# DanecLacey/basic_iterative_solvers

Hardware: AMD Instinct MI355X
Metric: CG iterations/sec + SpMV GFLOP/s (% HBM roofline), HPCG 256^3 at 1/2/4/8 GPUs (higher is better)
Workload: dtype f64

## Files before the change

basic_iterative_solvers_amd/__init__.py:

```python
import ctypes as C
import os

import numpy as np

PKG = os.path.dirname(os.path.abspath(__file__))
LIB_PATH = os.path.join(PKG, "lib", "libbis_hip.so")

PC = dict(none=0, j=1, gs=2, bgs=3, sgs=4, **{"2st": 5, "s2st": 6, "ilu0": 7, "ilu0it": 8, "fsai": 9, "mg": 10, "bj": 11})

_lib = None


class BisError(RuntimeError):
    pass


def load_library():
    global _lib
    if _lib is None:
        if not os.path.exists(LIB_PATH):
            raise BisError(
                f"{LIB_PATH} is missing: build it with "
                "`python -m basic_iterative_solvers_amd.build` (hipcc, gfx950)")
        _lib = C.CDLL(LIB_PATH)
# ... 165 lines not shown

    def scale_sym(self, A, init=0.0):
        s = self.alloc(A.n_rows)
        self.init_vector(s, init)
        self.check(self.lib.bis_mat_scale_sym(self.h, A.h, C.c_void_p(s.ptr)))
        return s

    def gather(self, out, vec, perm):
        n = len(perm)
        raw = np.zeros((n + 1) // 2 + 1)
        raw.view(np.int32)[:n] = np.asarray(perm, dtype=np.int32)
        store = self.upload(raw)
        self.check(self.lib.bis_vec_gather(self.h, C.c_void_p(out.ptr), C.c_void_p(vec.ptr), C.c_void_p(store.ptr), _i64(n)))
        self.sync()
        store.free()

    def tune_placement(self, A, max_trials=6):
        f, b = C.c_double(), C.c_double()
        self.check(self.lib.bis_mat_tune_placement(self.h, A.h, C.c_int(max_trials), C.byref(f), C.byref(b)))
        return f.value, b.value

    def split_strict(self, A):
        n = A.n_rows
        D, Dinv = self.alloc(n), self.alloc(n)
        hl, hu = C.c_void_p(), C.c_void_p()
        self.check(self.lib.bis_mat_split_strict(self.h, A.h, C.byref(hl), C.byref(hu),
                                                 C.c_void_p(D.ptr), C.c_void_p(Dinv.ptr)))
        return Mat(self, hl), Mat(self, hu), D, Dinv

    def mat_diag(self, A, row_offset=0):
        D, Dinv = self.alloc(A.n_rows), self.alloc(A.n_rows)
        self.check(self.lib.bis_mat_diag(self.h, A.h, _i64(row_offset), C.c_void_p(D.ptr), C.c_void_p(Dinv.ptr)))
        return D, Dinv

    def diag_block(self, A, row_offset=0):
        h = C.c_void_p()
        self.check(self.lib.bis_mat_diag_block(self.h, A.h, _i64(row_offset), C.byref(h)))
        return Mat(self, h)

    def ilu0(self, A, pivot_tol=1e-8, pivot_repl=1e-4):
        n = A.n_rows
        L_D, U_D = self.alloc(n), self.alloc(n)
        hl, hu = C.c_void_p(), C.c_void_p()
        self.check(self.lib.bis_mat_ilu0(self.h, A.h, C.c_double(pivot_tol), C.c_double(pivot_repl),
                                         C.byref(hl), C.byref(hu), C.c_void_p(L_D.ptr),
                                         C.c_void_p(U_D.ptr)))
        return Mat(self, hl), L_D, Mat(self, hu), U_D

    def iluk(self, A, level, pivot_tol=1e-8, pivot_repl=1e-4):
        n = A.n_rows
        L_D, U_D = self.alloc(n), self.alloc(n)
        hl, hu, nf = C.c_void_p(), C.c_void_p(), C.c_int64()
        self.check(self.lib.bis_mat_iluk(self.h, A.h, C.c_int(int(level)), C.c_double(pivot_tol), C.c_double(pivot_repl),
                                         C.byref(hl), C.byref(hu), C.c_void_p(L_D.ptr), C.c_void_p(U_D.ptr), C.byref(nf)))
        return Mat(self, hl), L_D, Mat(self, hu), U_D, nf.value

    def iluk_symbolic(self, A, level):
        h, nf = C.c_void_p(), C.c_int64()
        self.check(self.lib.bis_mat_iluk_symbolic(self.h, A.h, C.c_int(int(level)), C.byref(h), C.byref(nf)))
        return Mat(self, h), nf.value

    def fsai(self, A):
        hg, hgt, nf = C.c_void_p(), C.c_void_p(), C.c_int64()
        self.check(self.lib.bis_mat_fsai(self.h, A.h, C.byref(hg), C.byref(hgt), C.byref(nf)))
        return Mat(self, hg), Mat(self, hgt), nf.value

    def spgemm(self, A, B):
        h = C.c_void_p()
        self.check(self.lib.bis_spgemm(self.h, A.h, B.h, C.byref(h)))
        return Mat(self, h)

    def mg(self, A, cycle=None, cycle_levels=0, smooth=False, prolong_omega=0.0, smoother=None, degree=2, ratio=None, est_steps=10,
           safety=1.1, **params):
        m = MG(self, A, smooth=smooth, prolong_omega=prolong_omega, **params)
        try:
            if cycle is not None:
                m.set_cycle(cycle, cycle_levels)
            if smoother is not None:
                m.set_smoother(smoother, degree=degree, ratio=ratio, est_steps=est_steps, safety=safety)
        except Exception:
            m.free()
            raise
        return m

    def bjacobi(self, A, block_size=None, block_ptr=None, symmetrize=False):
        return BJ(self, A, block_size, block_ptr, symmetrize)

    def spmv(self, A, x, y):
        self.check(self.lib.bis_spmv(self.h, A.h, C.c_void_p(x.ptr), C.c_void_p(y.ptr)))

    def spmm(self, A, X, Y, k):
        self.check(self.lib.bis_spmm(self.h, A.h, C.c_void_p(X.ptr), C.c_void_p(Y.ptr), C.c_int(int(k))))

    def mvec_set_col(self, X, n, k, j, v):
        self.check(self.lib.bis_mvec_set_col(self.h, C.c_void_p(X.ptr), _i64(n), C.c_int(int(k)), C.c_int(int(j)), C.c_void_p(v.ptr)))

    def mvec_get_col(self, v, X, n, k, j):
        self.check(self.lib.bis_mvec_get_col(self.h, C.c_void_p(v.ptr), C.c_void_p(X.ptr), _i64(n), C.c_int(int(k)), C.c_int(int(j))))

    def sptrsv(self, Ls, x, D, b):
        self.check(self.lib.bis_sptrsv(self.h, Ls.h, C.c_void_p(x.ptr), C.c_void_p(D.ptr),
                                       C.c_void_p(b.ptr)))

    def bsptrsv(self, Us, x, D, b):
        self.check(self.lib.bis_bsptrsv(self.h, Us.h, C.c_void_p(x.ptr), C.c_void_p(D.ptr),
                                        C.c_void_p(b.ptr)))

    def sptrsm(self, Ls, X, D, B, k):
        self.check(self.lib.bis_sptrsm(self.h, Ls.h, C.c_void_p(X.ptr), C.c_void_p(D.ptr), C.c_void_p(B.ptr), C.c_int(int(k))))

    def bsptrsm(self, Us, X, D, B, k):
        self.check(self.lib.bis_bsptrsm(self.h, Us.h, C.c_void_p(X.ptr), C.c_void_p(D.ptr), C.c_void_p(B.ptr), C.c_int(int(k))))

    def mitrsv(self, T, D_inv, B, X, work, n_sweeps, k):
        self.check(self.lib.bis_mitrsv(self.h, T.h, C.c_void_p(D_inv.ptr), C.c_void_p(B.ptr), C.c_void_p(X.ptr),
                                       C.c_void_p(work.ptr) if work is not None else C.c_void_p(), C.c_int(int(n_sweeps)), C.c_int(int(k))))

    def mvec_div_diag(self, R, A, D, n, k):
        self.check(self.lib.bis_mvec_div_diag(self.h, C.c_void_p(R.ptr), C.c_void_p(A.ptr), C.c_void_p(D.ptr), _i64(n), C.c_int(int(k))))

    def mvec_mul_diag(self, R, A, D, n, k):
        self.check(self.lib.bis_mvec_mul_diag(self.h, C.c_void_p(R.ptr), C.c_void_p(A.ptr), C.c_void_p(D.ptr), _i64(n), C.c_int(int(k))))

    def itrsv(self, T, D_inv, b, x, work, n_sweeps):
        self.check(self.lib.bis_itrsv(self.h, T.h, C.c_void_p(D_inv.ptr), C.c_void_p(b.ptr), C.c_void_p(x.ptr),
                                      C.c_void_p(work.ptr) if work is not None else C.c_void_p(), C.c_int(int(n_sweeps))))

    def _ew3(self, fn, r, a, b, scale, n=None):
        n = r.n if n is None else n
        self.check(fn(self.h, C.c_void_p(r.ptr), C.c_void_p(a.ptr), C.c_void_p(b.ptr), _i64(n),
                      C.c_double(scale)))

    def subtract_vectors(self, r, a, b, scale=1.0, n=None):
        self._ew3(self.lib.bis_subtract_vectors, r, a, b, scale, n)

    def sum_vectors(self, r, a, b, scale=1.0, n=None):
        self._ew3(self.lib.bis_sum_vectors, r, a, b, scale, n)

    def elemwise_mult_vectors(self, r, a, b, scale=1.0, n=None):
        self._ew3(self.lib.bis_elemwise_mult_vectors, r, a, b, scale, n)

    def elemwise_div_vectors(self, r, a, b, scale=1.0, n=None):
        self._ew3(self.lib.bis_elemwise_div_vectors, r, a, b, scale, n)

    def compute_residual(self, A, x, b, res, tmp):
        self.check(self.lib.bis_compute_residual(self.h, A.h, C.c_void_p(x.ptr), C.c_void_p(b.ptr),
                                                 C.c_void_p(res.ptr), C.c_void_p(tmp.ptr)))

    def dot(self, a, b, n=None):
        out = C.c_double()
        self.check(self.lib.bis_dot(self.h, C.c_void_p(a.ptr), C.c_void_p(b.ptr),
                                    _i64(a.n if n is None else n), C.byref(out)))
        return out.value

    def euclidean_vec_norm(self, v, n=None):
        out = C.c_double()
        self.check(self.lib.bis_euclidean_vec_norm(self.h, C.c_void_p(v.ptr),
                                                   _i64(v.n if n is None else n), C.byref(out)))
        return out.value

    def scale(self, r, v, scalar, n=None):
        self.check(self.lib.bis_scale(self.h, C.c_void_p(r.ptr), C.c_void_p(v.ptr),
                                      C.c_double(scalar), _i64(r.n if n is None else n)))

    def init_vector(self, v, val, n=None):
        self.check(self.lib.bis_init_vector(self.h, C.c_void_p(v.ptr), C.c_double(val),
                                            _i64(v.n if n is None else n)))

    def copy_vector(self, out, inp, n=None):
        self.check(self.lib.bis_copy_vector(self.h, C.c_void_p(out.ptr), C.c_void_p(inp.ptr),
                                            _i64(out.n if n is None else n)))

    def normalize_x(self, x_new, x_old, D, b):
        self.check(self.lib.bis_normalize_x(self.h, C.c_void_p(x_new.ptr), C.c_void_p(x_old.ptr),
                                            C.c_void_p(D.ptr), C.c_void_p(b.ptr), _i64(x_new.n)))

    def multi_axpy(self, V, ldv, y_host, n_vec, out, n):
        y = np.ascontiguousarray(y_host, dtype=np.float64)
        self.check(self.lib.bis_multi_axpy(self.h, C.c_void_p(V.ptr), _i64(ldv), y.ctypes,
                                           C.c_int(n_vec), C.c_void_p(out.ptr), _i64(n)))

    def apply_preconditioner(self, pc, n, Ls, Us, A_D, A_D_inv, L_D, U_D, out, inp, tmp, work,
                             outer=1, inner=0):
        def p(v):
            return C.c_void_p(v.ptr) if v is not None else C.c_void_p()
        self.check(self.lib.bis_apply_preconditioner(
            self.h, C.c_int(PC[pc] if isinstance(pc, str) else pc), _i64(n),
            Ls.h if Ls is not None else C.c_void_p(), Us.h if Us is not None else C.c_void_p(),
            p(A_D), p(A_D_inv), p(L_D), p(U_D), p(out), p(inp), p(tmp), p(work),
            C.c_int(outer), C.c_int(inner)))

    def mapply_preconditioner(self, pc, n, k, Ls, Us, A_D, A_D_inv, L_D, U_D, out, inp, tmp, work, outer=1, inner=0):
        def p(v):
            return C.c_void_p(v.ptr) if v is not None else C.c_void_p()
        self.check(self.lib.bis_mapply_preconditioner(
            self.h, C.c_int(PC[pc] if isinstance(pc, str) else pc), _i64(n), C.c_int(int(k)),
            Ls.h if Ls is not None else C.c_void_p(), Us.h if Us is not None else C.c_void_p(),
            p(A_D), p(A_D_inv), p(L_D), p(U_D), p(out), p(inp), p(tmp), p(work),
            C.c_int(outer), C.c_int(inner)))

    def cg(self, A, b, x, A_D=None):
        return CG(self, A, b, x, A_D)

    def mcg(self, A, B, X, k, A_D=None):
        return MCG(self, A, B, X, k, A_D)

    def mbicgstab(self, A, B, X, k):
        return MBiCGSTAB(self, A, B, X, k)

    def mgmres(self, A, B, X, k, restart=10):
        return MGMRES(self, A, B, X, k, restart)

    def fgmres(self, A, b, x, restart=10):
        return FGMRES(self, A, b, x, restart)

    def minres(self, A, b, x):
        return MINRES(self, A, b, x)

    def idr(self, A, b, x, s=4):
        return IDR(self, A, b, x, s)

    def stat(self, kind, A, D, b, x, Ls=None, Us=None):
        return Stat(self, kind, A, D, b, x, Ls, Us)

    def profile(self, on):
        self.check(self.lib.bis_profile_enable(self.h, C.c_int(int(on))))

    def profile_read(self):
        n = C.c_int64()
        ms = C.c_double()
        self.check(self.lib.bis_profile_read(self.h, C.byref(n), C.byref(ms)))
        return n.value, ms.value

    def profile_read_sweeps(self):
        n = C.c_int64()
        ms = C.c_double()
        self.check(self.lib.bis_profile_read_sweeps(self.h, C.byref(n), C.byref(ms)))
        return n.value, ms.value


class Vec:

    def __init__(self, ctx, ptr, n, owner):
        self.ctx, self.ptr, self.n, self.owner = ctx, ptr, n, owner

    def offset(self, k, n=None):
        return Vec(self.ctx, self.ptr + 8 * int(k), self.n - int(k) if n is None else n, False)

    def to_host(self):
        out = np.empty(self.n, dtype=np.float64)
        self.ctx.check(self.ctx.lib.bis_vec_download(self.ctx.h, out.ctypes, C.c_void_p(self.ptr),
                                                     _i64(self.n)))
        return out

    def set(self, arr):
        arr = np.ascontiguousarray(arr, dtype=np.float64)
        assert arr.size == self.n
        self.ctx.check(self.ctx.lib.bis_vec_upload(self.ctx.h, C.c_void_p(self.ptr), arr.ctypes,
                                                   _i64(self.n)))

    def free(self):
        if self.owner and self.ptr:
            self.ctx.lib.bis_vec_free(self.ctx.h, C.c_void_p(self.ptr))
            self.ptr = 0


class Mat:
    def __init__(self, ctx, h):
        self.ctx, self.h = ctx, h
        n_rows, n_cols, nnz = C.c_int64(), C.c_int64(), C.c_int64()
        ctx.lib.bis_mat_info(h, C.byref(n_rows), C.byref(n_cols), C.byref(nnz))
        self.n_rows, self.n_cols, self.nnz = n_rows.value, n_cols.value, nnz.value

    @property
    def rp_width(self):
        return int(self.ctx.lib.bis_mat_rp_width(self.h))

    def spmv_stream_info(self):
        c, v, d, f = C.c_int(), C.c_int(), C.c_int(), C.c_int()
        self.ctx.check(self.ctx.lib.bis_mat_spmv_stream_info(self.ctx.h, self.h, C.byref(c), C.byref(v), C.byref(d), C.byref(f)))
        return c.value, v.value, d.value, f.value

    def spmv_streamed_bytes(self):
        b = C.c_int64()
        self.ctx.check(self.ctx.lib.bis_mat_spmv_streamed_bytes(self.ctx.h, self.h, C.byref(b)))
        return b.value

    def debug_ptrs(self):
        a, b, c = C.c_void_p(), C.c_void_p(), C.c_void_p()
        self.ctx.check(self.ctx.lib.bis_mat_debug_ptrs(self.h, C.byref(a), C.byref(b), C.byref(c)))
        return a.value, b.value, c.value

    def win8_tuning(self):
        t, a, b = C.c_int(), C.c_double(), C.c_double()
        self.ctx.lib.bis_mat_win8_tuning(self.h, C.byref(t), C.byref(a), C.byref(b))
        return t.value, a.value, b.value

    def win8_layout(self):
        ch, ex, sl = C.c_int64(), C.c_int64(), C.c_int64()
        bl, im = C.c_int(), C.c_int()
        self.ctx.lib.bis_mat_win8_layout(self.h, C.byref(ch), C.byref(ex), C.byref(sl), C.byref(bl), C.byref(im))
        return ch.value, ex.value, sl.value, bl.value, bool(im.value)

    def colslab_info(self):
        k, a, b = C.c_int(), C.c_double(), C.c_double()
        self.ctx.lib.bis_mat_colslab_info(self.h, C.byref(k), C.byref(a), C.byref(b))
        return k.value, a.value, b.value

    def sweep_kernel(self, backward=False):
        return self.ctx.lib.bis_mat_sweep_kernel(self.h, C.c_int(int(backward))).decode()

    def sweepm_kernel(self, backward=False):
        return self.ctx.lib.bis_mat_sweepm_kernel(self.h, C.c_int(int(backward))).decode()

    def spmv_kernel(self, fused=False):
        return self.ctx.lib.bis_mat_spmv_kernel(self.h, C.c_int(int(fused))).decode()

    def spmm_kernel(self):
        return self.ctx.lib.bis_mat_spmm_kernel(self.h).decode()

    def spmm_streamed_bytes(self, k):
        b = C.c_int64()
        if self.ctx.lib.bis_mat_spmm_streamed_bytes(self.h, C.c_int(int(k)), C.byref(b)) != 0:
            raise BisError("bis_mat_spmm_streamed_bytes: bad arguments")
        return b.value

    def ilu0_kernel(self):
        return self.ctx.lib.bis_mat_ilu0_kernel(self.h).decode()

    def iluk_kernel(self):
        return self.ctx.lib.bis_mat_iluk_kernel(self.h).decode()

    def fsai_kernel(self):
        return self.ctx.lib.bis_mat_fsai_kernel(self.h).decode()

    def itrsv_kernel(self):
        return self.ctx.lib.bis_itrsv_kernel(self.h).decode()

    def spgemm_kernel(self):
        return self.ctx.lib.bis_spgemm_kernel(self.h).decode()

    def transpose(self):
        h = C.c_void_p()
        self.ctx.check(self.ctx.lib.bis_mat_transpose(self.ctx.h, self.h, C.byref(h)))
        return Mat(self.ctx, h)

    def round_f32(self):
        m = C.c_double()
        self.ctx.check(self.ctx.lib.bis_mat_round_f32(self.ctx.h, self.h, C.byref(m)))
        return m.value

    def grid_hint(self):
        g = (C.c_int64 * 4)()
        self.ctx.check(self.ctx.lib.bis_mat_grid_hint(self.h, g))
        return tuple(g)

    def retune(self):
        self.ctx.check(self.ctx.lib.bis_mat_retune(self.ctx.h, self.h))

    def set_grid_hint(self, nx, ny, nz, dof=1):
        self.ctx.check(self.ctx.lib.bis_mat_set_grid_hint(self.h, _i64(nx), _i64(ny), _i64(nz), C.c_int(dof)))

    def download(self):
        rp = np.zeros(self.n_rows + 1, dtype=np.int64)
        col = np.zeros(self.nnz, dtype=np.int32)
        val = np.zeros(self.nnz, dtype=np.float64)
        self.ctx.check(self.ctx.lib.bis_mat_download(self.ctx.h, self.h, rp.ctypes, col.ctypes,
                                                     val.ctypes))
        return rp, col, val

    def free(self):
        if self.h:
            self.ctx.lib.bis_mat_destroy(self.ctx.h, self.h)
            self.h = C.c_void_p()


class MGParams(C.Structure):
    _fields_ = [("max_levels", C.c_int), ("coarse_limit", C.c_int64), ("coarsening", C.c_int), ("nu", C.c_int),
                ("coarse_sweeps", C.c_int), ("omega", C.c_double), ("coarse_scale", C.c_double)]


class MGSmoother(C.Structure):
    _fields_ = [("kind", C.c_int), ("degree", C.c_int), ("ratio", C.c_double), ("est_steps", C.c_int), ("safety", C.c_double)]


class MG:

    COARSENING = dict(auto=0, grid=1, mis=2)
    CYCLE = dict(v=0, w=1, k=2, kgcr=3)
    SMOOTHER = dict(jacobi=0, cheb=1)
    DEFAULT_RATIO = 4.0

    def __init__(self, ctx, A, max_levels=10, coarse_limit=256, coarsening=0, nu=1, coarse_sweeps=4, omega=0.0, coarse_scale=1.0,
                 smooth=False, prolong_omega=0.0):
        self.ctx, self._keep = ctx, A
        self.h = C.c_void_p()
        self.smoothed = bool(smooth)
        p = MGParams(int(max_levels), int(coarse_limit), int(self.COARSENING.get(coarsening, coarsening)), int(nu),
                     int(coarse_sweeps), float(omega), float(coarse_scale))
        if self.smoothed:
            ctx.check(ctx.lib.bis_mg_create_smoothed(ctx.h, A.h, C.byref(p), C.c_double(float(prolong_omega)), C.byref(self.h)))
        else:
            if prolong_omega:
                raise BisError("MG: prolong_omega needs smooth=True")
            ctx.check(ctx.lib.bis_mg_create(ctx.h, A.h, C.byref(p), C.byref(self.h)))
        n = C.c_int()
        rows, nnz, kinds = (C.c_int64 * 16)(), (C.c_int64 * 16)(), (C.c_int * 16)()
        ctx.lib.bis_mg_info(self.h, C.byref(n), rows, nnz, kinds)
        self.levels = n.value
        self.rows, self.nnz, self.kinds = list(rows[:n.value]), list(nnz[:n.value]), list(kinds[:n.value])
        self.operand = Mat(ctx, C.c_void_p(ctx.lib.bis_mg_operand(self.h)))

    def level_matrix(self, l):
        h = self.ctx.lib.bis_mg_level_matrix(self.h, C.c_int(int(l)))
        if not h:
            raise BisError(f"MG.level_matrix: no level {l}")
        return Mat(self.ctx, C.c_void_p(h))

    def prolongator(self, l):
        h = self.ctx.lib.bis_mg_level_prolongator(self.h, C.c_int(int(l)))
        return Mat(self.ctx, C.c_void_p(h)) if h else None

    def restrictor(self, l):
        h = self.ctx.lib.bis_mg_level_restrictor(self.h, C.c_int(int(l)))
        return Mat(self.ctx, C.c_void_p(h)) if h else None

    def prolong_omega(self, l):
        w = C.c_double()
        return w.value if self.ctx.lib.bis_mg_level_prolong_omega(self.h, C.c_int(int(l)), C.byref(w)) == 0 else None

    def aggregates(self, l):
        out = np.zeros(self.rows[l], dtype=np.int32)
        self.ctx.check(self.ctx.lib.bis_mg_level_aggregates(self.ctx.h, self.h, C.c_int(int(l)), out.ctypes))
        return out

    def weights(self, l):
        out = np.zeros(self.rows[l], dtype=np.float64)
        self.ctx.check(self.ctx.lib.bis_mg_level_weights(self.ctx.h, self.h, C.c_int(int(l)), out.ctypes))
        return out

    def set_cycle(self, cycle, levels=0):
        if isinstance(cycle, str):
            if cycle not in self.CYCLE:
                raise BisError(f"MG.set_cycle: cycle {cycle!r} is none of {sorted(self.CYCLE)}")
            cycle = self.CYCLE[cycle]
        self.ctx.check(self.ctx.lib.bis_mg_set_cycle(self.ctx.h, self.h, C.c_int(int(cycle)), C.c_int(int(levels))))

    @property
    def cycle(self):
        c, k = C.c_int(), C.c_int()
        self.ctx.check(self.ctx.lib.bis_mg_cycle(self.h, C.byref(c), C.byref(k)))
        return c.value, k.value

    def set_smoother(self, kind, degree=2, ratio=None, est_steps=10, safety=1.1):
        if isinstance(kind, str):
            if kind not in self.SMOOTHER:
                raise BisError(f"MG.set_smoother: kind {kind!r} is none of {sorted(self.SMOOTHER)}")
            kind = self.SMOOTHER[kind]
        s = MGSmoother(int(kind), int(degree), float(self.DEFAULT_RATIO if ratio is None else ratio), int(est_steps), float(safety))
        self.ctx.check(self.ctx.lib.bis_mg_set_smoother(self.ctx.h, self.h, C.byref(s)))

    def smoother(self):
        s = MGSmoother()
        self.ctx.check(self.ctx.lib.bis_mg_smoother_info(self.h, C.byref(s)))
        return dict(kind=s.kind, degree=s.degree, ratio=s.ratio, est_steps=s.est_steps, safety=s.safety)

    def spectrum(self, l):
        v = [C.c_double() for _ in range(4)]
        if self.ctx.lib.bis_mg_level_spectrum(self.h, C.c_int(int(l)), *[C.byref(x) for x in v]) != 0:
            return None
        return dict(zip(("bound", "estimate", "lambda_max", "lambda_min"), (x.value for x in v)))

    def cheb_coeffs(self, l):
        k = self.smoother()["degree"]
        c1, c2 = np.zeros(max(k, 1)), np.zeros(max(k, 1))
        if self.ctx.lib.bis_mg_level_cheb_coeffs(self.h, C.c_int(int(l)), c1.ctypes, c2.ctypes) != 0:
            return None
        return c1[:k], c2[:k]

    def apply(self, out, inp):
        self.ctx.check(self.ctx.lib.bis_mg_apply(self.ctx.h, self.h, C.c_void_p(out.ptr), C.c_void_p(inp.ptr)))

    def free(self):
        if self.h:
            self.ctx.lib.bis_mg_destroy(self.ctx.h, self.h)
            self.h = C.c_void_p()


class BJParams(C.Structure):
    _fields_ = [("block_size", C.c_int), ("block_ptr", C.POINTER(C.c_int32)), ("n_blocks", C.c_int64), ("symmetrize", C.c_int)]


class BJ:

    def __init__(self, ctx, A, block_size=None, block_ptr=None, symmetrize=False):
        self.ctx = ctx
        self.h = C.c_void_p()
        if block_ptr is not None:
            bp = np.ascontiguousarray(block_ptr, dtype=np.int32)
            p = BJParams(0 if block_size is None else int(block_size), bp.ctypes.data_as(C.POINTER(C.c_int32)), len(bp) - 1,
                         int(bool(symmetrize)))
        else:
            if block_size is None:
                raise BisError("Context.bjacobi: give block_size or block_ptr")
            p = BJParams(int(block_size), None, 0, int(bool(symmetrize)))
        ctx.check(ctx.lib.bis_bj_create(ctx.h, A.h, C.byref(p), C.byref(self.h)))
        self.n_blocks, self.max_block, self.value_count = self.info()
        self.operand = Mat(ctx, C.c_void_p(ctx.lib.bis_bj_operand(self.h)))

    def info(self):
        nb, mb, vc = C.c_int64(), C.c_int(), C.c_int64()
        self.ctx.lib.bis_bj_info(self.h, C.byref(nb), C.byref(mb), C.byref(vc))
        return nb.value, mb.value, vc.value

    def blocks(self):
        vals = np.zeros(self.value_count, dtype=np.float64)
        offs = np.zeros(self.n_blocks + 1, dtype=np.int64)
        self.ctx.check(self.ctx.lib.bis_bj_blocks(self.ctx.h, self.h, vals.ctypes, offs.ctypes))
        return vals, offs

    def apply(self, out, inp):
        self.ctx.check(self.ctx.lib.bis_bj_apply(self.ctx.h, self.h, C.c_void_p(out.ptr), C.c_void_p(inp.ptr)))

    def mapply(self, out, inp, k):
        self.ctx.check(self.ctx.lib.bis_bj_mapply(self.ctx.h, self.h, C.c_void_p(out.ptr), C.c_void_p(inp.ptr), C.c_int(int(k))))

    def free(self):
        if self.h:
            self.ctx.lib.bis_bj_destroy(self.ctx.h, self.h)
            self.h = C.c_void_p()


def _handle_pc(pc, Ls):
    if isinstance(pc, MG):
        return "mg", pc.operand
    if isinstance(pc, BJ):
        return "bj", pc.operand
    return pc, Ls


class _Solver:

    _sym = None

    def _fn(self, what):
        return getattr(self.ctx.lib, f"bis_{self._sym}_{what}")

    def set_preconditioner(self, pc, Ls=None, Us=None, A_D=None, A_D_inv=None, L_D=None, U_D=None, outer=1, inner=0):
        def p(v):
            return C.c_void_p(v.ptr) if v is not None else C.c_void_p()
        pc, Ls = _handle_pc(pc, Ls)
        self._keep_pc = (Ls, Us, A_D, A_D_inv, L_D, U_D)
        self.ctx.check(self._fn("set_preconditioner")(
            self.ctx.h, self.h, C.c_int(PC[pc] if isinstance(pc, str) else pc),
            Ls.h if Ls is not None else C.c_void_p(), Us.h if Us is not None else C.c_void_p(),
            p(A_D), p(A_D_inv), p(L_D), p(U_D), C.c_int(outer), C.c_int(inner)))

    def iterate(self, n):
        self.ctx.check(self._fn("iterate")(self.ctx.h, self.h, C.c_int(int(n))))

    def free(self):
        if self.h:
            self._fn("destroy")(self.ctx.h, self.h)
            self.h = C.c_void_p()


class CG(_Solver):
    _sym = "cg"

    def __init__(self, ctx, A, b, x, A_D=None):
        self.ctx = ctx
        self.h = C.c_void_p()
        ctx.check(ctx.lib.bis_cg_create(ctx.h, A.h, C.c_void_p(A_D.ptr) if A_D else C.c_void_p(),
                                        C.c_void_p(b.ptr), C.c_void_p(x.ptr), C.byref(self.h)))

    def init(self, tol):
        r0 = C.c_double()
        self.ctx.check(self.ctx.lib.bis_cg_init(self.ctx.h, self.h, C.c_double(tol), C.byref(r0)))
        return r0.value

    def status(self, hist_cap=4096):
        iters, conv = C.c_int(), C.c_int()
        hist = np.zeros(hist_cap)
        self.ctx.check(self.ctx.lib.bis_cg_status(self.ctx.h, self.h, C.byref(iters), C.byref(conv),
                                                  hist.ctypes, C.c_int(hist_cap)))
        return iters.value, bool(conv.value), hist[:min(iters.value + 1, hist_cap)].copy()


class MCG(_Solver):

    _sym = "mcg"

    def __init__(self, ctx, A, B, X, k, A_D=None):
        self.ctx, self.k = ctx, int(k)
        self.h = C.c_void_p()
        self._keep = (A, B, X, A_D)
        ctx.check(ctx.lib.bis_mcg_create(ctx.h, A.h, C.c_void_p(A_D.ptr) if A_D else C.c_void_p(),
                                         C.c_void_p(B.ptr), C.c_void_p(X.ptr), C.c_int(self.k), C.byref(self.h)))

    def init(self, tol):
        r0 = np.zeros(self.k)
        self.ctx.check(self.ctx.lib.bis_mcg_init(self.ctx.h, self.h, C.c_double(tol), r0.ctypes))
        return r0

    def status(self, j, hist_cap=4096):
        iters, conv = C.c_int(), C.c_int()
# ... 289 lines not shown
```

basic_iterative_solvers_amd/csrc/bis_blas1.hip:

```cpp
#include "bis_internal.hpp"

#include <algorithm>
#include <cstdlib>

namespace {

constexpr int kEwThreads = 256;
constexpr int kMaxEwBlocks = 16384;

inline int ew_grid(int64_t n_items) {
    int64_t g = (n_items + kEwThreads - 1) / kEwThreads;
    if (g < 1) g = 1;
    if (g > kMaxDotBlocks) g = kMaxDotBlocks;
    return (int)g;
}
inline int ew_grid_wide(int64_t n_items) {
    int64_t g = (n_items + kEwThreads - 1) / kEwThreads;
    if (g < 1) g = 1;
    if (g > kMaxEwBlocks) g = kMaxEwBlocks;
    return (int)g;
}

typedef double ew_v2d_t __attribute__((ext_vector_type(2)));
__device__ __forceinline__ double2 ld_stream(const double2 *p) {
    const ew_v2d_t v = __builtin_nontemporal_load(reinterpret_cast<const ew_v2d_t *>(p));
    return make_double2(v.x, v.y);
}
__device__ __forceinline__ double ld_stream(const double *p) { return __builtin_nontemporal_load(p); }

inline bool aligned16(const void *p) { return (reinterpret_cast<uintptr_t>(p) & 15) == 0; }

enum { OP_SUB, OP_SUM, OP_MUL, OP_DIV };

template <int OP>
__device__ __forceinline__ double ew_apply(double a, double b, double s) {
    if (OP == OP_SUB) return fma(-s, b, a);
    if (OP == OP_SUM) return fma(s, b, a);
    if (OP == OP_MUL) return (a * s) * b;
    return a / (s * b);
}

template <int OP, bool VEC>
__global__ __launch_bounds__(kEwThreads) void ew3_kernel(double *r, const double *a,
                                                         const double *b, int64_t n,
                                                         double s_val, const double *s_dev) {
    const double s = s_dev ? *s_dev : s_val;
    const int64_t stride = (int64_t)gridDim.x * kEwThreads;
    int64_t i = (int64_t)blockIdx.x * kEwThreads + threadIdx.x;
    if (VEC) {
        const int64_t n2 = n >> 1;
        const double2 *a2 = reinterpret_cast<const double2 *>(a);
        const double2 *b2 = reinterpret_cast<const double2 *>(b);
        double2 *r2 = reinterpret_cast<double2 *>(r);
        for (; i < n2; i += stride) {
            double2 av = ld_stream(a2 + i), bv = ld_stream(b2 + i), rv;
            rv.x = ew_apply<OP>(av.x, bv.x, s);
            rv.y = ew_apply<OP>(av.y, bv.y, s);
            r2[i] = rv;
        }
        if ((n & 1) && blockIdx.x == 0 && threadIdx.x == 0)
            r[n - 1] = ew_apply<OP>(a[n - 1], b[n - 1], s);
    } else {
        for (; i < n; i += stride) r[i] = ew_apply<OP>(ld_stream(a + i), ld_stream(b + i), s);
    }
}

enum { U_SCALE, U_COPY, U_FILL };

template <int OP, bool VEC>
__global__ __launch_bounds__(kEwThreads) void ew2_kernel(double *r, const double *a,
                                                         int64_t n, double s_val, const double *s_dev) {
    const double s = s_dev ? *s_dev : s_val;
    const int64_t stride = (int64_t)gridDim.x * kEwThreads;
    int64_t i = (int64_t)blockIdx.x * kEwThreads + threadIdx.x;
    if (VEC) {
        const int64_t n2 = n >> 1;
        const double2 *a2 = reinterpret_cast<const double2 *>(a);
        double2 *r2 = reinterpret_cast<double2 *>(r);
        for (; i < n2; i += stride) {
            double2 rv;
            if (OP == U_FILL) {
                rv.x = s; rv.y = s;
            } else {
                double2 av = ld_stream(a2 + i);
                rv.x = (OP == U_SCALE) ? av.x * s : av.x;
                rv.y = (OP == U_SCALE) ? av.y * s : av.y;
            }
            r2[i] = rv;
        }
        if ((n & 1) && blockIdx.x == 0 && threadIdx.x == 0)
            r[n - 1] = (OP == U_FILL) ? s : ((OP == U_SCALE) ? a[n - 1] * s : a[n - 1]);
    } else {
        for (; i < n; i += stride)
            r[i] = (OP == U_FILL) ? s : ((OP == U_SCALE) ? a[i] * s : a[i]);
    }
}

__global__ __launch_bounds__(kEwThreads) void normalize_x_kernel(double *x_new,
                                                                 const double *x_old,
                                                                 const double *D,
                                                                 const double *b,
                                                                 int64_t n) {
    const int64_t stride = (int64_t)gridDim.x * kEwThreads;
    for (int64_t i = (int64_t)blockIdx.x * kEwThreads + threadIdx.x; i < n; i += stride) {
        const double d = ld_stream(D + i);
        const double adjusted = fma(-d, ld_stream(x_old + i), ld_stream(x_new + i));
        x_new[i] = (ld_stream(b + i) - adjusted) / d;
    }
}

struct MultiAxpyCoef { double y[64]; };
__global__ __launch_bounds__(kEwThreads) void multi_axpy_kernel(const double *V, int64_t ldv,
                                                                MultiAxpyCoef c, int n_vec,
                                                                double *out, int64_t n) {
    const int64_t stride = (int64_t)gridDim.x * kEwThreads;
    for (int64_t i = (int64_t)blockIdx.x * kEwThreads + threadIdx.x; i < n; i += stride) {
        double acc = 0.0;
        for (int k = 0; k < n_vec; ++k) acc = fma(ld_stream(V + (int64_t)k * ldv + i), c.y[k], acc);
        out[i] = acc;
    }
}

template <bool VEC, bool SAME>
__global__ __launch_bounds__(kEwThreads) void dot_partial_kernel(const double *a,
                                                                 const double *b, int64_t n,
                                                                 double *partials) {
    __shared__ double lds[kEwThreads / 64];
    const int64_t stride = (int64_t)gridDim.x * kEwThreads;
    int64_t i = (int64_t)blockIdx.x * kEwThreads + threadIdx.x;
    double acc0 = 0.0, acc1 = 0.0;
    if (VEC) {
        const int64_t n2 = n >> 1;
        const double2 *a2 = reinterpret_cast<const double2 *>(a);
        const double2 *b2 = reinterpret_cast<const double2 *>(b);
        for (; i < n2; i += stride) {
            const double2 av = ld_stream(a2 + i), bv = SAME ? av : ld_stream(b2 + i);
            acc0 = fma(av.x, bv.x, acc0);
            acc1 = fma(av.y, bv.y, acc1);
        }
        if ((n & 1) && blockIdx.x == 0 && threadIdx.x == 0)
            acc0 = fma(a[n - 1], b[n - 1], acc0);
    } else {
        for (; i < n; i += stride) { const double av = ld_stream(a + i); acc0 = fma(av, SAME ? av : ld_stream(b + i), acc0); }
    }
    const double s = block_sum<kEwThreads>(acc0 + acc1, lds);
    if (threadIdx.x == 0) partials[blockIdx.x] = s;
}

template <bool VEC>
__global__ __launch_bounds__(kEwThreads) void axpy_dot_kernel(double *w, const double *u, const double *v, int64_t n,
                                                              const double *s_dev, double *partials) {
    __shared__ double lds[kEwThreads / 64];
    const double s = *s_dev;
    const int64_t stride = (int64_t)gridDim.x * kEwThreads;
    int64_t i = (int64_t)blockIdx.x * kEwThreads + threadIdx.x;
    double acc0 = 0.0, acc1 = 0.0;
    if (VEC) {
        const int64_t n2 = n >> 1;
        double2 *w2 = reinterpret_cast<double2 *>(w);
        const double2 *u2 = reinterpret_cast<const double2 *>(u);
        const double2 *v2 = reinterpret_cast<const double2 *>(v);
        for (; i < n2; i += stride) {
            double2 wv = ld_stream(w2 + i);
            const double2 uv = ld_stream(u2 + i);
            wv.x = ew_apply<OP_SUB>(wv.x, uv.x, s);
            wv.y = ew_apply<OP_SUB>(wv.y, uv.y, s);
            w2[i] = wv;
            const double2 vv = v ? ld_stream(v2 + i) : wv;
            acc0 = fma(wv.x, vv.x, acc0);
            acc1 = fma(wv.y, vv.y, acc1);
        }
        if ((n & 1) && blockIdx.x == 0 && threadIdx.x == 0) {
            const double t = ew_apply<OP_SUB>(w[n - 1], u[n - 1], s);
            w[n - 1] = t;
            acc0 = fma(t, v ? v[n - 1] : t, acc0);
        }
    } else {
        for (; i < n; i += stride) {
            const double t = ew_apply<OP_SUB>(w[i], u[i], s);
            w[i] = t;
            acc0 = fma(t, v ? v[i] : t, acc0);
        }
    }
    const double r = block_sum<kEwThreads>(acc0 + acc1, lds);
    if (threadIdx.x == 0) partials[blockIdx.x] = r;
}

__global__ __launch_bounds__(256) void reduce_finish_kernel(const double *partials,
                                                            int n_partials, size_t stride,
                                                            double *result) {
    __shared__ double lds[4];
    const double *p = partials + (size_t)blockIdx.x * stride;
    double acc = 0.0;
    for (int i = threadIdx.x; i < n_partials; i += 256) acc += p[i];
    const double s = block_sum<256>(acc, lds);
    if (threadIdx.x == 0) result[blockIdx.x] = s;
}

enum { SC_DIV, SC_RATIO_PRODUCT, SC_SQRT_INV };
__global__ void scalar_kernel(int op, double *out, double *out2, const double *a, const double *b, const double *c,
                              const double *d) {
    if (op == SC_DIV) *out = *a / *b;
    else if (op == SC_RATIO_PRODUCT) *out = (*a / *b) * (*c / *d);
    else { const double nrm = sqrt(*a); *out = nrm; *out2 = 1.0 / nrm; }
}

}

bis_status bis_reduce_finish(bis_ctx *ctx, int n_partials, int n_values, size_t stride,
                             double *result_dev) {
    hipLaunchKernelGGL(reduce_finish_kernel, dim3(n_values), dim3(256), 0, ctx->stream,
                       ctx->partials, n_partials, stride, result_dev);
    BIS_HIP_CHECK(ctx, hipGetLastError());
    return BIS_OK;
}

bis_status bis_ensure_partials(bis_ctx *ctx, size_t n) {
    if (n <= ctx->partials_cap) return BIS_OK;
    BIS_HIP_CHECK(ctx, hipStreamSynchronize(ctx->stream));
    if (ctx->partials) BIS_HIP_CHECK(ctx, hipFree(ctx->partials));
    ctx->partials = nullptr;
    ctx->partials_cap = 0;
    BIS_HIP_CHECK(ctx, hipMalloc(&ctx->partials, sizeof(double) * n));
    ctx->partials_cap = n;
    return BIS_OK;
}

bis_status bis_fault_check(bis_ctx *ctx) {
    volatile unsigned *f = ctx->fault_host;
    if (!f || *f == 0) return BIS_OK;
    *f = 0;
    ctx->err = "a triangular sweep lost a hand-off: a row waited for a result that was never published "
               "(a workgroup of the persistent grid could not become resident, or the dependency data is corrupt); "
               "the vectors written since the last blocking call are invalid";
    return BIS_ERR_SYNC;
}

#define BIS_OPTIONS_ENV(X) X(spmv_variant) X(spmv_window) X(spmv_chunk) X(spmv_chunk_fused) X(spmv_xcd_remap) X(trsv_grid) X(ilu0_wgs) X(trsv_wave_wgs) X(trsv_trial) X(trsv_one_xcd) X(trsv_host_analysis) X(ilu0_wave) X(spmv_packed) X(spmv_packed32) X(spmv_valdict) X(spmv_sellwin) X(device_share) X(spmv_sellwin_rows) X(spmv_sellwin_joint) X(spmv_sellwin_pairs) X(spmv_sellwin_masks) X(spmv_colslab) X(spmv_win8) X(spmv_win8_rows) X(spmv_win8_depth) X(spmv_win8_sets) X(spmv_win8_implicit) X(spmv_win8_tune) X(spmv_win4) X(grid_autodetect) X(tune_placement) X(force_rp64) X(trsv_tiled) X(trsv_chain) X(trsv_tile_rows) X(trsv_tile_wgs) X(trsv_tile_edge) X(trsv_tile_backoff)
#define BIS_OPTIONS_API(Y) Y(trsv_batch) Y(trsv_wave) Y(ilu0_persistent) Y(trsv_by_pos) Y(spmv_lds_pad) Y(trsv_chain_idle) Y(trsv_chain_pause) Y(trsv_chain_pairs) Y(trsv_chain_prefix) Y(trsv_tile_exp) Y(cg_nt_x) Y(spmv_sellwin_nt) Y(dist_host_plan) Y(trsv_inject_loss) Y(trsv_inject_oom) Y(trsm_form) Y(spgemm_row_cap) Y(spgemm_batch)

namespace {
std::string &opts_env_seen() { static std::string s; return s; }
std::string upper_env(const char *name) {
    std::string e = "BIS_";
    for (const char *c = name; *c; ++c) e += (char)((*c >= 'a' && *c <= 'z') ? *c - 32 : *c);
    return e;
}
}

bis_options &bis_opts() {
    static bis_options o = [] {
        bis_options v;
#define X(name) { const std::string en = upper_env(#name); if (const char *e = getenv(en.c_str())) { v.name = atoi(e); \
                  std::string &seen = opts_env_seen(); if (!seen.empty()) seen += ' '; seen += en + "=" + e; } }
        BIS_OPTIONS_ENV(X)
#undef X
        return v;
    }();
    return o;
}

extern "C" {

bis_status bis_set_option(const char *name, int value) {
    if (!name) return BIS_ERR_INVALID;
    bis_options &o = bis_opts();
#define X(opt) if (!strcmp(name, #opt)) { o.opt = value; return BIS_OK; }
    BIS_OPTIONS_ENV(X)
    BIS_OPTIONS_API(X)
#undef X
    return BIS_ERR_INVALID;
}

int bis_options_describe(char *buf, int cap) {
    const bis_options &o = bis_opts();
    std::string s = "{";
    bool first = true;
#define X(opt) if (o.opt != -1) { if (!first) s += ", "; first = false; s += std::string("\"") + #opt + "\": " + std::to_string(o.opt); }
    BIS_OPTIONS_ENV(X)
    BIS_OPTIONS_API(X)
#undef X
    if (!first) s += ", ";
    s += "\"env\": \"";
    for (char c : opts_env_seen()) if (c != '"' && c != '\\' && (unsigned char)c >= 32) s += c;
    s += "\"}";
    if (buf && cap > 0) { const int n = std::min((int)s.size(), cap - 1); memcpy(buf, s.data(), (size_t)n); buf[n] = 0; }
    return (int)s.size();
}

int bis_abi_version(void) { return 1; }

bis_status bis_ctx_create(int device, void *stream, bis_ctx **out) {
    if (!out) return BIS_ERR_INVALID;
    *out = nullptr;
    int count = 0;
    if (hipGetDeviceCount(&count) != hipSuccess || count <= 0) return BIS_ERR_NO_DEVICE;
    if (device < 0 || device >= count) return BIS_ERR_NO_DEVICE;
    if (hipSetDevice(device) != hipSuccess) return BIS_ERR_NO_DEVICE;
    hipDeviceProp_t prop;
    if (hipGetDeviceProperties(&prop, device) != hipSuccess) return BIS_ERR_NO_DEVICE;
    bis_ctx *ctx = new bis_ctx;
    ctx->device = device;
    ctx->n_cus = prop.multiProcessorCount;
    ctx->arch = prop.gcnArchName;
    ctx->hbm_bytes = (int64_t)prop.totalGlobalMem;
    if (ctx->arch.rfind("gfx950", 0) != 0) {
        fprintf(stderr, "bis_hip: device %d is %s, this library is built for gfx950 only\n",
                device, ctx->arch.c_str());
        delete ctx;
        return BIS_ERR_NO_DEVICE;
    }
    if (stream) {
        ctx->stream = (hipStream_t)stream;
    } else {
        if (hipStreamCreateWithFlags(&ctx->stream, hipStreamNonBlocking) != hipSuccess) {
            delete ctx;
            return BIS_ERR_HIP;
        }
        ctx->own_stream = true;
    }
    ctx->partials_cap = std::max((size_t)kMaxReduceBlocks * 4, (size_t)kMaxDotBlocks * 2);
    bool ok = hipMalloc(&ctx->partials, sizeof(double) * ctx->partials_cap) == hipSuccess &&
              hipMalloc(&ctx->scalars_dev, sizeof(double) * 64) == hipSuccess &&
              hipHostMalloc(&ctx->scalars_host, sizeof(double) * 64) == hipSuccess &&
              hipMalloc(&ctx->counters, sizeof(unsigned) * 64) == hipSuccess &&
              hipMemset(ctx->counters, 0, sizeof(unsigned) * 64) == hipSuccess &&
              hipMemset(ctx->scalars_dev, 0, sizeof(double) * 64) == hipSuccess &&
              hipHostMalloc(&ctx->fault_host, sizeof(unsigned) * 16, hipHostMallocMapped) == hipSuccess &&
              hipHostGetDevicePointer((void **)&ctx->fault_dev, ctx->fault_host, 0) == hipSuccess;
    if (ok) memset(ctx->fault_host, 0, sizeof(unsigned) * 16);
    if (!ok) {
        delete ctx;
        return BIS_ERR_HIP;
    }
    *out = ctx;
    return BIS_OK;
}

bis_status bis_ctx_destroy(bis_ctx *ctx) {
    BIS_CTX_OK(ctx);
    hipStreamSynchronize(ctx->stream);
    for (auto &p : ctx->prof_events) { hipEventDestroy(p.first); hipEventDestroy(p.second); }
    for (auto &p : ctx->prof_sweep_events) { hipEventDestroy(p.first); hipEventDestroy(p.second); }
    hipFree(ctx->partials);
    hipFree(ctx->scalars_dev);
    hipHostFree(ctx->scalars_host);
    hipFree(ctx->counters);
    hipHostFree(ctx->fault_host);
    if (ctx->own_stream) hipStreamDestroy(ctx->stream);
    delete ctx;
    return BIS_OK;
}

const char *bis_last_error(const bis_ctx *ctx) { return ctx ? ctx->err.c_str() : "no context (no usable gfx950 device)"; }

bis_status bis_sync(bis_ctx *ctx) {
    BIS_CTX_OK(ctx);
    BIS_SYNC_CHECK(ctx);
    return BIS_OK;
}

void *bis_ctx_stream(bis_ctx *ctx) { return ctx ? (void *)ctx->stream : nullptr; }

bis_status bis_device_info(bis_ctx *ctx, char *arch, size_t arch_len, int *n_cus,
                           int64_t *hbm_bytes) {
    BIS_CTX_OK(ctx);
    if (arch && arch_len) {
        strncpy(arch, ctx->arch.c_str(), arch_len - 1);
        arch[arch_len - 1] = 0;
    }
    if (n_cus) *n_cus = ctx->n_cus;
    if (hbm_bytes) *hbm_bytes = ctx->hbm_bytes;
    return BIS_OK;
}

bis_status bis_vec_alloc(bis_ctx *ctx, int64_t n, double **out) {
    BIS_CTX_OK(ctx);
    BIS_REQUIRE(ctx, out && n >= 0, "bis_vec_alloc: bad arguments");
    void *p = nullptr;
    BIS_HIP_CHECK(ctx, hipMalloc(&p, sizeof(double) * (size_t)(n > 0 ? n : 1)));
    *out = (double *)p;
    return BIS_OK;
}

bis_status bis_vec_free(bis_ctx *ctx, double *v) {
    BIS_CTX_OK(ctx);
    if (!v) return BIS_OK;
    BIS_HIP_CHECK(ctx, hipStreamSynchronize(ctx->stream));
    BIS_HIP_CHECK(ctx, hipFree(v));
    return BIS_OK;
}

bis_status bis_vec_upload(bis_ctx *ctx, double *dst, const double *src, int64_t n) {
    BIS_CTX_OK(ctx);
    BIS_REQUIRE(ctx, n >= 0 && (n == 0 || (dst && src)), "bis_vec_upload: bad arguments");
    if (n == 0) return BIS_OK;
    BIS_HIP_CHECK(ctx, hipMemcpyAsync(dst, src, sizeof(double) * (size_t)n, hipMemcpyHostToDevice,
                                      ctx->stream));
    BIS_HIP_CHECK(ctx, hipStreamSynchronize(ctx->stream));
    return BIS_OK;
}

bis_status bis_vec_download(bis_ctx *ctx, double *dst, const double *src, int64_t n) {
    BIS_CTX_OK(ctx);
    BIS_REQUIRE(ctx, n >= 0 && (n == 0 || (dst && src)), "bis_vec_download: bad arguments");
    if (n == 0) return BIS_OK;
    BIS_HIP_CHECK(ctx, hipMemcpyAsync(dst, src, sizeof(double) * (size_t)n, hipMemcpyDeviceToHost,
                                      ctx->stream));
    BIS_SYNC_CHECK(ctx);
    return BIS_OK;
}

}

template <int OP>
static bis_status launch_ew3(bis_ctx *ctx, double *r, const double *a, const double *b,
                             int64_t n, double s, const double *s_dev = nullptr) {
    BIS_CTX_OK(ctx);
    BIS_REQUIRE(ctx, n >= 0 && (n == 0 || (r && a && b)), "elementwise kernel: bad arguments");
    if (n == 0) return BIS_OK;
    const bool vec = aligned16(r) && aligned16(a) && aligned16(b) && n >= 2;
    if (vec)
        hipLaunchKernelGGL((ew3_kernel<OP, true>), dim3(ew_grid_wide(n >> 1)), dim3(kEwThreads), 0,
                           ctx->stream, r, a, b, n, s, s_dev);
    else
        hipLaunchKernelGGL((ew3_kernel<OP, false>), dim3(ew_grid_wide(n)), dim3(kEwThreads), 0,
                           ctx->stream, r, a, b, n, s, s_dev);
    BIS_HIP_CHECK(ctx, hipGetLastError());
    return BIS_OK;
}

template <int OP>
static bis_status launch_ew2(bis_ctx *ctx, double *r, const double *a, int64_t n, double s, const double *s_dev = nullptr);

extern "C" {

bis_status bis_subtract_vectors(bis_ctx *ctx, double *r, const double *a, const double *b,
                                int64_t n, double scale) {
    return launch_ew3<OP_SUB>(ctx, r, a, b, n, scale);
}
bis_status bis_sum_vectors(bis_ctx *ctx, double *r, const double *a, const double *b, int64_t n,
                           double scale) {
    return launch_ew3<OP_SUM>(ctx, r, a, b, n, scale);
}
bis_status bis_elemwise_mult_vectors(bis_ctx *ctx, double *r, const double *a, const double *b,
                                     int64_t n, double scale) {
    return launch_ew3<OP_MUL>(ctx, r, a, b, n, scale);
}
bis_status bis_elemwise_div_vectors(bis_ctx *ctx, double *r, const double *a, const double *b,
                                    int64_t n, double scale) {
    return launch_ew3<OP_DIV>(ctx, r, a, b, n, scale);
}
bis_status bis_subtract_vectors_dev(bis_ctx *ctx, double *r, const double *a, const double *b,
                                    int64_t n, const double *scale_dev) {
    BIS_REQUIRE(ctx, scale_dev, "bis_subtract_vectors_dev: null scalar");
    return launch_ew3<OP_SUB>(ctx, r, a, b, n, 0.0, scale_dev);
}
bis_status bis_sum_vectors_dev(bis_ctx *ctx, double *r, const double *a, const double *b, int64_t n,
                               const double *scale_dev) {
    BIS_REQUIRE(ctx, scale_dev, "bis_sum_vectors_dev: null scalar");
    return launch_ew3<OP_SUM>(ctx, r, a, b, n, 0.0, scale_dev);
}

}

template <int OP>
static bis_status launch_ew2(bis_ctx *ctx, double *r, const double *a, int64_t n, double s, const double *s_dev) {
    BIS_CTX_OK(ctx);
    BIS_REQUIRE(ctx, n >= 0 && (n == 0 || (r && (a || OP == U_FILL))),
                "elementwise kernel: bad arguments");
    if (n == 0) return BIS_OK;
    const bool vec = aligned16(r) && (OP == U_FILL || aligned16(a)) && n >= 2;
    if (vec)
        hipLaunchKernelGGL((ew2_kernel<OP, true>), dim3(ew_grid_wide(n >> 1)), dim3(kEwThreads), 0,
                           ctx->stream, r, a, n, s, s_dev);
    else
        hipLaunchKernelGGL((ew2_kernel<OP, false>), dim3(ew_grid_wide(n)), dim3(kEwThreads), 0,
                           ctx->stream, r, a, n, s, s_dev);
    BIS_HIP_CHECK(ctx, hipGetLastError());
    return BIS_OK;
}

extern "C" {

bis_status bis_scale(bis_ctx *ctx, double *r, const double *v, double scalar, int64_t n) {
    return launch_ew2<U_SCALE>(ctx, r, v, n, scalar);
}
bis_status bis_scale_dev(bis_ctx *ctx, double *r, const double *v, const double *scalar_dev, int64_t n) {
    BIS_REQUIRE(ctx, scalar_dev, "bis_scale_dev: null scalar");
    return launch_ew2<U_SCALE>(ctx, r, v, n, 0.0, scalar_dev);
}
bis_status bis_init_vector(bis_ctx *ctx, double *v, double val, int64_t n) {
    return launch_ew2<U_FILL>(ctx, v, nullptr, n, val);
}
bis_status bis_copy_vector(bis_ctx *ctx, double *out, const double *in, int64_t n) {
    if (out == in) return ctx ? BIS_OK : BIS_ERR_NO_DEVICE;
    return launch_ew2<U_COPY>(ctx, out, in, n, 0.0);
}

bis_status bis_normalize_x(bis_ctx *ctx, double *x_new, const double *x_old, const double *D,
                           const double *b, int64_t n) {
    BIS_CTX_OK(ctx);
    BIS_REQUIRE(ctx, n >= 0 && (n == 0 || (x_new && x_old && D && b)), "bis_normalize_x: bad arguments");
    if (n == 0) return BIS_OK;
    hipLaunchKernelGGL(normalize_x_kernel, dim3(ew_grid_wide(n)), dim3(kEwThreads), 0, ctx->stream,
                       x_new, x_old, D, b, n);
    BIS_HIP_CHECK(ctx, hipGetLastError());
    return BIS_OK;
}

bis_status bis_multi_axpy(bis_ctx *ctx, const double *V, int64_t ldv, const double *y_host,
                          int n_vec, double *out, int64_t n) {
    BIS_CTX_OK(ctx);
    BIS_REQUIRE(ctx, n >= 0 && n_vec >= 0 && n_vec <= 64 && (n == 0 || (V && out)) &&
                         (n_vec == 0 || y_host),
                "bis_multi_axpy: bad arguments (n_vec must be <= 64)");
    if (n == 0) return BIS_OK;
    MultiAxpyCoef c;
    for (int k = 0; k < 64; ++k) c.y[k] = k < n_vec ? y_host[k] : 0.0;
    hipLaunchKernelGGL(multi_axpy_kernel, dim3(ew_grid_wide(n)), dim3(kEwThreads), 0, ctx->stream, V,
                       ldv, c, n_vec, out, n);
    BIS_HIP_CHECK(ctx, hipGetLastError());
    return BIS_OK;
}

bis_status bis_dot_dev(bis_ctx *ctx, const double *a, const double *b, int64_t n,
                       double *result_dev) {
    BIS_CTX_OK(ctx);
    BIS_REQUIRE(ctx, n >= 0 && result_dev && (n == 0 || (a && b)), "bis_dot: bad arguments");
    const bool vec = aligned16(a) && aligned16(b) && n >= 2;
    const int grid = n == 0 ? 1 : (vec ? ew_grid(n >> 1) : ew_grid(n));
#define BIS_DOT_LAUNCH(V, S) hipLaunchKernelGGL((dot_partial_kernel<V, S>), dim3(grid), dim3(kEwThreads), 0, ctx->stream, a, b, n, ctx->partials)
    if (vec) { if (a == b) BIS_DOT_LAUNCH(true, true); else BIS_DOT_LAUNCH(true, false); }
    else { if (a == b) BIS_DOT_LAUNCH(false, true); else BIS_DOT_LAUNCH(false, false); }
#undef BIS_DOT_LAUNCH
    BIS_HIP_CHECK(ctx, hipGetLastError());
    return bis_reduce_finish(ctx, grid, 1, 0, result_dev);
}

bis_status bis_axpy_dot_dev(bis_ctx *ctx, double *w, const double *u, const double *scale_dev, const double *v, int64_t n,
                            double *result_dev) {
// ... 107 lines not shown
```

basic_iterative_solvers_amd/csrc/bis_internal.hpp:

```cpp
#pragma once

#include <hip/hip_runtime.h>

#include <cstdint>
#include <cstdio>
#include <cstring>
#include <map>
#include <string>
#include <vector>

#include "bis_hip.h"

struct bis_trsv_plan;
struct bis_trsv_tiled;
struct bis_trsv_chain;
struct bis_trsm_plan;
struct bis_trsv_side {
    bis_trsv_plan *level = nullptr;
    bis_trsv_tiled *tiled = nullptr;
    bis_trsv_chain *chain = nullptr;
    bis_trsm_plan *multi = nullptr;
    bool tiled_tried = false, chain_tried = false;
    const char *kernel = "";
    const char *kernel_m = "";
};

struct bis_named_kernel {
    int type = 0;
    const bis_mat *A = nullptr;
    double *B = nullptr, *C = nullptr;
    int64_t size_B = 0, size_C = 0;
    const double *D = nullptr;
    bool upper = false;
};

struct bis_ctx {
    int device = 0;
    hipStream_t stream = nullptr;
    bool own_stream = false;
    int n_cus = 0;
    std::string arch;
    int64_t hbm_bytes = 0;
    std::string err;

    double *partials = nullptr;
    size_t partials_cap = 0;
    double *scalars_dev = nullptr;
    double *scalars_host = nullptr;
    unsigned *counters = nullptr;
    unsigned *fault_host = nullptr, *fault_dev = nullptr;

    std::map<std::string, bis_named_kernel> kernels;

    const int *spmv_stop = nullptr;

    bool profile = false;
    std::vector<std::pair<hipEvent_t, hipEvent_t>> prof_events;
    size_t prof_used = 0;
    std::vector<std::pair<hipEvent_t, hipEvent_t>> prof_sweep_events;
    size_t prof_sweep_used = 0;
};

struct bis_options;
bis_options &bis_opts();
struct bis_options {
    int spmv_variant = -1;
    int spmv_window = -1;
    int spmv_chunk = -1;
    int spmv_chunk_fused = -1;
    int spmv_xcd_remap = -1;
    int trsv_grid = -1;
    int ilu0_wave = -1;
    int ilu0_wgs = -1;
    int ilu0_persistent = -1;
    int trsv_host_analysis = -1;
    int trsv_wave = -1;
    int trsv_wave_wgs = -1;
    int trsv_trial = -1;
    int trsv_batch = -1;
    int trsv_by_pos = -1;
    int trsv_one_xcd = -1;
    int tune_placement = -1;
    int spmv_packed32 = -1;
    int spmv_lds_pad = -1;
    int spmv_packed = -1;
    int spmv_valdict = -1;
    int dist_host_plan = -1;
    int grid_autodetect = -1;
    int trsv_chain = -1;
    int trsv_chain_idle = -1;
    int trsv_chain_pause = -1;
    int trsv_chain_prefix = -1;
    int trsv_chain_pairs = -1;
    int trsv_tiled = -1;
    int trsv_tile_rows = -1;
    int trsv_tile_wgs = -1;
    int trsv_tile_backoff = -1;
    int spmv_sellwin_nt = -1;
    int cg_nt_x = -1;
    int trsv_tile_exp = -1;
    int trsv_tile_edge = -1;
    int force_rp64 = -1;
    int spmv_sellwin = -1;
    int spmv_sellwin_rows = -1;
    int spmv_sellwin_pairs = -1;
    int spmv_sellwin_joint = -1;
    int spmv_colslab = -1;
    int spmv_win8 = -1;
    int spmv_win8_rows = -1;
    int spmv_win8_depth = -1;
    int spmv_win8_sets = -1;
    int spmv_win8_implicit = -1;
    int spmv_win8_tune = -1;
    int spmv_win4 = -1;
    int spmv_sellwin_masks = -1;
    int device_share = -1;
    int trsm_form = -1;
    int spgemm_row_cap = -1;
    int spgemm_batch = -1;
    int trsv_inject_oom = -1;
    int trsv_inject_loss = -1;
};
inline bool bis_want_rp64(int64_t nnz) { return nnz >= (int64_t)INT32_MAX - 8 || bis_opts().force_rp64 > 0; }

constexpr int kMaxReduceBlocks = 2048;
constexpr int kMaxDotBlocks = 8192;
constexpr int kWinMaxTiles = 128;
constexpr int kWinTile = 16;
constexpr int kWinTileLog = 4;
constexpr int kSwRows = 256;
constexpr int kSwMaxR = 4;

struct bis_mat {
    int64_t n_rows = 0, n_cols = 0, nnz = 0;
    bool rp64 = false;
    bool view = false;
    void *row_ptr = nullptr;
    int32_t *col = nullptr;
    double *val = nullptr;
    int32_t *blk_row = nullptr;
    int64_t *blk_nnz = nullptr;
    uint16_t *loc = nullptr;
    int32_t *tiles = nullptr;
    int32_t *tile_cnt = nullptr;
    int64_t loc_base = 0;
    int max_tiles = 0;
    bool win_ok = false;
    int n_blocks = 0;
    uint16_t *pk[2] = {nullptr, nullptr};
    int32_t *pk_seg[2] = {nullptr, nullptr};
    int64_t pk_base[2] = {0, 0};
    int pk_state[2] = {0, 0};
    int pk_kind[2] = {0, 0};
    uint8_t *vcode = nullptr;
    double *vdict = nullptr;
    int64_t vd_base = 0;
    int vd_state = 0, vd_n = 0;
    double *vdiag = nullptr;
    bool vd_diag = false;
    bool vd_rm_only = false;
    int64_t view_row0 = 0;
    int64_t *rm_nnz = nullptr;
    uint16_t *rm_pk = nullptr;
    int32_t *rm_seg = nullptr;
    int64_t rm_base = 0;
    int rm_state = 0, rm_blocks = 0, rm_kind = 1;
    struct bis_sellwin *sw = nullptr;
    int sw_state = 0;
    struct bis_sellwin *sw8 = nullptr;
    std::vector<bis_mat *> *colslabs = nullptr;
    int cs_state = 0;
    double cs_trial_ms[2] = {0.0, 0.0};
    int sw8_state = 0;
    struct bis_sellwin *sw4 = nullptr;
    int sw4_state = 0;
    bool f32_exact = false;
    int32_t *blkf_row = nullptr;
    int64_t *blkf_nnz = nullptr;
    int n_blocks_f = 0;
    int chunk_f = 0;
    int chunk_nnz = 0;
    int max_row_nnz = 0;
    int64_t max_block_nnz = 0;
    int64_t grid[4] = {0, 0, 0, 0};
    bis_trsv_side trsv[2];
    const char *spmv_kernel[2] = {"", ""};
    const char *ilu0_kernel = "";
    const char *itrsv_kernel = "";
    const char *spmm_kernel = "";
    const char *iluk_kernel = "";
    const char *spgemm_kernel = "";
    const char *fsai_kernel = "";
    struct bis_mg *mg = nullptr;
    struct bis_bj *bj = nullptr;
};

#define BIS_HIP_CHECK(ctx, call)                                               \
    do {                                                                       \
        hipError_t e_ = (call);                                                \
        if (e_ != hipSuccess) {                                                \
            (ctx)->err = std::string(#call) + ": " + hipGetErrorString(e_);    \
            return BIS_ERR_HIP;                                                \
        }                                                                      \
    } while (0)

bis_status bis_fault_check(bis_ctx *ctx);
#define BIS_SYNC_CHECK(ctx)                                                    \
    do {                                                                       \
        BIS_HIP_CHECK(ctx, hipStreamSynchronize((ctx)->stream));               \
        if (bis_status fs_ = bis_fault_check(ctx)) return fs_;                 \
    } while (0)

#define BIS_REQUIRE(ctx, cond, msg)                                            \
    do {                                                                       \
        if (!(cond)) {                                                         \
            if (ctx) (ctx)->err = (msg);                                       \
            return BIS_ERR_INVALID;                                            \
        }                                                                      \
    } while (0)

#define BIS_CTX_OK(ctx)                                                        \
    do {                                                                       \
        if (!(ctx)) return BIS_ERR_NO_DEVICE;                                  \
    } while (0)

template <class T>
inline bis_status bis_alloc_zeroed(bis_ctx *ctx, T **out, size_t count) {
    const size_t bytes = sizeof(T) * count;
    return hipMalloc(out, bytes) == hipSuccess && hipMemsetAsync(*out, 0, bytes, ctx->stream) == hipSuccess ? BIS_OK : BIS_ERR_HIP;
}

__device__ __forceinline__ double wave_sum(double v) {
#pragma unroll
    for (int off = 32; off > 0; off >>= 1) v += __shfl_down(v, off, 64);
    return v;
}

__device__ __forceinline__ double bis_mul_sep(double a, double b) {
    double p = a * b;
    asm volatile("" : "+v"(p));
    return p;
}

template <int T>
__device__ __forceinline__ double block_sum(double v, double *lds ) {
    v = wave_sum(v);
    const int lane = threadIdx.x & 63, w = threadIdx.x >> 6;
    if (lane == 0) lds[w] = v;
    __syncthreads();
    double r = 0.0;
    if (threadIdx.x == 0) {
#pragma unroll
        for (int i = 0; i < T / 64; ++i) r += lds[i];
    }
    return r;
}

__device__ __forceinline__ void publish(double *slot, double v) {
    __hip_atomic_store(slot, v, __ATOMIC_RELAXED, __HIP_MEMORY_SCOPE_AGENT);
}
__device__ __forceinline__ double fetch(const double *slot) {
    return __hip_atomic_load(slot, __ATOMIC_RELAXED, __HIP_MEMORY_SCOPE_AGENT);
}
__device__ __forceinline__ bool arrive_last(unsigned *counter, unsigned n_groups) {
    asm volatile("s_waitcnt vmcnt(0)" ::: "memory");
    const unsigned t = __hip_atomic_fetch_add(counter, 1u, __ATOMIC_RELAXED, __HIP_MEMORY_SCOPE_AGENT);
    if (t != n_groups - 1) return false;
    __hip_atomic_store(counter, 0u, __ATOMIC_RELAXED, __HIP_MEMORY_SCOPE_AGENT);
    return true;
}

constexpr unsigned kArriveGroup = 16;
constexpr unsigned kArriveSubs = 2048 / kArriveGroup;
__device__ __forceinline__ bool arrive_last2(unsigned *top, unsigned *sub, unsigned block, unsigned n_blocks) {
    asm volatile("s_waitcnt vmcnt(0)" ::: "memory");
    const unsigned g = block / kArriveGroup;
    const unsigned n_in = min(kArriveGroup, n_blocks - g * kArriveGroup), n_groups = (n_blocks + kArriveGroup - 1) / kArriveGroup;
    if (__hip_atomic_fetch_add(&sub[g], 1u, __ATOMIC_RELAXED, __HIP_MEMORY_SCOPE_AGENT) != n_in - 1) return false;
    __hip_atomic_store(&sub[g], 0u, __ATOMIC_RELAXED, __HIP_MEMORY_SCOPE_AGENT);
    if (__hip_atomic_fetch_add(top, 1u, __ATOMIC_RELAXED, __HIP_MEMORY_SCOPE_AGENT) != n_groups - 1) return false;
    __hip_atomic_store(top, 0u, __ATOMIC_RELAXED, __HIP_MEMORY_SCOPE_AGENT);
    return true;
}

__device__ __forceinline__ int xcd_remap(int b, int n_padded8) {
    const int per = n_padded8 >> 3;
    return (b & 7) * per + (b >> 3);
}
__device__ __forceinline__ int xcd_group_remap(int b, int G) {
    const int j = b & 7, q = b >> 3;
    return (q / G) * (8 * G) + j * G + (q % G);
}

inline void bis_prof_begin(bis_ctx *ctx) {
    if (!ctx->profile) return;
    if (ctx->prof_used == ctx->prof_events.size()) {
        hipEvent_t a, b;
        hipEventCreate(&a);
        hipEventCreate(&b);
        ctx->prof_events.emplace_back(a, b);
    }
    hipEventRecord(ctx->prof_events[ctx->prof_used].first, ctx->stream);
}
inline void bis_prof_end(bis_ctx *ctx) {
    if (!ctx->profile) return;
    hipEventRecord(ctx->prof_events[ctx->prof_used].second, ctx->stream);
    ++ctx->prof_used;
}

bis_status bis_reduce_finish(bis_ctx *ctx, int n_partials, int n_values,
                             size_t stride, double *result_dev);
bis_status bis_ensure_partials(bis_ctx *ctx, size_t n);
bis_status bis_spmv_launch(bis_ctx *ctx, const bis_mat *A, const double *x,
                           double *y, const double *w, int *n_partials,
                           size_t partials_off = 0);
bis_status bis_spmm_launch(bis_ctx *ctx, const bis_mat *A, const double *X, double *Y, int n_rhs);
size_t bis_spmv_partials_bound(const bis_mat *A);
bis_status bis_spmv_trsv_level(bis_ctx *ctx, const bis_mat *T, const double *x, double *y,
                               const double *b, const double *D);
bis_status bis_spmv_itrsv_step(bis_ctx *ctx, const bis_mat *T, const double *x_old, double *x_new, const double *b,
                               const double *D_inv, int *form);
bis_status bis_mat_row_view(bis_ctx *ctx, const bis_mat *A, int64_t ra,
                            int64_t rb, bis_mat **out);

bis_status bis_mat_alloc(bis_ctx *ctx, int64_t n_rows, int64_t n_cols,
                         int64_t nnz, bool rp64, bis_mat **out);
bis_status bis_mat_finalize(bis_ctx *ctx, bis_mat *A);
bis_status bis_spmv_build_window(bis_ctx *ctx, bis_mat *A);
void bis_spmv_drop_packed(bis_mat *A);
void bis_spmv_drop_valdict(bis_mat *A);
bis_status bis_spmv_try_valdict(bis_ctx *ctx, bis_mat *A, bool consecutive_ok);
bis_status bis_spmv_sellwin_try(bis_ctx *ctx, bis_mat *A);
int bis_spmv_sellwin_blocks(const bis_mat *A);
int64_t bis_spmv_sellwin_bytes(const bis_mat *A);
int64_t bis_spmv_sellwin_slices(const bis_mat *A);
int bis_spmv_sellwin_format(const bis_mat *A);
bis_status bis_spmv_sellwin_launch(bis_ctx *ctx, const bis_mat *A, const double *x, double *y, int mode, const double *w,
                                   double *partials, const int *stop, int remap_arg, int grid);
void bis_spmv_sellwin_drop(bis_mat *A);
bis_status bis_spmv_win8_try(bis_ctx *ctx, bis_mat *A, int vb = 8);
int bis_spmv_win8_blocks(const bis_mat *A, int vb = 8);
int bis_spmv_win8_rows(const bis_mat *A, int vb = 8);
int64_t bis_spmv_win8_bytes(const bis_mat *A, int vb = 8);
bis_status bis_spmv_win8_launch(bis_ctx *ctx, const bis_mat *A, const double *x, double *y, int mode, const double *w,
                                double *partials, const int *stop, int remap_arg, int grid, int vb = 8);
void bis_spmv_win8_drop(bis_mat *A);
int bis_spmv_win8_active(const bis_mat *A);
bis_status bis_spmv_colslab_build(bis_ctx *ctx, const bis_mat *A, int K, std::vector<bis_mat *> &slabs, bool *ok);
void bis_spmv_colslab_free(bis_ctx *ctx, std::vector<bis_mat *> &slabs);
void bis_spmv_colslab_drop(bis_mat *A);
int bis_spmv_remap_arg(int nb);
int bis_spmv_grid(int nb);
size_t bis_spmv_win8_stream_bytes(const bis_mat *A, int vb = 8);
bool bis_spmv_win8_implied(const bis_mat *A, int vb = 8);
double bis_spmv_win8_moved_bytes(const bis_mat *A, int vb = 8);
bool bis_spmv_win8_fast(const bis_mat *A, double ms, int vb = 8);
void *bis_spmv_win8_swap_stream(bis_mat *A, void *stream, int vb = 8);
bis_status bis_spmv_try_pack(bis_ctx *ctx, bis_mat *A, int t);
void bis_mat_free_meta(bis_mat *A);
void bis_mat_values_changed(bis_mat *A);
void bis_trsv_plan_destroy(bis_trsv_plan *p);
void bis_trsm_plan_destroy(bis_trsm_plan *p);
inline bis_trsv_side &bis_trsv_side_of(bis_mat *A, bool backward) { return A->trsv[backward ? 1 : 0]; }
void bis_trsv_drop(bis_mat *A, bool chains);
bool bis_trsv_holds_plans(const bis_mat *A);
void bis_trsv_plan_adopt(bis_mat *to, bis_mat *from, bool backward);
bis_status bis_mat_split_strict_impl(bis_ctx *ctx, const bis_mat *A, bis_mat **L_strict,
                                     bis_mat **U_strict, double *D, double *D_inv, bool check_diag);
bis_status bis_mat_ilu0_impl(bis_ctx *ctx, const bis_mat *A, double pivot_tol, double pivot_repl, bis_mat **L_strict,
                             bis_mat **U_strict, double *L_D, double *U_D, bool fill);
bis_status bis_mat_sorted_copy(bis_ctx *ctx, const bis_mat *A, bis_mat **W, int64_t **dpos, int64_t **ustart);
bis_status bis_mat_pattern_symmetric(bis_ctx *ctx, const bis_mat *A, bool *symmetric);
bis_status bis_trsv_tiled_build(bis_ctx *ctx, const bis_mat *T, bool backward, bis_trsv_tiled **out);
bis_status bis_trsv_tiled_solve(bis_ctx *ctx, bis_trsv_tiled *p, double *x, const double *D, const double *b);
void bis_trsv_tiled_destroy(bis_trsv_tiled *p);
bis_status bis_trsv_analyse_device(bis_ctx *ctx, const bis_mat *T, bool backward, int32_t *perm_dev,
                                   std::vector<int64_t> &level_ptr, int &n_levels, int64_t &max_width,
                                   bool &triangular, int **level_out = nullptr);
bis_status bis_trsv_chain_build(bis_ctx *ctx, const bis_mat *T, bool backward, const int *level_dev, int n_levels,
                                bis_trsv_chain **out);
bis_status bis_trsv_chain_solve(bis_ctx *ctx, const bis_mat *T, bis_trsv_chain *p, double *x, const double *D, const double *b);
void bis_trsv_chain_destroy(bis_trsv_chain *p);
int bis_trsv_chain_resident_pairs(const bis_ctx *ctx, bool rp64, bool backward);
bis_status bis_trsv_blocks_device(bis_ctx *ctx, const bis_mat *T, bool backward, int max_blocks,
                                  std::vector<int64_t> &bounds, int32_t *perm_dev, bool &triangular);
bis_status bis_trsv_level_sets(bis_ctx *ctx, const bis_mat *T_lower, const std::vector<int64_t> **level_ptr,
                               const int32_t **perm_dev);
```

basic_iterative_solvers_amd/csrc/bis_spmv_sell.hip:

```cpp
#include <algorithm>
#include <cstring>
#include <cstdio>
#include <cstdlib>
#include <vector>

#include <rocprim/rocprim.hpp>

#include "bis_internal.hpp"

struct bis_sellwin {
    int n_blocks = 0;
    int64_t n_slices = 0, total_chunks = 0;
    int32_t *hdr = nullptr;
    int64_t *slice_chunk0 = nullptr;
    int32_t *own_rank = nullptr;
    uint32_t *codes = nullptr;
    double *dict = nullptr;
    int max_gran = 0;
    int fmt = 0;
    int uniform_chunks = 0;
    int n_pairs = 0, pair_stride = 0, diag_pair = -1;
    int16_t *blk_base = nullptr;
    unsigned long long *pair_key = nullptr;
    uint16_t *row_of = nullptr;
    void *own_codes = nullptr;
    size_t w8_desc = 0, w8_side = 0, w8_end = 0;
    int64_t *slice_rec = nullptr;
    int64_t expl_chunks = 0;
    int64_t win_gran_sum = 0;
    int tune_trials = 0;
    double tune_first_ms = 0.0, tune_kept_ms = 0.0;
    int R = 1;
    int vb = 8;
    bool diag = false;
    int pad_idx = 0, diag_idx = 0;
};

namespace {

constexpr int kSwRuns = 32;
constexpr int kSwRunGran = 64;
constexpr int kSwHash = 4096;
constexpr int kSwMaxGran = 940;
constexpr int kSwDefaultR = 2;
constexpr int kSwMaxPairs = 253;
inline int sw_gran_cap(int R) { return R == 4 ? kSwMaxGran : std::min(kSwMaxGran, (65536 - (4096 + 4096 * R) - 16) / 64); }

__device__ __forceinline__ unsigned long long sw_pair_key(int32_t offset, unsigned vcode) {
    return ((unsigned long long)((unsigned)offset ^ 0x80000000u) << 8) | vcode;
}

__device__ __forceinline__ int sw_wave_max(int v) {
    for (int o = 32; o > 0; o >>= 1) v = max(v, __shfl_xor(v, o));
    return v;
}

template <typename RP>
__global__ __launch_bounds__(256) void sw_plan_kernel(const RP *__restrict__ row_ptr, const int32_t *__restrict__ col,
                                                      int64_t n_rows, int R, int max_gran, int64_t row0, int32_t *__restrict__ hdr,
                                                      int32_t *__restrict__ slice_chunks, int32_t *__restrict__ own_rank, int *status) {
    __shared__ int table[kSwHash];
    __shared__ int list[1024];
    __shared__ int cnt, n_runs, failed;
    __shared__ int run_g0[kSwRuns], run_rank[kSwRuns], srt_g0[kSwRuns], srt_rank[kSwRuns + 1];
    const int b = blockIdx.x, tid = threadIdx.x;
    const int64_t r0 = (int64_t)b * kSwRows * R;
    const int rows = (int)min((int64_t)kSwRows * R, n_rows - r0);
    for (int i = tid; i < kSwHash; i += 256) table[i] = -1;
    if (tid == 0) { cnt = 0; n_runs = 0; failed = 0; }
    __syncthreads();
    for (int r = 0; r < R; ++r) {
        const int sl = (tid >> 6) * R + r, lr = sl * 64 + (tid & 63);
        int len = 0;
        if (lr < rows) len = (int)((int64_t)row_ptr[r0 + lr + 1] - (int64_t)row_ptr[r0 + lr]);
        const int m = sw_wave_max(len);
        if ((tid & 63) == 0) { slice_chunks[(size_t)b * 4 * R + sl] = (m + 3) >> 2; atomicMax(&status[5], (m + 3) >> 2); }
    }
    const int64_t s = (int64_t)row_ptr[r0], e = (int64_t)row_ptr[r0 + rows];
    for (int64_t k = s + tid; k < e; k += 256) {
        if (__hip_atomic_load(&failed, __ATOMIC_RELAXED, __HIP_MEMORY_SCOPE_WORKGROUP)) break;
        const int g = col[k] >> 3;
        unsigned h = ((unsigned)g * 2654435761u) >> 20;
        for (;;) {
            const int cur = __hip_atomic_load(&table[h], __ATOMIC_RELAXED, __HIP_MEMORY_SCOPE_WORKGROUP);
            if (cur == g) break;
            if (cur == -1) {
                const int old = atomicCAS(&table[h], -1, g);
                if (old == -1) {
                    if (atomicAdd(&cnt, 1) >= max_gran) atomicExch(&failed, 1);
                    break;
                }
                if (old == g) break;
            }
            h = (h + 1) & (kSwHash - 1);
        }
    }
    __syncthreads();
    const int n = cnt;
    if (failed || n > max_gran) {
        if (tid == 0) atomicExch(&status[0], 1);
        return;
    }
    __syncthreads();
    if (tid == 0) cnt = 0;
    __syncthreads();
    for (int i = tid; i < kSwHash; i += 256) {
        const int g = table[i];
        if (g != -1) list[atomicAdd(&cnt, 1)] = g;
    }
    int P = 2;
    while (P < n) P <<= 1;
    __syncthreads();
    for (int i = n + tid; i < P; i += 256) list[i] = INT32_MAX;
    __syncthreads();
    for (int k = 2; k <= P; k <<= 1)
        for (int j = k >> 1; j > 0; j >>= 1) {
            for (int i = tid; i < P; i += 256) {
                const int o = i ^ j;
                if (o > i) {
                    const int a = list[i], c = list[o];
                    if ((a > c) == ((i & k) == 0)) { list[i] = c; list[o] = a; }
                }
            }
            __syncthreads();
        }
    if (tid == 0) {
        const int64_t c_first = r0 + row0, c_last = c_first + rows - 1;
        int own = -1;
        if ((c_first & 7) == 0) {
            const int g_first = (int)(c_first >> 3), g_last = (int)(c_last >> 3);
            int lo = 0, hi = n - 1;
            while (lo < hi) { const int mid = (lo + hi) >> 1; if (list[mid] < g_first) lo = mid + 1; else hi = mid; }
            if (n > 0 && list[lo] == g_first && lo + (g_last - g_first) < n && list[lo + (g_last - g_first)] == g_last) own = lo;
        }
        own_rank[b] = own;
    }
    for (int i = tid; i < n; i += 256)
        if (i == 0 || list[i] != list[i - 1] + 1) {
            const int idx = atomicAdd(&n_runs, 1);
            if (idx < kSwRuns) { run_g0[idx] = list[i]; run_rank[idx] = i; }
        }
    __syncthreads();
    const int nr = n_runs;
    if (nr > kSwRuns) {
        if (tid == 0) atomicExch(&status[0], 1);
        return;
    }
    if (tid < nr) {
        const int my = run_rank[tid];
        int pos = 0;
        for (int m = 0; m < nr; ++m) pos += run_rank[m] < my;
        srt_g0[pos] = run_g0[tid];
        srt_rank[pos] = my;
    }
    if (tid == 0) srt_rank[nr] = n;
    __syncthreads();
    if (tid == 0) {
        int m = 0;
        for (int k = 0; k < nr; ++k) {
            const int len = srt_rank[k + 1] - srt_rank[k];
            for (int o = 0; o < len; o += kSwRunGran, ++m)
                if (m < kSwRuns) {
                    run_g0[m] = srt_g0[k] + o;
                    run_rank[m] = (srt_rank[k] + o) | (min(kSwRunGran, len - o) << 16);
                }
        }
        n_runs = m;
    }
    __syncthreads();
    const int nr2 = n_runs;
    if (nr2 > kSwRuns) {
        if (tid == 0) atomicExch(&status[0], 1);
        return;
    }
    if (tid < 64) {
        const int k = tid & 31;
        int word = 0;
        if (k < nr2) word = tid < 32 ? run_g0[k] : run_rank[k];
        hdr[(size_t)b * 64 + tid] = word;
    }
    if (tid == 0) atomicMax(&status[1], n);
}

__global__ __launch_bounds__(256) void sw_uniform_kernel(int64_t *__restrict__ chunk0, int64_t n, int64_t per) {
    const int64_t i = (int64_t)blockIdx.x * 256 + threadIdx.x;
    if (i < n) chunk0[i] = i * per;
}

__global__ __launch_bounds__(256) void sw_widen_kernel(const int32_t *__restrict__ in, int64_t *__restrict__ out, int64_t n) {
    const int64_t i = (int64_t)blockIdx.x * 256 + threadIdx.x;
    if (i < n) out[i] = in[i];
}

template <typename RP>
__global__ __launch_bounds__(256) void sw_fill_kernel(const RP *__restrict__ row_ptr, const int32_t *__restrict__ col,
                                                      const uint8_t *__restrict__ vcode, int64_t vd_base, int64_t n_rows, int R, int fmt,
                                                      const int32_t *__restrict__ hdr, const int64_t *__restrict__ slice_chunk0,
                                                      uint32_t *__restrict__ codes, int pad_idx, int diag_idx) {
    __shared__ int g0s[kSwRuns], rk[kSwRuns];
    __shared__ int nr_s;
    const int b = blockIdx.x, tid = threadIdx.x, lane = tid & 63, wv = tid >> 6;
    if (tid < kSwRuns) {
        g0s[tid] = hdr[(size_t)b * 64 + tid];
        const int w2 = hdr[(size_t)b * 64 + 32 + tid];
        rk[tid] = w2 & 0xffff;
        const unsigned long long m = __ballot((w2 >> 16) != 0);
        if (tid == 0) nr_s = __popcll(m);
    }
    __syncthreads();
    const int nr = nr_s;
    const int words = fmt == 2 ? 2 : 3;
    for (int rr = 0; rr < R; ++rr) {
        const int64_t slice = ((int64_t)b * 4 + wv) * R + rr;
        const int64_t r = slice * 64 + lane;
        int64_t rs = 0;
        int len = 0;
        if (r < n_rows) {
            rs = (int64_t)row_ptr[r];
            len = (int)((int64_t)row_ptr[r + 1] - rs);
        }
        const int64_t c0 = slice_chunk0[slice];
        const int nch = (int)(slice_chunk0[slice + 1] - c0);
        for (int c = 0; c < nch; ++c) {
            unsigned cc[4], vv[4];
#pragma unroll
            for (int q = 0; q < 4; ++q) {
                const int j = 4 * c + q;
                cc[q] = 0;
                vv[q] = (unsigned)pad_idx;
                if (j < len) {
                    const int ci = col[rs + j];
                    const int g = ci >> 3;
                    int lo = 0, hi = nr - 1;
                    while (lo < hi) {
                        const int mid = (lo + hi + 1) >> 1;
                        if (g0s[mid] <= g) lo = mid; else hi = mid - 1;
                    }
                    cc[q] = (unsigned)(2 + (rk[lo] + (g - g0s[lo])) * 8 + (ci & 7));
                    const unsigned vb = vcode[rs + j - vd_base];
                    vv[q] = vb == 255u && diag_idx >= 0 ? (unsigned)diag_idx : vb;
                }
            }
            uint32_t *dst = codes + ((size_t)(c0 + c) * 64 + lane) * words;
            if (fmt == 2) {
                dst[0] = (cc[0] << 3 | vv[0]) | (cc[1] << 3 | vv[1]) << 16;
                dst[1] = (cc[2] << 3 | vv[2]) | (cc[3] << 3 | vv[3]) << 16;
            } else {
                const unsigned sh = fmt == 1 ? 3 : 0;
                dst[0] = (cc[0] * 8u) | (cc[1] * 8u) << 16;
                dst[1] = (cc[2] * 8u) | (cc[3] * 8u) << 16;
                dst[2] = (vv[0] << sh) | (vv[1] << sh) << 8 | (vv[2] << sh) << 16 | (vv[3] << sh) << 24;
            }
        }
    }
}

template <typename RP>
__global__ __launch_bounds__(64) void sw_pairs_kernel(const RP *__restrict__ row_ptr, const int32_t *__restrict__ col,
                                                      const uint8_t *__restrict__ vcode, int64_t vd_base, int64_t n_rows, int64_t row0,
                                                      unsigned long long *__restrict__ lists, int *overflow) {
    __shared__ unsigned long long list[256];
    const int lane = threadIdx.x;
    int n = 0;
    for (int64_t rb = (int64_t)blockIdx.x * 64; rb < n_rows && n <= kSwMaxPairs; rb += (int64_t)gridDim.x * 64) {
        if (__hip_atomic_load(overflow, __ATOMIC_RELAXED, __HIP_MEMORY_SCOPE_AGENT)) { n = kSwMaxPairs + 1; break; }
        const int64_t r = rb + lane;
        int64_t k = 0, k1 = 0;
        if (r < n_rows) { k = (int64_t)row_ptr[r]; k1 = (int64_t)row_ptr[r + 1]; }
        while (__ballot(k < k1) && n <= kSwMaxPairs) {
            bool found = true;
            unsigned long long v = 0;
            if (k < k1) {
                v = sw_pair_key(col[k] - (int32_t)(r + row0), vcode[k - vd_base]);
                found = false;
                ++k;
            }
            for (int j = 0; j < n && __ballot(!found); ++j) found |= list[j] == v;
            while (const unsigned long long open = __ballot(!found)) {
                const int leader = (int)__builtin_ctzll(open);
                const unsigned long long lv = __shfl(v, leader);
                if (n == kSwMaxPairs) { n = kSwMaxPairs + 1; break; }
                if (lane == 0) list[n] = lv;
                ++n;
                found |= v == lv;
            }
            __syncthreads();
        }
    }
    if (n > kSwMaxPairs && lane == 0) atomicExch(overflow, 1);
    if (lane == 0) lists[(size_t)blockIdx.x * 257] = (unsigned long long)n;
    for (int j = lane; j < n && j < 256; j += 64) lists[(size_t)blockIdx.x * 257 + 1 + j] = list[j];
}

template <typename RP>
__global__ __launch_bounds__(256) void sw_fill_pairs_kernel(const RP *__restrict__ row_ptr, const int32_t *__restrict__ col,
                                                            const uint8_t *__restrict__ vcode, int64_t vd_base, int64_t n_rows, int64_t row0,
                                                            int R, const int32_t *__restrict__ hdr, const int64_t *__restrict__ slice_chunk0,
                                                            uint32_t *__restrict__ codes, const unsigned long long *__restrict__ pair_key,
                                                            int n_pairs, int pair_stride, int16_t *__restrict__ blk_base, int *status) {
    __shared__ int g0s[kSwRuns], rk[kSwRuns];
    __shared__ int nr_s;
    __shared__ unsigned long long keys[256];
    __shared__ int base[256];
    const int b = blockIdx.x, tid = threadIdx.x, lane = tid & 63, wv = tid >> 6;
    keys[tid] = pair_key[tid];
    base[tid] = INT32_MIN;
    if (tid < kSwRuns) {
        g0s[tid] = hdr[(size_t)b * 64 + tid];
        const int w2 = hdr[(size_t)b * 64 + 32 + tid];
        rk[tid] = w2 & 0xffff;
        const unsigned long long m = __ballot((w2 >> 16) != 0);
        if (tid == 0) nr_s = __popcll(m);
    }
    __syncthreads();
    const int nr = nr_s;
    bool bad = false;
    for (int rr = 0; rr < R; ++rr) {
        const int64_t slice = ((int64_t)b * 4 + wv) * R + rr;
        const int64_t r = slice * 64 + lane;
        const int r_in_block = (wv * R + rr) * 64 + lane;
        int64_t rs = 0;
        int len = 0;
        if (r < n_rows) {
            rs = (int64_t)row_ptr[r];
            len = (int)((int64_t)row_ptr[r + 1] - rs);
        }
        const int64_t c0 = slice_chunk0[slice];
        const int nch = (int)(slice_chunk0[slice + 1] - c0);
        for (int c = 0; c < nch; ++c) {
            unsigned word = 0;
// ... 498 lines not shown
    int over = 0;
    SW_CHECK(hipMemcpyAsync(&over, status + 3, sizeof over, hipMemcpyDeviceToHost, ctx->stream));
    SW_CHECK(hipMemcpyAsync(h.data(), lists, sizeof(unsigned long long) * h.size(), hipMemcpyDeviceToHost, ctx->stream));
    SW_CHECK(hipStreamSynchronize(ctx->stream));
    hipFree(lists); tmp = nullptr;
    if (over) return BIS_OK;
    std::vector<unsigned long long> &all = P.all;
    for (int w = 0; w < n_waves; ++w) {
        const size_t n = (size_t)h[(size_t)w * 257];
        if (n > (size_t)kSwMaxPairs) { all.clear(); return BIS_OK; }
        all.insert(all.end(), h.begin() + (size_t)w * 257 + 1, h.begin() + (size_t)w * 257 + 1 + n);
    }
    std::sort(all.begin(), all.end());
    all.erase(std::unique(all.begin(), all.end()), all.end());
    P.fits = !all.empty() && all.size() <= (size_t)kSwMaxPairs;
    return BIS_OK;
}

static bis_status sw_try_pairs(bis_ctx *ctx, bis_mat *A, const double *table, int pad_idx, SwPairs &P) {
    bis_sellwin *sw = A->sw;
    int *status = (int *)ctx->counters + 52;
    if (!P.known) {
        if (bis_status st = sw_collect_pairs(ctx, A, P)) return st;
        if (!A->sw) return BIS_OK;
    }
    if (!P.fits) return BIS_OK;
    const std::vector<unsigned long long> &all = P.all;
    const int n_pairs = (int)all.size();
    unsigned long long keys[256];
    double vals[256];
    int diag_pair = -1;
    for (int e = 0; e < 256; ++e) { keys[e] = ~0ull; vals[e] = 0.0; }
    for (int e = 0; e < n_pairs; ++e) {
        keys[e] = all[e];
        const unsigned vc = (unsigned)(all[e] & 0xffu);
        if (A->vd_diag && vc == 255u) {
            if (diag_pair >= 0) return BIS_OK;
            diag_pair = e;
        } else vals[e] = table[vc];
    }
    vals[n_pairs] = table[pad_idx];
    const int stride = (n_pairs + 63) / 64 * 64;
    const int nb = sw->n_blocks;
    for (int attempt = (n_pairs <= 32 && diag_pair < 0 && bis_opts().spmv_sellwin_masks != 0) ? 0 : 1; attempt < 2; ++attempt) {
        const bool masks = attempt == 0;
        const int64_t total = sw->total_chunks;
        const size_t code_words = masks ? (size_t)nb * 256 * (size_t)sw->R : 64 * (size_t)(total + 1);
        int16_t *blk_base = nullptr;
        unsigned long long *pair_key = nullptr;
        uint32_t *codes = nullptr;
        double *dict3 = nullptr;
        hipError_t e = hipMalloc(&blk_base, sizeof(int16_t) * (size_t)stride * (size_t)nb);
        if (e == hipSuccess) e = hipMalloc(&pair_key, sizeof keys);
        if (e == hipSuccess) e = hipMalloc(&codes, sizeof(uint32_t) * code_words);
        if (e == hipSuccess) e = hipMalloc(&dict3, sizeof vals);
        if (e == hipSuccess) e = hipMemcpyAsync(pair_key, keys, sizeof keys, hipMemcpyHostToDevice, ctx->stream);
        if (e == hipSuccess) e = hipMemcpyAsync(dict3, vals, sizeof vals, hipMemcpyHostToDevice, ctx->stream);
        if (e == hipSuccess) e = hipMemsetAsync(status + 2, 0, sizeof(int), ctx->stream);
        if (e == hipSuccess && !masks) e = hipMemsetAsync(codes + (size_t)total * 64, 0, sizeof(uint32_t) * 64, ctx->stream);
        if (e == hipSuccess) {
#define SW_FILLP(RP) hipLaunchKernelGGL((sw_fill_pairs_kernel<RP>), dim3(nb), dim3(256), 0, ctx->stream, (const RP *)A->row_ptr, A->col, A->vcode, A->vd_base, A->n_rows, A->view_row0, sw->R, sw->hdr, sw->slice_chunk0, codes, pair_key, n_pairs, stride, blk_base, status)
#define SW_FILLM(RP) hipLaunchKernelGGL((sw_fill_masks_kernel<RP>), dim3(nb), dim3(256), 0, ctx->stream, (const RP *)A->row_ptr, A->col, A->vcode, A->vd_base, A->n_rows, A->view_row0, sw->R, sw->hdr, codes, pair_key, n_pairs, stride, blk_base, status)
            if (masks) { if (A->rp64) SW_FILLM(int64_t); else SW_FILLM(int32_t); }
            else { if (A->rp64) SW_FILLP(int64_t); else SW_FILLP(int32_t); }
#undef SW_FILLP
#undef SW_FILLM
            e = hipGetLastError();
        }
        int bad = 0;
        if (e == hipSuccess) e = hipMemcpyAsync(&bad, status + 2, sizeof bad, hipMemcpyDeviceToHost, ctx->stream);
        if (e == hipSuccess) e = hipStreamSynchronize(ctx->stream);
        if (e != hipSuccess || bad) {
            hipFree(blk_base); hipFree(pair_key); hipFree(codes); hipFree(dict3);
            if (e == hipSuccess && masks) continue;
            if (e == hipSuccess || e == hipErrorOutOfMemory) { (void)hipGetLastError(); return BIS_OK; }
            ctx->err = std::string("bis_spmv sellwin pairs: ") + hipGetErrorString(e);
            bis_spmv_sellwin_drop(A);
            A->sw_state = -1;
            return BIS_ERR_HIP;
        }
        hipFree(sw->dict);
        sw->dict = dict3;
        sw->codes = codes;
        sw->blk_base = blk_base;
        sw->pair_key = pair_key;
        sw->fmt = masks ? 4 : 3;
        sw->n_pairs = n_pairs;
        sw->pair_stride = stride;
        sw->diag_pair = diag_pair;
        A->sw_state = 1;
        return BIS_OK;
    }
    return BIS_OK;
}

static bis_status sw_try_rows(bis_ctx *ctx, bis_mat *A, int R, SwPairs &P);

bis_status bis_spmv_sellwin_try(bis_ctx *ctx, bis_mat *A) {
    if (A->sw_state != 0) return BIS_OK;
    A->sw_state = -1;
    if (!sw_enabled() || A->vd_state != 1 || A->n_rows == 0 || A->nnz == 0 || A->n_cols >= ((int64_t)1 << 31) - 16) return BIS_OK;
    int R = kSwDefaultR;
    while (R > 1 && A->n_rows < (int64_t)kSwRows * R * 1024) R >>= 1;
    bool big = R == 2 && A->n_rows >= (int64_t)kSwRows * 4 * 1024;
    if (bis_opts().spmv_sellwin_rows > 0) {
        R = bis_opts().spmv_sellwin_rows >= 2 ? 2 : 1;
        big = bis_opts().spmv_sellwin_rows >= 4;
    }
    SwPairs P;
    if (big && !A->vd_diag && bis_opts().spmv_sellwin_masks != 0 && bis_opts().spmv_sellwin_pairs != 0) {
        if (bis_status st = sw_collect_pairs(ctx, A, P)) return st;
        if (P.fits && P.all.size() <= 32) {
            if (bis_status st = sw_try_rows(ctx, A, 4, P)) return st;
            if (A->sw_state == 1) return BIS_OK;
            A->sw_state = -1;
        }
    }
    return sw_try_rows(ctx, A, R, P);
}

static bis_status sw_try_rows(bis_ctx *ctx, bis_mat *A, int R, SwPairs &P) {
    const int64_t nb64 = (A->n_rows + (int64_t)kSwRows * R - 1) / ((int64_t)kSwRows * R);
    if (nb64 > (int64_t)1 << 26) return BIS_OK;
    const int nb = (int)nb64;
    double table[256];
    BIS_HIP_CHECK(ctx, hipMemcpyAsync(table, A->vdict, sizeof table, hipMemcpyDeviceToHost, ctx->stream));
    BIS_HIP_CHECK(ctx, hipStreamSynchronize(ctx->stream));
    const int cap_small = A->vd_diag ? 31 : 32, cap_gen = A->vd_diag ? 255 : 256;
    int pad_idx = -1;
    for (int i = 0; i < A->vd_n; ++i)
        if (table[i] == 1.0 && !std::signbit(table[i])) pad_idx = i;
    int n_tab = A->vd_n;
    if (pad_idx < 0) {
        if (n_tab >= cap_gen) return BIS_OK;
        pad_idx = n_tab++;
        table[pad_idx] = 1.0;
    }
    bis_sellwin *sw = new bis_sellwin;
    A->sw = sw;
    sw->n_blocks = nb;
    sw->R = R;
    sw->n_slices = (int64_t)nb * 4 * R;
    sw->diag = A->vd_diag;
    const bool joint = n_tab <= (A->vd_diag ? 7 : 8) && bis_opts().spmv_sellwin_joint != 0;
    sw->fmt = joint ? 2 : (n_tab <= cap_small ? 1 : 0);
    sw->pad_idx = pad_idx;
    sw->diag_idx = !A->vd_diag ? -1 : (sw->fmt == 2 ? 7 : (sw->fmt == 1 ? 31 : 255));
    int32_t *slice_chunks = nullptr;
    void *tmp = nullptr;
    int *status = (int *)ctx->counters + 52;
    SW_CHECK(hipMalloc(&sw->hdr, sizeof(int32_t) * 64 * (size_t)nb));
    SW_CHECK(hipMalloc(&sw->own_rank, sizeof(int32_t) * (size_t)nb));
    SW_CHECK(hipMemsetAsync(sw->own_rank, 0xFF, sizeof(int32_t) * (size_t)nb, ctx->stream));
    SW_CHECK(hipMalloc(&slice_chunks, sizeof(int32_t) * (size_t)(sw->n_slices + 1)));
    SW_CHECK(hipMalloc(&sw->slice_chunk0, sizeof(int64_t) * (size_t)(sw->n_slices + 1)));
    SW_CHECK(hipMalloc(&sw->dict, sizeof table));
    SW_CHECK(hipMemcpyAsync(sw->dict, table, sizeof table, hipMemcpyHostToDevice, ctx->stream));
    SW_CHECK(hipMemsetAsync(status, 0, 2 * sizeof(int), ctx->stream));
    SW_CHECK(hipMemsetAsync(status + 5, 0, sizeof(int), ctx->stream));
    SW_CHECK(hipMemsetAsync(slice_chunks + sw->n_slices, 0, sizeof(int32_t), ctx->stream));
    if (A->rp64) hipLaunchKernelGGL(sw_plan_kernel<int64_t>, dim3(nb), dim3(256), 0, ctx->stream, (const int64_t *)A->row_ptr, A->col, A->n_rows, R, sw_gran_cap(R), A->view_row0, sw->hdr, slice_chunks, sw->own_rank, status);
    else hipLaunchKernelGGL(sw_plan_kernel<int32_t>, dim3(nb), dim3(256), 0, ctx->stream, (const int32_t *)A->row_ptr, A->col, A->n_rows, R, sw_gran_cap(R), A->view_row0, sw->hdr, slice_chunks, sw->own_rank, status);
    SW_CHECK(hipGetLastError());
    int h[2] = {0, 0}, h_maxch = 0;
    SW_CHECK(hipMemcpyAsync(h, status, sizeof h, hipMemcpyDeviceToHost, ctx->stream));
    SW_CHECK(hipMemcpyAsync(&h_maxch, status + 5, sizeof h_maxch, hipMemcpyDeviceToHost, ctx->stream));
    const int64_t ns1 = sw->n_slices + 1;
    hipLaunchKernelGGL(sw_widen_kernel, dim3((unsigned)((ns1 + 255) / 256)), dim3(256), 0, ctx->stream, slice_chunks, sw->slice_chunk0, ns1);
    SW_CHECK(hipGetLastError());
    size_t tmp_bytes = 0;
    SW_CHECK(rocprim::exclusive_scan(nullptr, tmp_bytes, sw->slice_chunk0, sw->slice_chunk0, (int64_t)0, (size_t)ns1, rocprim::plus<int64_t>(), ctx->stream));
    SW_CHECK(hipMalloc(&tmp, tmp_bytes));
    SW_CHECK(rocprim::exclusive_scan(tmp, tmp_bytes, sw->slice_chunk0, sw->slice_chunk0, (int64_t)0, (size_t)ns1, rocprim::plus<int64_t>(), ctx->stream));
    int64_t total = 0;
    SW_CHECK(hipMemcpyAsync(&total, sw->slice_chunk0 + sw->n_slices, sizeof total, hipMemcpyDeviceToHost, ctx->stream));
    SW_CHECK(hipStreamSynchronize(ctx->stream));
    hipFree(tmp); tmp = nullptr;
    hipFree(slice_chunks); slice_chunks = nullptr;
    if (h_maxch > 0 && h_maxch <= 8 && !h[0] && (double)h_maxch * (double)sw->n_slices <= 1.03 * (double)total) {
        hipLaunchKernelGGL(sw_uniform_kernel, dim3((unsigned)((ns1 + 255) / 256)), dim3(256), 0, ctx->stream, sw->slice_chunk0, ns1, (int64_t)h_maxch);
        SW_CHECK(hipGetLastError());
        total = (int64_t)h_maxch * sw->n_slices;
        sw->uniform_chunks = h_maxch;
    }
    sw->total_chunks = total;
    sw->max_gran = h[1];
    if (h[0] || (double)total * 256.0 > 1.3 * (double)A->nnz + 256.0 * 4 * 64) {
        bis_spmv_sellwin_drop(A);
        A->sw_state = -1;
        return BIS_OK;
    }
    if (bis_opts().spmv_sellwin_pairs != 0) {
        if (bis_status st = sw_try_pairs(ctx, A, table, pad_idx, P)) return st;
        if (A->sw && sw->R == 4 && !(A->sw_state == 1 && sw->fmt == 4)) {
            bis_spmv_sellwin_drop(A);
            A->sw_state = -1;
            return BIS_OK;
        }
        if (A->sw_state == 1 || !A->sw) return BIS_OK;
    }
    if (sw->R == 4) { bis_spmv_sellwin_drop(A); A->sw_state = -1; return BIS_OK; }
    const size_t cw = sw->fmt == 2 ? 128 : 192;
    SW_CHECK(hipMalloc(&sw->codes, sizeof(uint32_t) * cw * (size_t)(total + 1)));
    SW_CHECK(hipMemsetAsync(sw->codes + (size_t)total * cw, 0, sizeof(uint32_t) * cw, ctx->stream));
#define SW_FILL(RP) hipLaunchKernelGGL((sw_fill_kernel<RP>), dim3(nb), dim3(256), 0, ctx->stream, (const RP *)A->row_ptr, A->col, A->vcode, A->vd_base, A->n_rows, R, sw->fmt, sw->hdr, sw->slice_chunk0, sw->codes, sw->pad_idx, sw->diag_idx)
    if (A->rp64) SW_FILL(int64_t); else SW_FILL(int32_t);
#undef SW_FILL
    SW_CHECK(hipGetLastError());
    A->sw_state = 1;
    return BIS_OK;
}

int bis_spmv_sellwin_blocks(const bis_mat *A) { return A->sw_state == 1 ? A->sw->n_blocks : 0; }
int64_t bis_spmv_sellwin_slices(const bis_mat *A) { return A->sw_state == 1 ? A->sw->n_slices : 0; }
int bis_spmv_sellwin_format(const bis_mat *A) { return A->sw_state == 1 ? A->sw->fmt : -1; }

int64_t bis_spmv_sellwin_bytes(const bis_mat *A) {
    if (A->sw_state != 1) return 0;
    if (A->sw->fmt == 4)
        return 4 * (int64_t)A->sw->n_blocks * 256 * A->sw->R + (int64_t)A->sw->n_blocks * (256 + 2 * A->sw->pair_stride + 4) + 2048;
    const int64_t chunk_bytes = A->sw->fmt == 3 ? 256 : (A->sw->fmt == 2 ? 512 : 768);
    return A->sw->total_chunks * chunk_bytes + (int64_t)A->sw->n_blocks * (256 + 2 * A->sw->pair_stride) + 8 * (A->sw->n_slices + 1) + 2048;
}

bis_status bis_spmv_sellwin_launch(bis_ctx *ctx, const bis_mat *A, const double *x, double *y, int mode, const double *w,
                                   double *partials, const int *stop, int remap_arg, int grid) {
    const bis_sellwin *sw = A->sw;
    const int x_al16 = ((uintptr_t)x & 15) == 0;
    const size_t win = (size_t)(2 + 8 * sw->max_gran) * 8;
    const size_t win_off3 = (size_t)sw_layout3(sw->n_pairs, sw->diag, sw->R).win_off;
    static long long *dbg_buf = nullptr;
    static int dbg_cap = 0;
    long long *dbg = nullptr;
    const char *dbg_file = getenv("BIS_SELLWIN_DEBUG");
    if (dbg_file) {
        if (dbg_cap < sw->n_blocks) { hipFree(dbg_buf); dbg_buf = nullptr; if (hipMalloc(&dbg_buf, sizeof(long long) * 4 * (size_t)sw->n_blocks) == hipSuccess) dbg_cap = sw->n_blocks; }
        dbg = dbg_buf;
    }
    const int32_t *own = (mode == 1 && w == x + A->view_row0 && x_al16) ? sw->own_rank : nullptr;
    if (sw->fmt == 4) {
#define SM_L3(MODE, RR, NN)                                                                                                \
    hipLaunchKernelGGL((spmv_sellmask_kernel<MODE, RR, NN>), dim3(grid), dim3(256), win, ctx->stream, x, y, A->n_rows, A->n_cols, \
                       sw->n_blocks, remap_arg, w, partials, stop, sw->hdr, sw->codes, sw->dict, x_al16 | (bis_opts().spmv_sellwin_nt != 0 ? 2 : 0), \
                       (const int32_t *)sw->blk_base, sw->n_pairs, own, dbg)
#define SM_L2(MODE) do {                                                                                                   \
        if (sw->R == 4 && sw->n_pairs == 27) SM_L3(MODE, 4, 27);                                                           \
        else if (sw->R == 4) SM_L3(MODE, 4, 0);                                                                            \
        else if (sw->R == 2 && sw->n_pairs == 27) SM_L3(MODE, 2, 27);                                                      \
        else if (sw->R == 2) SM_L3(MODE, 2, 0); else SM_L3(MODE, 1, 0); } while (0)
        if (mode == 1) SM_L2(1); else SM_L2(0);
#undef SM_L2
#undef SM_L3
    } else {
#define SW_L4(MODE, DIAG, FMT, RR)                                                                                     \
    hipLaunchKernelGGL((spmv_sellwin_kernel<MODE, DIAG, FMT, RR>), dim3(grid), dim3(256), (FMT == 3 ? win_off3 : (size_t)(SwLayout<DIAG, FMT, RR>::kWinOff)) + win, \
                       ctx->stream, x, y, A->n_rows, A->n_cols, sw->n_blocks, remap_arg, w, partials, stop, sw->hdr,   \
                       sw->slice_chunk0, sw->codes, sw->dict, A->vdiag, x_al16 | (bis_opts().spmv_sellwin_nt != 0 ? 2 : 0), sw->blk_base, sw->pair_stride, sw->n_pairs, sw->diag_pair, own, dbg)
#define SW_L4N(MODE, DIAG, RR, NN)                                                                                      \
    hipLaunchKernelGGL((spmv_sellwin_kernel<MODE, DIAG, 3, RR, NN>), dim3(grid), dim3(256), win_off3 + win,             \
                       ctx->stream, x, y, A->n_rows, A->n_cols, sw->n_blocks, remap_arg, w, partials, stop, sw->hdr,   \
                       sw->slice_chunk0, sw->codes, sw->dict, A->vdiag, x_al16 | (bis_opts().spmv_sellwin_nt != 0 ? 2 : 0), sw->blk_base, sw->pair_stride, sw->n_pairs, sw->diag_pair, own, dbg)
#define SW_L3(MODE, DIAG, FMT) do {                                                                                    \
        if (FMT == 3 && sw->uniform_chunks == 7 && sw->R == 2) SW_L4N(MODE, DIAG, 2, 7);                               \
        else if (FMT == 3 && sw->uniform_chunks == 2 && sw->R == 2) SW_L4N(MODE, DIAG, 2, 2);                          \
        else if (sw->R == 2) SW_L4(MODE, DIAG, FMT, 2); else SW_L4(MODE, DIAG, FMT, 1); } while (0)
#define SW_L2(MODE, DIAG) do { if (sw->fmt == 3) SW_L3(MODE, DIAG, 3); else if (sw->fmt == 2) SW_L3(MODE, DIAG, 2); else if (sw->fmt == 1) SW_L3(MODE, DIAG, 1); else SW_L3(MODE, DIAG, 0); } while (0)
#define SW_L1(MODE) do { if (sw->diag) SW_L2(MODE, true); else SW_L2(MODE, false); } while (0)
    if (mode == 1) SW_L1(1); else SW_L1(0);
#undef SW_L1
#undef SW_L2
#undef SW_L3
#undef SW_L4
#undef SW_L4N
    }
    BIS_HIP_CHECK(ctx, hipGetLastError());
    if (dbg) {
        std::vector<long long> hd((size_t)4 * sw->n_blocks);
        BIS_HIP_CHECK(ctx, hipMemcpyAsync(hd.data(), dbg, sizeof(long long) * hd.size(), hipMemcpyDeviceToHost, ctx->stream));
        BIS_HIP_CHECK(ctx, hipStreamSynchronize(ctx->stream));
        if (FILE *f = fopen(dbg_file, "w")) {
            for (int b = 0; b < sw->n_blocks; ++b) fprintf(f, "%lld %lld %lld %lld\n", hd[4 * b], hd[4 * b + 1], hd[4 * b + 2], hd[4 * b + 3]);
            fclose(f);
        }
    }
    return BIS_OK;
}

namespace {

constexpr int kW8ChunkBytes = 2560;
constexpr int kW8ValBytes = 2048;
template <typename VT> constexpr int w8_chunk_bytes() { return 512 + 256 * (int)sizeof(VT); }
template <typename VT> constexpr int w8_val_bytes() { return 256 * (int)sizeof(VT); }
static_assert(w8_chunk_bytes<double>() == kW8ChunkBytes && w8_val_bytes<double>() == kW8ValBytes, "the 8-byte stream's chunk sizes");
inline size_t w8_chunk_bytes(int vb) { return 512 + 256 * (size_t)vb; }
inline size_t w8_val_bytes(int vb) { return 256 * (size_t)vb; }

constexpr int kW8Runs = 64;
constexpr int kW8GapMerge = 4;

template <typename RP>
__global__ __launch_bounds__(256) void w8_plan_kernel(const RP *__restrict__ row_ptr, const int32_t *__restrict__ col, int64_t n_rows, int R,
                                                      int max_gran, int64_t row0, int32_t *__restrict__ hdr, int32_t *__restrict__ slice_chunks,
                                                      int32_t *__restrict__ own_rank, uint16_t *__restrict__ row_of, int *status) {
    __shared__ int table[kSwHash];
    __shared__ int list[1024];
    __shared__ int keys[1024];
    __shared__ int cnt, failed, n_out, win_gran, own_s, ident;
    __shared__ int out_g0[kW8Runs], out_rk[kW8Runs];
    const int b = blockIdx.x, tid = threadIdx.x;
    const int64_t r0 = (int64_t)b * kSwRows * R;
    const int rows = (int)min((int64_t)kSwRows * R, n_rows - r0);
    const int cap = kSwRows * R;
    for (int i = tid; i < kSwHash; i += 256) table[i] = -1;
    if (tid == 0) { cnt = 0; failed = 0; n_out = 0; win_gran = 0; own_s = -1; ident = 1; }
    __syncthreads();
    for (int i = tid; i < 1024; i += 256) {
        int len = -1;
        if (i < rows) len = (int)((int64_t)row_ptr[r0 + i + 1] - (int64_t)row_ptr[r0 + i]);
        keys[i] = i < cap ? ((min(len, (1 << 20) - 1) + 1) << 10 | (1023 - i)) : -1;
    }
    __syncthreads();
    for (int k = 2; k <= 1024; k <<= 1)
        for (int j = k >> 1; j > 0; j >>= 1) {
            for (int i = tid; i < 1024; i += 256) {
                const int o = i ^ j;
                if (o > i) {
                    const int a = keys[i], c = keys[o];
                    if ((a < c) == ((i & k) == 0)) { keys[i] = c; keys[o] = a; }
                }
            }
            __syncthreads();
        }
    for (int i = tid; i < cap; i += 256) {
        const int row = 1023 - (keys[i] & 1023);
        row_of[(size_t)b * cap + i] = (uint16_t)row;
        if (row != i) atomicExch(&ident, 0);
        if ((i & 63) == 0) {
            const int len = (keys[i] >> 10) - 1;
            const int ch = len > 0 ? (len + 3) >> 2 : 0;
            slice_chunks[(size_t)b * 4 * R + (i >> 6)] = ch;
            atomicMax(&status[5], ch);
        }
    }
    const int64_t s = (int64_t)row_ptr[r0], e = (int64_t)row_ptr[r0 + rows];
    for (int64_t k = s + tid; k < e; k += 256) {
        if (__hip_atomic_load(&failed, __ATOMIC_RELAXED, __HIP_MEMORY_SCOPE_WORKGROUP)) break;
        const int g = col[k] >> 3;
        unsigned h = ((unsigned)g * 2654435761u) >> 20;
        for (;;) {
            const int cur = __hip_atomic_load(&table[h], __ATOMIC_RELAXED, __HIP_MEMORY_SCOPE_WORKGROUP);
            if (cur == g) break;
            if (cur == -1) {
                const int old = atomicCAS(&table[h], -1, g);
                if (old == -1) {
                    if (atomicAdd(&cnt, 1) >= max_gran) atomicExch(&failed, 1);
                    break;
                }
                if (old == g) break;
            }
            h = (h + 1) & (kSwHash - 1);
        }
    }
    __syncthreads();
    const int n = cnt;
    if (failed || n > max_gran) {
        if (tid == 0) atomicExch(&status[0], 1);
        return;
    }
    __syncthreads();
    if (tid == 0) cnt = 0;
    __syncthreads();
    for (int i = tid; i < kSwHash; i += 256) {
        const int g = table[i];
        if (g != -1) list[atomicAdd(&cnt, 1)] = g;
    }
    int P = 2;
    while (P < n) P <<= 1;
    __syncthreads();
    for (int i = n + tid; i < P; i += 256) list[i] = INT32_MAX;
    __syncthreads();
    for (int k = 2; k <= P; k <<= 1)
        for (int j = k >> 1; j > 0; j >>= 1) {
            for (int i = tid; i < P; i += 256) {
                const int o = i ^ j;
                if (o > i) {
                    const int a = list[i], c = list[o];
                    if ((a > c) == ((i & k) == 0)) { list[i] = c; list[o] = a; }
                }
            }
            __syncthreads();
        }
    if (tid == 0) {
        int m = 0, rank = 0;
        int i = 0;
        bool ok = true;
        const int64_t c_first = r0 + row0, c_last = c_first + rows - 1;
        const int g_first = (int)(c_first >> 3), g_last = (int)(c_last >> 3);
        int own = -1;
        while (i < n && ok) {
            const int g0 = list[i];
            int g1 = g0;
            ++i;
            while (i < n && list[i] - g1 <= kW8GapMerge + 1) { g1 = list[i]; ++i; }
            const int len = g1 - g0 + 1;
            if ((c_first & 7) == 0 && g0 <= g_first && g_last <= g1) own = rank + (g_first - g0);
            for (int o = 0; o < len && ok; o += kSwRunGran) {
                if (m >= kW8Runs) { ok = false; break; }
                out_g0[m] = g0 + o;
                out_rk[m] = (rank + o) | (min(kSwRunGran, len - o) << 16);
                ++m;
            }
            rank += len;
            if (rank > max_gran) ok = false;
        }
        if (!ok) atomicExch(&failed, 1);
        n_out = m;
        win_gran = rank;
        own_s = own;
    }
    __syncthreads();
    if (failed) {
        if (tid == 0) atomicExch(&status[0], 1);
        return;
    }
    if (tid < 2 * kW8Runs) {
        const int k = tid % kW8Runs;
        int word = 0;
        if (k < n_out) word = tid < kW8Runs ? out_g0[k] : out_rk[k];
        hdr[(size_t)b * 2 * kW8Runs + tid] = word;
    }
    if (tid == 0) {
        own_rank[b] = ident ? own_s : -1;
        atomicMax(&status[1], win_gran);
        atomicAdd(reinterpret_cast<unsigned *>(&status[2]), (unsigned)win_gran);
    }
}

template <typename RP, int PHASE, typename VT = double>
__global__ __launch_bounds__(256) void w8_fill_kernel(const RP *__restrict__ row_ptr, const int32_t *__restrict__ col, const double *__restrict__ val,
                                                      int64_t n_rows, int R, const int32_t *__restrict__ hdr,
                                                      const int64_t *__restrict__ slice_chunk0, const uint16_t *__restrict__ row_of,
                                                      unsigned char *__restrict__ stream, int64_t *__restrict__ slice_rec,
                                                      uint2 *__restrict__ desc, unsigned char *__restrict__ side) {
    __shared__ int g0s[kW8Runs], rk[kW8Runs];
    __shared__ int nr_s;
    const int b = blockIdx.x, tid = threadIdx.x, lane = tid & 63, wv = tid >> 6;
    if (tid < kW8Runs) {
        g0s[tid] = hdr[(size_t)b * 2 * kW8Runs + tid];
        const int w2 = hdr[(size_t)b * 2 * kW8Runs + kW8Runs + tid];
        rk[tid] = w2 & 0xffff;
        const unsigned long long m = __ballot((w2 >> 16) != 0);
        if (tid == 0) nr_s = __popcll(m);
    }
    __syncthreads();
    const int nr = nr_s;
    for (int rr = 0; rr < R; ++rr) {
        const int64_t slice = ((int64_t)b * 4 + wv) * R + rr;
        const int64_t pos = slice * 64 + lane;
        const int in_block = row_of[pos];
        const int64_t r = (int64_t)b * kSwRows * R + in_block;
        int64_t rs = 0;
        int len = 0;
        if (r < n_rows) {
            rs = (int64_t)row_ptr[r];
            len = (int)((int64_t)row_ptr[r + 1] - rs);
        }
        const int64_t c0 = slice_chunk0[slice];
        const int nch = (int)(slice_chunk0[slice + 1] - c0);
        bool implicit = false;
        if (PHASE == 1) implicit = __ballot(r < n_rows && len == __builtin_amdgcn_readfirstlane(len)) == ~0ull;
        if (PHASE == 2) implicit = slice_rec[slice + 1] == slice_rec[slice];
        for (int c = 0; c < nch && (PHASE != 1 || implicit); ++c) {
            unsigned cc[4];
            double vv[4];
#pragma unroll
            for (int q = 0; q < 4; ++q) {
                const int j = 4 * c + q;
                cc[q] = 0;
                vv[q] = 1.0;
                if (j < len) {
                    const int ci = col[rs + j];
                    const int g = ci >> 3;
                    int lo = 0, hi = nr - 1;
                    while (lo < hi) {
                        const int mid = (lo + hi + 1) >> 1;
                        if (g0s[mid] <= g) lo = mid; else hi = mid - 1;
                    }
                    cc[q] = (unsigned)(2 + (rk[lo] + (g - g0s[lo])) * 8 + (ci & 7)) * 8u;
                    if (PHASE != 1) vv[q] = val[rs + j];
                }
            }
            unsigned base[4];
#pragma unroll
            for (int q = 0; q < 4; ++q) base[q] = 4 * c + q < len ? (cc[q] - 8u * (unsigned)in_block) & 0xffffu : 1u;
            if (PHASE == 1) {
#pragma unroll
                for (int q = 0; q < 4; ++q)
                    if (__ballot(base[q] != (unsigned)__builtin_amdgcn_readfirstlane((int)base[q])) != 0ull) implicit = false;
            } else if (PHASE == 0) {
                unsigned char *p = stream + (size_t)(c0 + c) * w8_chunk_bytes<VT>();
                *reinterpret_cast<uint2 *>(p + lane * 8) = make_uint2(cc[0] | cc[1] << 16, cc[2] | cc[3] << 16);
                if constexpr (sizeof(VT) == 4) {
                    *reinterpret_cast<float4 *>(p + 512 + lane * 16) = make_float4((float)vv[0], (float)vv[1], (float)vv[2], (float)vv[3]);
                } else {
                    *reinterpret_cast<double2 *>(p + 512 + lane * 16) = make_double2(vv[0], vv[1]);
                    *reinterpret_cast<double2 *>(p + 1536 + lane * 16) = make_double2(vv[2], vv[3]);
                }
            } else {
                unsigned char *p = stream + (size_t)(c0 + c) * w8_val_bytes<VT>();
                if constexpr (sizeof(VT) == 4) {
                    *reinterpret_cast<float4 *>(p + lane * 16) = make_float4((float)vv[0], (float)vv[1], (float)vv[2], (float)vv[3]);
                } else {
                    *reinterpret_cast<double2 *>(p + lane * 16) = make_double2(vv[0], vv[1]);
                    *reinterpret_cast<double2 *>(p + 1024 + lane * 16) = make_double2(vv[2], vv[3]);
                }
                if (!implicit) *reinterpret_cast<uint2 *>(side + (size_t)(slice_rec[slice] + c) * 512 + lane * 8) = make_uint2(cc[0] | cc[1] << 16, cc[2] | cc[3] << 16);
                else if (lane == 0) desc[c0 + c] = make_uint2(base[0] | base[1] << 16, base[2] | base[3] << 16);
            }
        }
        if (PHASE == 1 && lane == 0) slice_rec[slice] = implicit ? 0 : nch;
    }
}

typedef double w8_v2d __attribute__((ext_vector_type(2)));
typedef unsigned w8_v2u __attribute__((ext_vector_type(2)));
typedef float w8_v4f __attribute__((ext_vector_type(4)));
template <typename VT> struct W8Chunk { w8_v2u code; w8_v2d v0, v1; };
template <> struct W8Chunk<float> { w8_v2u code; w8_v4f v; };

template <typename VT>
__device__ __forceinline__ W8Chunk<VT> w8_load(const unsigned char *__restrict__ stream, int64_t c, int lane) {
    const unsigned char *p = stream + (size_t)c * w8_chunk_bytes<VT>();
    W8Chunk<VT> ch;
    ch.code = __builtin_nontemporal_load(reinterpret_cast<const w8_v2u *>(p + lane * 8));
    if constexpr (sizeof(VT) == 4) {
        ch.v = __builtin_nontemporal_load(reinterpret_cast<const w8_v4f *>(p + 512 + lane * 16));
    } else {
        ch.v0 = __builtin_nontemporal_load(reinterpret_cast<const w8_v2d *>(p + 512 + lane * 16));
        ch.v1 = __builtin_nontemporal_load(reinterpret_cast<const w8_v2d *>(p + 1536 + lane * 16));
    }
    return ch;
}

template <typename VT>
__device__ __forceinline__ void w8_load_values(const unsigned char *__restrict__ stream, int64_t c, int lane, W8Chunk<VT> &ch) {
    const unsigned char *p = stream + (size_t)c * w8_val_bytes<VT>();
    if constexpr (sizeof(VT) == 4) {
        ch.v = __builtin_nontemporal_load(reinterpret_cast<const w8_v4f *>(p + lane * 16));
    } else {
        ch.v0 = __builtin_nontemporal_load(reinterpret_cast<const w8_v2d *>(p + lane * 16));
        ch.v1 = __builtin_nontemporal_load(reinterpret_cast<const w8_v2d *>(p + 1024 + lane * 16));
    }
}

typedef unsigned short w8_v2h __attribute__((ext_vector_type(2)));
__device__ __forceinline__ unsigned w8_imply(unsigned code, unsigned off2) {
    const unsigned pad = (code & 0x10001u) * 0xffffu;
    return __builtin_bit_cast(unsigned, __builtin_bit_cast(w8_v2h, code) + __builtin_bit_cast(w8_v2h, off2)) & ~pad;
}

__device__ __forceinline__ void w8_consume(const unsigned char *win, const W8Chunk<double> &ch, double &acc) {
#pragma clang fp contract(off)
    const double x0 = *reinterpret_cast<const double *>(win + (ch.code.x & 0xffffu));
    const double x1 = *reinterpret_cast<const double *>(win + (ch.code.x >> 16));
    const double x2 = *reinterpret_cast<const double *>(win + (ch.code.y & 0xffffu));
    const double x3 = *reinterpret_cast<const double *>(win + (ch.code.y >> 16));
    const double p0 = ch.v0.x * x0, p1 = ch.v0.y * x1, p2 = ch.v1.x * x2, p3 = ch.v1.y * x3;
    acc = acc + p0;
    acc = acc + p1;
    acc = acc + p2;
    acc = acc + p3;
}
__device__ __forceinline__ void w8_consume(const unsigned char *win, const W8Chunk<float> &ch, double &acc) {
#pragma clang fp contract(off)
    const double x0 = *reinterpret_cast<const double *>(win + (ch.code.x & 0xffffu));
    const double x1 = *reinterpret_cast<const double *>(win + (ch.code.x >> 16));
    const double x2 = *reinterpret_cast<const double *>(win + (ch.code.y & 0xffffu));
    const double x3 = *reinterpret_cast<const double *>(win + (ch.code.y >> 16));
    const double p0 = (double)ch.v.x * x0, p1 = (double)ch.v.y * x1, p2 = (double)ch.v.z * x2, p3 = (double)ch.v.w * x3;
    acc = acc + p0;
    acc = acc + p1;
    acc = acc + p2;
    acc = acc + p3;
}

template <int MODE, int R, int D, bool IMPL, typename VT = double, bool TWO = false>
__global__ __launch_bounds__(256) void spmv_win8_kernel(
    const double *x, double *__restrict__ y, int64_t n_rows, int64_t n_cols, int n_blocks, int remap_arg, const double *w,
    double *__restrict__ partials, const int *stop, const int32_t *__restrict__ hdr, const int64_t *__restrict__ slice_chunk0,
    const unsigned char *__restrict__ stream, int x_al16, const int32_t *__restrict__ own_rank, const uint16_t *__restrict__ row_of,
    const w8_v2u *__restrict__ desc, const unsigned char *__restrict__ side, const int64_t *__restrict__ slice_rec) {
    if (stop && stop[1]) return;
    extern __shared__ __attribute__((aligned(16))) unsigned char lds[];
    const int b = remap_arg > 0 ? xcd_remap(blockIdx.x, remap_arg)
                                : (remap_arg < -1 ? xcd_group_remap(blockIdx.x, -remap_arg) : (int)blockIdx.x);
    if (b >= n_blocks) return;
    const int tid = threadIdx.x, lane = tid & 63;
    const int wv = __builtin_amdgcn_readfirstlane(tid >> 6);
    const int hw_g = hdr[(size_t)b * 2 * kW8Runs + lane], hw_r = hdr[(size_t)b * 2 * kW8Runs + kW8Runs + lane];
    const int64_t slice0 = ((int64_t)b * 4 + wv) * R;
    const int64_t block_row0 = (int64_t)b * kSwRows * R;
    int64_t rows_of[R];
#pragma unroll
    for (int r = 0; r < R; ++r) rows_of[r] = block_row0 + row_of[(slice0 + r) * 64 + lane];
    const int64_t my_bnd = slice_chunk0[slice0 + min(lane, R)];
    auto bnd = [&](int r) {
        const unsigned lo = (unsigned)__builtin_amdgcn_readlane((int)(unsigned)(unsigned long long)my_bnd, r);
        const unsigned hi = (unsigned)__builtin_amdgcn_readlane((int)(unsigned)((unsigned long long)my_bnd >> 32), r);
        return (int64_t)(((unsigned long long)hi << 32) | lo);
    };
    const int64_t C0 = bnd(0), C1 = bnd(R);
    const int64_t c_last = max(C1 - 1, C0);
    int64_t e[R];
#pragma unroll
    for (int rr = 0; rr < R; ++rr) e[rr] = bnd(rr + 1);
    int64_t rec[R + 1];
    unsigned off2[R];
    if (IMPL) {
        const int64_t my_rec = slice_rec[slice0 + min(lane, R)];
#pragma unroll
        for (int r = 0; r <= R; ++r) {
            const unsigned lo = (unsigned)__builtin_amdgcn_readlane((int)(unsigned)(unsigned long long)my_rec, r);
            const unsigned hi = (unsigned)__builtin_amdgcn_readlane((int)(unsigned)((unsigned long long)my_rec >> 32), r);
            rec[r] = (int64_t)(((unsigned long long)hi << 32) | lo);
        }
#pragma unroll
        for (int r = 0; r < R; ++r) off2[r] = rec[r + 1] == rec[r] ? (unsigned)(rows_of[r] - block_row0) * 0x80008u : 0u;
    }
    auto load = [&](int64_t cc) {
        if (!IMPL) return w8_load<VT>(stream, cc, lane);
        W8Chunk<VT> ch;
        w8_load_values<VT>(stream, cc, lane, ch);
        int64_t rs = 0, re = 0, cs = 0;
#pragma unroll
        for (int rr = 0; rr < R; ++rr)
            if (cc >= (rr ? e[rr - 1] : C0) && cc < e[rr]) { rs = rec[rr]; re = rec[rr + 1]; cs = rr ? e[rr - 1] : C0; }
        if (re > rs) ch.code = __builtin_nontemporal_load(reinterpret_cast<const w8_v2u *>(side + (size_t)(rs + cc - cs) * 512 + lane * 8));
        else ch.code = desc[cc];
        return ch;
    };
    W8Chunk<VT> ring[D];
#pragma unroll
    for (int d = 0; d < D; ++d) ring[d] = load(min(C0 + d, c_last));
    double wr[R];
    int own = -1;
    if (MODE == 1 && own_rank) own = own_rank[b];
#pragma unroll
    for (int r = 0; r < R; ++r) {
        const int64_t row = rows_of[r];
        wr[r] = (MODE == 1 && own < 0 && row < n_rows) ? w[row] : 0.0;
    }
    if (tid == 0) *reinterpret_cast<double *>(lds) = -0.0;
    {
        const int n_runs = __popcll(__ballot((hw_r >> 16) != 0));
        unsigned char *win = lds + 16;
        for (int k = 0; k < n_runs; ++k) {
            const int g0 = __builtin_amdgcn_readlane(hw_g, k);
            const int w2 = __builtin_amdgcn_readlane(hw_r, k);
            const int rank = w2 & 0xffff, n_pieces = (w2 >> 16) * 4;
            const int j = (wv + k) & 3;
            const int p = j * 64 + lane;
            const int64_t c = (int64_t)g0 * 8 + 2 * p;
            unsigned char *dst = win + (size_t)rank * 64 + (size_t)j * 1024;
            if (p < n_pieces) {
                if (x_al16 && c + 1 < n_cols) {
                    __builtin_amdgcn_global_load_lds((const __attribute__((address_space(1))) void *)(x + c),
                                                     (__attribute__((address_space(3))) void *)dst, 16, 0, 0);
                } else {
                    double2 v;
                    v.x = c < n_cols ? x[c] : 0.0;
                    v.y = c + 1 < n_cols ? x[c + 1] : 0.0;
                    *reinterpret_cast<double2 *>(dst + lane * 16) = v;
                }
            }
        }
    }
    __syncthreads();
    if (MODE == 1 && own >= 0) {
#pragma unroll
        for (int r = 0; r < R; ++r) wr[r] = *reinterpret_cast<const double *>(lds + 16 + ((size_t)own * 8 + (wv * R + r) * 64 + lane) * 8);
    }
    double dot_acc = 0.0;
    int64_t c = C0;
    int next = 0;
    double acc = 0.0;
    unsigned cur_off = IMPL ? off2[0] : 0u;
#define W8_END_SLICES()                                                                    \
    _Pragma("unroll") for (int rr = 0; rr < R; ++rr)                                       \
        if (rr == next && c == e[rr]) {                                                    \
            const int64_t row = rows_of[rr];                                               \
            if (row < n_rows) y[row] = acc;                                                \
            if (MODE == 1) dot_acc += row < n_rows ? acc * wr[rr] : 0.0;                   \
            acc = 0.0;                                                                     \
            ++next;                                                                        \
            if (IMPL) cur_off = off2[rr + 1 < R ? rr + 1 : R - 1];                         \
        }
    W8_END_SLICES()
#define W8_STEP(FROM, INTO)                                                                \
    {                                                                                      \
        W8Chunk<VT> cur = FROM;                                                            \
        INTO = load(min(c + D, c_last));                                                   \
        if (IMPL) {                                                                        \
            cur.code.x = w8_imply(cur.code.x, cur_off);                                    \
            cur.code.y = w8_imply(cur.code.y, cur_off);                                    \
        }                                                                                  \
        w8_consume(lds, cur, acc);                                                         \
        ++c;                                                                               \
        W8_END_SLICES()                                                                    \
    }
#define W8_TAIL(FROM)                                                                      \
    _Pragma("unroll") for (int d = 0; d < D - 1; ++d)                                      \
        if (c < C1) {                                                                      \
            W8Chunk<VT> cur = FROM[d];                                                     \
            if (IMPL) {                                                                    \
                cur.code.x = w8_imply(cur.code.x, cur_off);                                \
                cur.code.y = w8_imply(cur.code.y, cur_off);                                \
            }                                                                              \
            w8_consume(lds, cur, acc);                                                     \
            ++c;                                                                           \
            W8_END_SLICES()                                                                \
        }
    if constexpr (TWO) {
        W8Chunk<VT> ring2[D];
        while (c + 2 * D <= C1) {
#pragma unroll
            for (int d = 0; d < D; ++d) W8_STEP(ring[d], ring2[d])
#pragma unroll
            for (int d = 0; d < D; ++d) W8_STEP(ring2[d], ring[d])
        }
        if (c + D <= C1) {
#pragma unroll
            for (int d = 0; d < D; ++d) W8_STEP(ring[d], ring2[d])
            W8_TAIL(ring2)
        } else {
            W8_TAIL(ring)
        }
    } else {
        while (c < C1) {
#pragma unroll
            for (int d = 0; d < D; ++d) {
                if (c < C1) W8_STEP(ring[d], ring[d])
            }
        }
    }
#undef W8_TAIL
#undef W8_STEP
#undef W8_END_SLICES
    if (MODE == 1) {
        const double t = wave_sum(dot_acc);
        if (lane == 0) partials[(size_t)b * 4 + wv] = t;
    }
}

}

static inline bis_sellwin *&w8_ptr(bis_mat *A, int vb) { return vb == 4 ? A->sw4 : A->sw8; }
static inline int &w8_state(bis_mat *A, int vb) { return vb == 4 ? A->sw4_state : A->sw8_state; }
static inline const bis_sellwin *w8_get(const bis_mat *A, int vb) {
    return (vb == 4 ? A->sw4_state : A->sw8_state) == 1 ? (vb == 4 ? A->sw4 : A->sw8) : nullptr;
}

static void w8_drop_one(bis_mat *A, int vb) {
    if (bis_sellwin *&sw = w8_ptr(A, vb)) {
        if (sw->own_codes) sw->codes = reinterpret_cast<uint32_t *>(sw->own_codes);
        hipFree(sw->hdr); hipFree(sw->slice_chunk0); hipFree(sw->own_rank); hipFree(sw->codes); hipFree(sw->row_of);
        hipFree(sw->slice_rec);
        delete sw;
        sw = nullptr;
    }
    w8_state(A, vb) = 0;
}

void bis_spmv_win8_drop(bis_mat *A) {
    w8_drop_one(A, 8);
    w8_drop_one(A, 4);
}

int bis_spmv_win8_active(const bis_mat *A) {
    return A->f32_exact && A->sw4_state == 1 && bis_opts().spmv_win4 != 0 && bis_opts().spmv_win8 != 0 ? 4 : 8;
}

int bis_spmv_win8_blocks(const bis_mat *A, int vb) { const bis_sellwin *sw = w8_get(A, vb); return sw ? sw->n_blocks : 0; }
int bis_spmv_win8_rows(const bis_mat *A, int vb) { const bis_sellwin *sw = w8_get(A, vb); return sw ? sw->R : 0; }
bool bis_spmv_win8_implied(const bis_mat *A, int vb) { const bis_sellwin *sw = w8_get(A, vb); return sw && sw->slice_rec != nullptr; }
int64_t bis_spmv_win8_bytes(const bis_mat *A, int vb) {
    const bis_sellwin *sw = w8_get(A, vb);
    if (!sw) return 0;
    const int64_t meta = (int64_t)sw->n_blocks * (8 * kW8Runs + 2 * kSwRows * sw->R) + 8 * (sw->n_slices + 1);
    if (!sw->slice_rec) return sw->total_chunks * (int64_t)w8_chunk_bytes(vb) + meta;
    return sw->total_chunks * (int64_t)w8_val_bytes(vb) + 8 * (sw->total_chunks - sw->expl_chunks) + 512 * sw->expl_chunks + meta + 8 * (sw->n_slices + 1);
}

size_t bis_spmv_win8_stream_bytes(const bis_mat *A, int vb) {
    const bis_sellwin *sw = w8_get(A, vb);
    if (!sw) return 0;
    return sw->slice_rec ? sw->w8_end : w8_chunk_bytes(vb) * (size_t)(sw->total_chunks + 1);
}

double bis_spmv_win8_moved_bytes(const bis_mat *A, int vb) {
    const bis_sellwin *sw = w8_get(A, vb);
    if (!sw) return 0.0;
    return (double)bis_spmv_win8_bytes(A, vb) + 64.0 * (double)sw->win_gran_sum + 8.0 * (double)A->n_rows;
}
bool bis_spmv_win8_fast(const bis_mat *A, double ms, int vb) {
    return w8_get(A, vb) && ms > 0.0 && bis_spmv_win8_moved_bytes(A, vb) / (ms * 1e-3) >= 6.85e12;
}
void *bis_spmv_win8_swap_stream(bis_mat *A, void *stream, int vb) {
    bis_sellwin *sw = w8_ptr(A, vb);
    void *old = sw->codes;
    sw->codes = reinterpret_cast<uint32_t *>(stream);
    return old;
}

#define W8_CHECK(call)                                                         \
    do {                                                                       \
        hipError_t e_ = (call);                                                \
        if (e_ != hipSuccess) {                                                \
            (void)hipGetLastError();                                           \
            hipFree(slice_chunks); hipFree(tmp);                               \
            w8_drop_one(A, vb);                                                \
            w8_state(A, vb) = -1;                                              \
            if (e_ == hipErrorOutOfMemory) return BIS_OK;  \
            ctx->err = std::string(#call) + ": " + hipGetErrorString(e_);      \
            return BIS_ERR_HIP;                                                \
        }                                                                      \
    } while (0)

static bis_status w8_tune_placement(bis_ctx *ctx, bis_mat *A, int vb) {
    bis_sellwin *sw = w8_ptr(A, vb);
    const size_t bytes = bis_spmv_win8_stream_bytes(A, vb);
    const int k = bis_opts().spmv_win8_tune >= 0 ? bis_opts().spmv_win8_tune : ((size_t)kW8ChunkBytes * (size_t)(sw->total_chunks + 1) >= ((size_t)1 << 30) ? 12 : 0);
    if (k <= 0) return BIS_OK;
    double *x = nullptr, *y = nullptr, *part = nullptr;
    hipEvent_t e0 = nullptr, e1 = nullptr;
    std::vector<void *> losers;
    auto cleanup = [&]() {
        hipStreamSynchronize(ctx->stream);
        for (void *l : losers) hipFree(l);
        hipFree(x); hipFree(y); hipFree(part);
        if (e0) hipEventDestroy(e0);
        if (e1) hipEventDestroy(e1);
        (void)hipGetLastError();
    };
    const size_t nx = (size_t)std::max(A->n_cols, A->view_row0 + A->n_rows) + 2;
    if (hipMalloc(&x, sizeof(double) * nx) != hipSuccess || hipMalloc(&y, sizeof(double) * (size_t)A->n_rows) != hipSuccess ||
        hipMalloc(&part, sizeof(double) * 4 * (size_t)sw->n_blocks) != hipSuccess ||
        hipMemsetAsync(x, 0, sizeof(double) * nx, ctx->stream) != hipSuccess ||
        hipEventCreate(&e0) != hipSuccess || hipEventCreate(&e1) != hipSuccess) { cleanup(); return BIS_OK; }
    const int nb = sw->n_blocks, remap_arg = bis_spmv_remap_arg(nb), grid = bis_spmv_grid(nb);
    const bool implied = bis_spmv_win8_implied(A, vb);
    const int mode = implied ? 1 : 0;
    const double *w = implied ? x + A->view_row0 : nullptr;
    double *partials = implied ? part : nullptr;
    auto measure = [&](double &ms) -> bool {
        for (int i = 0; i < 2; ++i) if (bis_spmv_win8_launch(ctx, A, x, y, mode, w, partials, nullptr, remap_arg, grid, vb) != BIS_OK) return false;
        hipEventRecord(e0, ctx->stream);
        for (int i = 0; i < 5; ++i) if (bis_spmv_win8_launch(ctx, A, x, y, mode, w, partials, nullptr, remap_arg, grid, vb) != BIS_OK) return false;
        hipEventRecord(e1, ctx->stream);
        if (hipEventSynchronize(e1) != hipSuccess) return false;
        float f = 0.f;
        hipEventElapsedTime(&f, e0, e1);
        ms = f / 5.0;
        return true;
    };
    double best = 0.0;
    if (!measure(best)) { cleanup(); ctx->err = "win8 placement tuning: launch failed"; return BIS_ERR_HIP; }
    sw->tune_first_ms = best;
    double slowest = best;
    auto fast_enough = [&](double ms) { return bis_spmv_win8_fast(A, ms, vb) || (!implied && ms <= 0.92 * slowest); };
    int trials = 0;
    for (; trials < k && !fast_enough(best); ++trials) {
        size_t free_b = 0, total_b = 0;
        if (hipMemGetInfo(&free_b, &total_b) != hipSuccess || free_b < bytes + ((size_t)8 << 30)) break;
        void *cand = nullptr;
        if (hipMalloc(&cand, bytes) != hipSuccess) { (void)hipGetLastError(); break; }
        void *cur = bis_spmv_win8_swap_stream(A, cand, vb);
        hipMemcpyAsync(cand, cur, bytes, hipMemcpyDeviceToDevice, ctx->stream);
        double ms = 0.0;
        if (!measure(ms)) { bis_spmv_win8_swap_stream(A, cur, vb); losers.push_back(cand); cleanup(); ctx->err = "win8 placement tuning: launch failed"; return BIS_ERR_HIP; }
        slowest = std::max(slowest, ms);
        if (ms < best) { best = ms; losers.push_back(cur); }
        else { bis_spmv_win8_swap_stream(A, cur, vb); losers.push_back(cand); }
    }
    sw->tune_trials = trials;
    sw->tune_kept_ms = best;
    if (getenv("BIS_WIN8_STATS")) fprintf(stderr, "win8 placement: %d re-allocation(s) of %zu bytes tried, kernel %.4f ms on the first allocation, %.4f ms on the one kept (%.0f bytes moved: %.2f TB/s)\n", trials, bytes, sw->tune_first_ms, best, bis_spmv_win8_moved_bytes(A, vb), bis_spmv_win8_moved_bytes(A, vb) / (best * 1e9));
    cleanup();
    return BIS_OK;
}

extern "C" BIS_API bis_status bis_mat_win8_debug_stream(bis_mat *A, void **ptr, size_t *bytes, void *set) {
    const int vb = A ? bis_spmv_win8_active(A) : 8;
    if (!A || !w8_get(A, vb)) return BIS_ERR_INVALID;
    bis_sellwin *sw = w8_ptr(A, vb);
    if (ptr) *ptr = sw->own_codes ? sw->own_codes : (void *)sw->codes;
    if (bytes) *bytes = bis_spmv_win8_stream_bytes(A, vb);
    if (set) { if (!sw->own_codes) sw->own_codes = (void *)sw->codes; sw->codes = reinterpret_cast<uint32_t *>(set); }
    else if (sw->own_codes) { sw->codes = reinterpret_cast<uint32_t *>(sw->own_codes); sw->own_codes = nullptr; }
    return BIS_OK;
}

extern "C" BIS_API void bis_mat_win8_layout(const bis_mat *A, int64_t *chunks, int64_t *explicit_chunks, int64_t *slices, int *blocks, int *implied) {
    const bis_sellwin *sw = A ? w8_get(A, bis_spmv_win8_active(A)) : nullptr;
    if (chunks) *chunks = sw ? sw->total_chunks : 0;
    if (explicit_chunks) *explicit_chunks = sw ? sw->expl_chunks : 0;
    if (slices) *slices = sw ? sw->n_slices : 0;
    if (blocks) *blocks = sw ? sw->n_blocks : 0;
    if (implied) *implied = sw && sw->slice_rec != nullptr;
}

extern "C" BIS_API void bis_mat_win8_tuning(const bis_mat *A, int *trials, double *first_ms, double *kept_ms) {
    const bis_sellwin *sw = A ? w8_get(A, bis_spmv_win8_active(A)) : nullptr;
    if (trials) *trials = sw ? sw->tune_trials : 0;
    if (first_ms) *first_ms = sw ? sw->tune_first_ms : 0.0;
    if (kept_ms) *kept_ms = sw ? sw->tune_kept_ms : 0.0;
}

static bis_status w8_try_rows(bis_ctx *ctx, bis_mat *A, int R, bool *window_too_large, int vb);

bis_status bis_spmv_win8_try(bis_ctx *ctx, bis_mat *A, int vb) {
    if (w8_state(A, vb) != 0) return BIS_OK;
    w8_state(A, vb) = -1;
    if (A->n_rows == 0 || A->nnz == 0 || A->n_cols >= ((int64_t)1 << 31) - 16) return BIS_OK;
    int R = bis_opts().spmv_win8_rows > 0 ? std::min(bis_opts().spmv_win8_rows, 4) : 4;
    if (R == 3) R = 2;
    while (R > 1 && A->n_rows < (int64_t)kSwRows * R * 1024) R >>= 1;
    for (;; R >>= 1) {
        bool too_large = false;
        if (bis_status st = w8_try_rows(ctx, A, R, &too_large, vb)) return st;
        if (w8_state(A, vb) == 1 || !too_large || R == 1 || bis_opts().spmv_win8_rows > 0) return BIS_OK;
        w8_state(A, vb) = -1;
    }
}

static bis_status w8_try_rows(bis_ctx *ctx, bis_mat *A, int R, bool *window_too_large, int vb) {
    *window_too_large = false;
    const int64_t nb64 = (A->n_rows + (int64_t)kSwRows * R - 1) / ((int64_t)kSwRows * R);
    if (nb64 > (int64_t)1 << 26) return BIS_OK;
    const int nb = (int)nb64;
    bis_sellwin *sw = new bis_sellwin;
    w8_ptr(A, vb) = sw;
    sw->n_blocks = nb;
    sw->R = R;
    sw->vb = vb;
    sw->n_slices = (int64_t)nb * 4 * R;
    sw->fmt = 5;
    int32_t *slice_chunks = nullptr;
    void *tmp = nullptr;
    int *status = (int *)ctx->counters + 52;
    W8_CHECK(hipMalloc(&sw->hdr, sizeof(int32_t) * 2 * kW8Runs * (size_t)nb));
    W8_CHECK(hipMalloc(&sw->own_rank, sizeof(int32_t) * (size_t)nb));
    W8_CHECK(hipMemsetAsync(sw->own_rank, 0xFF, sizeof(int32_t) * (size_t)nb, ctx->stream));
    W8_CHECK(hipMalloc(&sw->row_of, sizeof(uint16_t) * (size_t)nb * kSwRows * (size_t)R));
    W8_CHECK(hipMalloc(&slice_chunks, sizeof(int32_t) * (size_t)(sw->n_slices + 1)));
    W8_CHECK(hipMalloc(&sw->slice_chunk0, sizeof(int64_t) * (size_t)(sw->n_slices + 1)));
    W8_CHECK(hipMemsetAsync(status, 0, 3 * sizeof(int), ctx->stream));
    W8_CHECK(hipMemsetAsync(status + 5, 0, sizeof(int), ctx->stream));
    W8_CHECK(hipMemsetAsync(slice_chunks, 0, sizeof(int32_t) * (size_t)(sw->n_slices + 1), ctx->stream));
    W8_CHECK(hipMemsetAsync(sw->hdr, 0, sizeof(int32_t) * 2 * kW8Runs * (size_t)nb, ctx->stream));
    if (A->rp64) hipLaunchKernelGGL(w8_plan_kernel<int64_t>, dim3(nb), dim3(256), 0, ctx->stream, (const int64_t *)A->row_ptr, A->col, A->n_rows, R, kSwMaxGran, A->view_row0, sw->hdr, slice_chunks, sw->own_rank, sw->row_of, status);
    else hipLaunchKernelGGL(w8_plan_kernel<int32_t>, dim3(nb), dim3(256), 0, ctx->stream, (const int32_t *)A->row_ptr, A->col, A->n_rows, R, kSwMaxGran, A->view_row0, sw->hdr, slice_chunks, sw->own_rank, sw->row_of, status);
    W8_CHECK(hipGetLastError());
    int h[3] = {0, 0, 0};
    W8_CHECK(hipMemcpyAsync(h, status, sizeof h, hipMemcpyDeviceToHost, ctx->stream));
    const int64_t ns1 = sw->n_slices + 1;
    hipLaunchKernelGGL(sw_widen_kernel, dim3((unsigned)((ns1 + 255) / 256)), dim3(256), 0, ctx->stream, slice_chunks, sw->slice_chunk0, ns1);
    W8_CHECK(hipGetLastError());
    size_t tmp_bytes = 0;
    W8_CHECK(rocprim::exclusive_scan(nullptr, tmp_bytes, sw->slice_chunk0, sw->slice_chunk0, (int64_t)0, (size_t)ns1, rocprim::plus<int64_t>(), ctx->stream));
    W8_CHECK(hipMalloc(&tmp, tmp_bytes));
    W8_CHECK(rocprim::exclusive_scan(tmp, tmp_bytes, sw->slice_chunk0, sw->slice_chunk0, (int64_t)0, (size_t)ns1, rocprim::plus<int64_t>(), ctx->stream));
    int64_t total = 0;
    W8_CHECK(hipMemcpyAsync(&total, sw->slice_chunk0 + sw->n_slices, sizeof total, hipMemcpyDeviceToHost, ctx->stream));
    W8_CHECK(hipStreamSynchronize(ctx->stream));
    hipFree(tmp); tmp = nullptr;
    hipFree(slice_chunks); slice_chunks = nullptr;
    sw->total_chunks = total;
    sw->max_gran = h[1];
    sw->win_gran_sum = (int64_t)(unsigned)h[2];
    if (h[0] || (double)total * 256.0 > 1.12 * (double)A->nnz + 256.0 * 4 * 64) {
        if (getenv("BIS_WIN8_STATS")) fprintf(stderr, "win8 plan (R = %d): %s, %.1f %% padding: not used\n", R, h[0] ? "window not representable" : "representable", 100.0 * ((double)total * 256.0 / (double)A->nnz - 1.0));
        *window_too_large = h[0] != 0;
        w8_drop_one(A, vb);
        w8_state(A, vb) = -1;
        return BIS_OK;
    }
#define W8_FILL(PHASE, VT, STREAM, DESC, SIDE)                                                                                                    \
    do {                                                                                                                                          \
        if (A->rp64) hipLaunchKernelGGL((w8_fill_kernel<int64_t, PHASE, VT>), dim3(nb), dim3(256), 0, ctx->stream, (const int64_t *)A->row_ptr, A->col, \
                                        A->val, A->n_rows, R, sw->hdr, sw->slice_chunk0, sw->row_of, STREAM, sw->slice_rec, DESC, SIDE);           \
        else hipLaunchKernelGGL((w8_fill_kernel<int32_t, PHASE, VT>), dim3(nb), dim3(256), 0, ctx->stream, (const int32_t *)A->row_ptr, A->col, \
                                A->val, A->n_rows, R, sw->hdr, sw->slice_chunk0, sw->row_of, STREAM, sw->slice_rec, DESC, SIDE);                   \
        W8_CHECK(hipGetLastError());                                                                                                              \
    } while (0)
    sw->expl_chunks = total;
    if (bis_opts().spmv_win8_implicit != 0 && total > 0) {
        W8_CHECK(hipMalloc(&sw->slice_rec, sizeof(int64_t) * (size_t)ns1));
        W8_CHECK(hipMemsetAsync(sw->slice_rec, 0, sizeof(int64_t) * (size_t)ns1, ctx->stream));
        W8_FILL(1, double, nullptr, nullptr, nullptr);
        tmp_bytes = 0;
        W8_CHECK(rocprim::exclusive_scan(nullptr, tmp_bytes, sw->slice_rec, sw->slice_rec, (int64_t)0, (size_t)ns1, rocprim::plus<int64_t>(), ctx->stream));
        W8_CHECK(hipMalloc(&tmp, tmp_bytes));
        W8_CHECK(rocprim::exclusive_scan(tmp, tmp_bytes, sw->slice_rec, sw->slice_rec, (int64_t)0, (size_t)ns1, rocprim::plus<int64_t>(), ctx->stream));
        int64_t expl = 0;
        W8_CHECK(hipMemcpyAsync(&expl, sw->slice_rec + sw->n_slices, sizeof expl, hipMemcpyDeviceToHost, ctx->stream));
        W8_CHECK(hipStreamSynchronize(ctx->stream));
        hipFree(tmp); tmp = nullptr;
        if (2 * (total - expl) >= total) sw->expl_chunks = expl;
        else { hipFree(sw->slice_rec); sw->slice_rec = nullptr; }
    }
    unsigned char *stream = nullptr;
    const size_t chunk_bytes = sw->slice_rec ? w8_val_bytes(vb) : w8_chunk_bytes(vb);
    size_t stream_bytes = chunk_bytes * (size_t)(total + 1);
    if (sw->slice_rec) {
        sw->w8_desc = stream_bytes;
        sw->w8_side = sw->w8_desc + ((8 * (size_t)(total + 1) + 255) & ~(size_t)255);
        sw->w8_end = stream_bytes = sw->w8_side + 512 * (size_t)sw->expl_chunks;
    }
    W8_CHECK(hipMalloc(&stream, stream_bytes));
    sw->codes = reinterpret_cast<uint32_t *>(stream);
    W8_CHECK(hipMemsetAsync(stream + (size_t)total * chunk_bytes, 0, chunk_bytes, ctx->stream));
    if (sw->slice_rec) {
        W8_CHECK(hipMemsetAsync(stream + sw->w8_desc, 0, sw->w8_side - sw->w8_desc, ctx->stream));
        if (vb == 4) W8_FILL(2, float, stream, reinterpret_cast<uint2 *>(stream + sw->w8_desc), stream + sw->w8_side);
        else W8_FILL(2, double, stream, reinterpret_cast<uint2 *>(stream + sw->w8_desc), stream + sw->w8_side);
    } else {
        if (vb == 4) W8_FILL(0, float, stream, nullptr, nullptr);
        else W8_FILL(0, double, stream, nullptr, nullptr);
    }
#undef W8_FILL
    w8_state(A, vb) = 1;
    if (bis_status tst = w8_tune_placement(ctx, A, vb)) return tst;
    if (getenv("BIS_WIN8_STATS")) fprintf(stderr, "win%d plan (R = %d): %d blocks, window <= %d granules (%zu bytes), %.1f %% padding: used; implied slots: %s, %.1f %% of %lld chunks implicit; stream at %p (%zu bytes), hdr %p\n", vb, R, nb, sw->max_gran, (size_t)(2 + 8 * sw->max_gran) * 8, 100.0 * ((double)total * 256.0 / (double)A->nnz - 1.0), sw->slice_rec ? "built" : "not built", 100.0 * (double)(total - sw->expl_chunks) / (double)std::max<int64_t>(total, 1), (long long)total, (void *)sw->codes, bis_spmv_win8_stream_bytes(A, vb), (void *)sw->hdr);
    return BIS_OK;
}
#undef W8_CHECK

bis_status bis_spmv_win8_launch(bis_ctx *ctx, const bis_mat *A, const double *x, double *y, int mode, const double *w,
                                double *partials, const int *stop, int remap_arg, int grid, int vb) {
    const bis_sellwin *sw = vb == 4 ? A->sw4 : A->sw8;
    const int x_al16 = ((uintptr_t)x & 15) == 0;
    const size_t lds = (size_t)(2 + 8 * sw->max_gran) * 8;
    const unsigned char *stream = reinterpret_cast<const unsigned char *>(sw->codes);
    const int32_t *own = (mode == 1 && w == x + A->view_row0 && x_al16) ? sw->own_rank : nullptr;
    const bool ragged = (double)sw->total_chunks * 256.0 > 1.08 * (double)A->nnz;
    const bool two = bis_opts().spmv_win8_sets > 0 ? bis_opts().spmv_win8_sets >= 2 : true;
    const int depth = bis_opts().spmv_win8_depth > 0 ? bis_opts().spmv_win8_depth
                      : two ? (sw->R == 1 ? 2 : 3) : (sw->R == 4 ? (ragged ? 2 : 1) : 3);
#define W8_L3(MODE, RR, DD) do { if (sw->slice_rec) W8_L5(MODE, RR, DD, true); else W8_L5(MODE, RR, DD, false); } while (0)
#define W8_L5(MODE, RR, DD, IMPL) do { if (vb == 4) W8_L6(MODE, RR, DD, IMPL, float); else W8_L6(MODE, RR, DD, IMPL, double); } while (0)
#define W8_L6(MODE, RR, DD, IMPL, VT) do { if (two && DD <= 4) W8_L4(MODE, RR, DD, IMPL, VT, (DD <= 4)); else W8_L4(MODE, RR, DD, IMPL, VT, false); } while (0)
#define W8_L4(MODE, RR, DD, IMPL, VT, TWO) hipLaunchKernelGGL((spmv_win8_kernel<MODE, RR, DD, IMPL, VT, TWO>), dim3(grid), dim3(256), lds, ctx->stream, x, y, A->n_rows, A->n_cols, \
                                               sw->n_blocks, remap_arg, w, partials, stop, sw->hdr, sw->slice_chunk0, stream, x_al16, own, sw->row_of, \
                                               reinterpret_cast<const w8_v2u *>(stream + sw->w8_desc), stream + sw->w8_side, sw->slice_rec)
#define W8_L2(MODE, RR) do { if (depth <= 1) W8_L3(MODE, RR, 1); else if (depth == 2) W8_L3(MODE, RR, 2); else if (depth == 3) W8_L3(MODE, RR, 3); else if (depth <= 5) W8_L3(MODE, RR, 4); else W8_L3(MODE, RR, 6); } while (0)
#define W8_L1(MODE) do { if (sw->R == 4) W8_L2(MODE, 4); else if (sw->R == 2) W8_L2(MODE, 2); else W8_L2(MODE, 1); } while (0)
    if (mode == 1) W8_L1(1); else W8_L1(0);
#undef W8_L1
#undef W8_L2
#undef W8_L3
#undef W8_L4
#undef W8_L5
#undef W8_L6
    BIS_HIP_CHECK(ctx, hipGetLastError());
    return BIS_OK;
}
```

include/bis_hip.h:

```cpp
#ifndef BIS_HIP_H
#define BIS_HIP_H

#include <stddef.h>
#include <stdint.h>

#ifdef __cplusplus
extern "C" {
#endif

#define BIS_API __attribute__((visibility("default")))

typedef int bis_status;
enum {
    BIS_OK = 0,
    BIS_ERR_NO_DEVICE = 1,
    BIS_ERR_INVALID = 2,
    BIS_ERR_HIP = 3,
    BIS_ERR_ZERO_DIAG = 4,
    BIS_ERR_NO_DIAG = 5,
    BIS_ERR_UNSUPPORTED = 6,
    BIS_ERR_COMM = 7,
    BIS_ERR_SYNC = 8
};

enum {
    BIS_PC_NONE = 0,
    BIS_PC_JACOBI = 1,
    BIS_PC_GAUSS_SEIDEL = 2,
    BIS_PC_BACKWARDS_GAUSS_SEIDEL = 3,
    BIS_PC_SYMMETRIC_GAUSS_SEIDEL = 4,
    BIS_PC_TWO_STAGE_GS = 5,
    BIS_PC_SYMMETRIC_TWO_STAGE_GS = 6,
    BIS_PC_ILU0 = 7,
    BIS_PC_ILU0_ITER = 8,
    BIS_PC_FSAI = 9,
    BIS_PC_MG = 10,
    BIS_PC_BLOCK_JACOBI = 11
};

typedef struct bis_ctx bis_ctx;
typedef struct bis_mat bis_mat;

BIS_API bis_status bis_ctx_create(int device, void *stream, bis_ctx **out);
BIS_API bis_status bis_ctx_destroy(bis_ctx *ctx);
BIS_API const char *bis_last_error(const bis_ctx *ctx);
BIS_API bis_status bis_sync(bis_ctx *ctx);
BIS_API void *bis_ctx_stream(bis_ctx *ctx);
BIS_API bis_status bis_device_info(bis_ctx *ctx, char *arch, size_t arch_len,
                                   int *n_cus, int64_t *hbm_bytes);
BIS_API bis_status bis_set_option(const char *name, int value);
BIS_API int bis_options_describe(char *buf, int cap);
BIS_API int bis_abi_version(void);

BIS_API bis_status bis_vec_alloc(bis_ctx *ctx, int64_t n, double **out);
BIS_API bis_status bis_vec_free(bis_ctx *ctx, double *v);
BIS_API bis_status bis_vec_upload(bis_ctx *ctx, double *dst_dev,
                                  const double *src_host, int64_t n);
BIS_API bis_status bis_vec_download(bis_ctx *ctx, double *dst_host,
                                    const double *src_dev, int64_t n);

BIS_API bis_status bis_mat_create(bis_ctx *ctx, int64_t n_rows, int64_t n_cols,
                                  int64_t nnz, const int32_t *row_ptr,
                                  const int32_t *col, const double *val,
                                  bis_mat **out);
BIS_API bis_status bis_mat_create64(bis_ctx *ctx, int64_t n_rows,
                                    int64_t n_cols, int64_t nnz,
                                    const int64_t *row_ptr, const int32_t *col,
                                    const double *val, bis_mat **out);
BIS_API bis_status bis_mat_destroy(bis_ctx *ctx, bis_mat *A);
BIS_API bis_status bis_mat_info(const bis_mat *A, int64_t *n_rows,
                                int64_t *n_cols, int64_t *nnz);
BIS_API int bis_mat_rp_width(const bis_mat *A);
BIS_API bis_status bis_mat_spmv_stream_info(bis_ctx *ctx, const bis_mat *A,
                                            int *col_bytes, int *val_bytes,
                                            int *n_dict, int *form);
BIS_API bis_status bis_mat_spmv_streamed_bytes(bis_ctx *ctx, const bis_mat *A,
                                               int64_t *bytes);
BIS_API bis_status bis_mat_set_grid_hint(bis_mat *A, int64_t nx, int64_t ny,
                                         int64_t nz, int dof);
BIS_API bis_status bis_mat_grid_hint(const bis_mat *A, int64_t hint[4]);
BIS_API bis_status bis_mat_retune(bis_ctx *ctx, bis_mat *A);
BIS_API void bis_mat_win8_tuning(const bis_mat *A, int *trials, double *first_ms, double *kept_ms);
BIS_API void bis_mat_win8_layout(const bis_mat *A, int64_t *chunks, int64_t *explicit_chunks, int64_t *slices, int *blocks, int *implied);
BIS_API void bis_mat_colslab_info(const bis_mat *A, int *slabs, double *one_pass_ms, double *slab_passes_ms);
BIS_API bis_status bis_mat_win8_debug_stream(bis_mat *A, void **ptr, size_t *bytes, void *set);
BIS_API bis_status bis_mat_tune_placement(bis_ctx *ctx, bis_mat *A, int max_trials,
                                          double *first_ms, double *best_ms);
BIS_API bis_status bis_mat_debug_ptrs(const bis_mat *A, void **row_ptr,
                                      void **col, void **val);
BIS_API bis_status bis_mat_download(bis_ctx *ctx, const bis_mat *A,
                                    int64_t *row_ptr, int32_t *col,
                                    double *val);

BIS_API bis_status bis_mat_gen_hpcg(bis_ctx *ctx, int64_t nx, int64_t ny,
                                    int64_t nz, int64_t row0, int64_t row1,
                                    bis_mat **out);
BIS_API bis_status bis_mat_gen_anderson(bis_ctx *ctx, int64_t L, double t,
                                        double W, double shift, uint64_t seed,
                                        int64_t row0, int64_t row1,
                                        bis_mat **out);

BIS_API bis_status bis_mat_gen_fem(bis_ctx *ctx, int64_t nx, int64_t ny,
                                   int64_t nz, int keep_percent, uint64_t seed,
                                   int64_t row0, int64_t row1, bis_mat **out);

BIS_API bis_status bis_mat_gen_unstr(bis_ctx *ctx, int64_t nx, int64_t ny,
                                     int64_t nz, int keep_percent, uint64_t seed,
                                     int32_t *perm_dev_out, bis_mat **out);

BIS_API bis_status bis_mat_split_strict(bis_ctx *ctx, const bis_mat *A,
                                        bis_mat **L_strict, bis_mat **U_strict,
                                        double *D, double *D_inv);

BIS_API bis_status bis_mat_scale_sym(bis_ctx *ctx, bis_mat *A, double *scale);

BIS_API bis_status bis_mat_round_f32(bis_ctx *ctx, bis_mat *A, double *max_rel_change);

BIS_API bis_status bis_mat_multicolour(bis_ctx *ctx, const bis_mat *A,
                                       bis_mat **B, int32_t *perm_dev,
                                       int *n_colours);
BIS_API bis_status bis_vec_gather(bis_ctx *ctx, double *out, const double *in,
                                  const int32_t *perm_dev, int64_t n);
BIS_API bis_status bis_mat_bfs_order(bis_ctx *ctx, const bis_mat *A, int rcm,
                                     int32_t *perm_dev);
BIS_API bis_status bis_mat_permute(bis_ctx *ctx, const bis_mat *A,
                                   const int32_t *perm_dev, bis_mat **B);
BIS_API bis_status bis_vec_scatter(bis_ctx *ctx, double *out, const double *in,
                                   const int32_t *perm_dev, int64_t n);

BIS_API bis_status bis_mat_ilu0(bis_ctx *ctx, const bis_mat *A, double pivot_tol,
                                double pivot_repl, bis_mat **L_strict,
                                bis_mat **U_strict, double *L_D, double *U_D);
BIS_API const char *bis_mat_ilu0_kernel(const bis_mat *L_strict);

BIS_API bis_status bis_mat_iluk_symbolic(bis_ctx *ctx, const bis_mat *A, int level, bis_mat **P, int64_t *n_fill);
BIS_API bis_status bis_mat_iluk(bis_ctx *ctx, const bis_mat *A, int level, double pivot_tol, double pivot_repl,
                                bis_mat **L_strict, bis_mat **U_strict, double *L_D, double *U_D, int64_t *n_fill);
BIS_API const char *bis_mat_iluk_kernel(const bis_mat *L_strict);
BIS_API bis_status bis_iluk_limits(int *max_level, int *max_visit);

BIS_API bis_status bis_mat_fsai(bis_ctx *ctx, const bis_mat *A, bis_mat **G, bis_mat **Gt, int64_t *n_fallback_rows);
BIS_API const char *bis_mat_fsai_kernel(const bis_mat *G);

BIS_API bis_status bis_spgemm(bis_ctx *ctx, const bis_mat *A, const bis_mat *B, bis_mat **C);
BIS_API bis_status bis_mat_transpose(bis_ctx *ctx, const bis_mat *A, bis_mat **At);
BIS_API const char *bis_spgemm_kernel(const bis_mat *C);
BIS_API bis_status bis_spgemm_limits(int *wave_cap, int *row_cap, int *row_cap_max, int64_t *batch);

typedef struct bis_mg bis_mg;
typedef struct {
    int max_levels;
    int64_t coarse_limit;
    int coarsening;
    int nu;
    int coarse_sweeps;
    double omega;
    double coarse_scale;
} bis_mg_params;
BIS_API bis_status bis_mg_create(bis_ctx *ctx, const bis_mat *A, const bis_mg_params *params, bis_mg **out);
BIS_API bis_status bis_mg_destroy(bis_ctx *ctx, bis_mg *mg);
BIS_API bis_status bis_mg_apply(bis_ctx *ctx, const bis_mg *mg, double *out, const double *in);
enum { BIS_MG_CYCLE_V = 0, BIS_MG_CYCLE_W = 1, BIS_MG_CYCLE_K = 2, BIS_MG_CYCLE_K_GCR = 3 };
BIS_API bis_status bis_mg_set_cycle(bis_ctx *ctx, bis_mg *mg, int cycle, int cycle_levels);
BIS_API bis_status bis_mg_cycle(const bis_mg *mg, int *cycle, int *cycle_levels);
BIS_API const bis_mat *bis_mg_operand(const bis_mg *mg);
BIS_API bis_status bis_mg_info(const bis_mg *mg, int *levels, int64_t *rows, int64_t *nnz, int *kind);
BIS_API const bis_mat *bis_mg_level_matrix(const bis_mg *mg, int level);
BIS_API bis_status bis_mg_level_aggregates(bis_ctx *ctx, const bis_mg *mg, int level, int32_t *host);
BIS_API bis_status bis_mg_level_weights(bis_ctx *ctx, const bis_mg *mg, int level, double *host);
BIS_API bis_status bis_mg_create_smoothed(bis_ctx *ctx, const bis_mat *A, const bis_mg_params *params, double prolong_omega, bis_mg **out);
BIS_API const bis_mat *bis_mg_level_prolongator(const bis_mg *mg, int level);
BIS_API const bis_mat *bis_mg_level_restrictor(const bis_mg *mg, int level);
BIS_API bis_status bis_mg_level_prolong_omega(const bis_mg *mg, int level, double *omega_l);
enum { BIS_MG_SMOOTH_JACOBI = 0, BIS_MG_SMOOTH_CHEBYSHEV = 1 };
typedef struct {
    int kind;
    int degree;
    double ratio;
    int est_steps;
    double safety;
} bis_mg_smoother;
BIS_API bis_status bis_mg_set_smoother(bis_ctx *ctx, bis_mg *mg, const bis_mg_smoother *smoother);
BIS_API bis_status bis_mg_smoother_info(const bis_mg *mg, bis_mg_smoother *out);
BIS_API bis_status bis_mg_level_spectrum(const bis_mg *mg, int level, double *bound, double *estimate, double *lambda_max,
                                         double *lambda_min);
BIS_API bis_status bis_mg_level_cheb_coeffs(const bis_mg *mg, int level, double *c1, double *c2);

typedef struct bis_bj bis_bj;
typedef struct {
    int block_size;
    const int32_t *block_ptr;
    int64_t n_blocks;
    int symmetrize;
} bis_bj_params;
BIS_API bis_status bis_bj_create(bis_ctx *ctx, const bis_mat *A, const bis_bj_params *params, bis_bj **out);
BIS_API bis_status bis_bj_destroy(bis_ctx *ctx, bis_bj *bj);
BIS_API bis_status bis_bj_apply(bis_ctx *ctx, const bis_bj *bj, double *out, const double *in);
BIS_API bis_status bis_bj_mapply(bis_ctx *ctx, const bis_bj *bj, double *OUT, const double *IN, int n_rhs);
BIS_API const bis_mat *bis_bj_operand(const bis_bj *bj);
BIS_API bis_status bis_bj_info(const bis_bj *bj, int64_t *n_blocks, int *max_block, int64_t *value_count);
BIS_API bis_status bis_bj_blocks(bis_ctx *ctx, const bis_bj *bj, double *host_values, int64_t *host_offsets);

BIS_API bis_status bis_spmv(bis_ctx *ctx, const bis_mat *A, const double *x,
                            double *y);
BIS_API bis_status bis_spmm(bis_ctx *ctx, const bis_mat *A, const double *X, double *Y, int n_rhs);
BIS_API const char *bis_mat_spmm_kernel(const bis_mat *A);
BIS_API bis_status bis_mat_spmm_streamed_bytes(const bis_mat *A, int n_rhs, int64_t *bytes);
BIS_API bis_status bis_mvec_set_col(bis_ctx *ctx, double *X, int64_t n, int n_rhs, int j, const double *v);
BIS_API bis_status bis_mvec_get_col(bis_ctx *ctx, double *v, const double *X, int64_t n, int n_rhs, int j);

BIS_API bis_status bis_sptrsv(bis_ctx *ctx, const bis_mat *L_strict, double *x,
                              const double *D, const double *b);
BIS_API bis_status bis_bsptrsv(bis_ctx *ctx, const bis_mat *U_strict,
                               double *x, const double *D, const double *b);
BIS_API bis_status bis_subtract_vectors(bis_ctx *ctx, double *r,
                                        const double *a, const double *b,
                                        int64_t n, double scale);
BIS_API bis_status bis_sum_vectors(bis_ctx *ctx, double *r, const double *a,
                                   const double *b, int64_t n, double scale);
BIS_API bis_status bis_elemwise_mult_vectors(bis_ctx *ctx, double *r,
                                             const double *a, const double *b,
                                             int64_t n, double scale);
BIS_API bis_status bis_elemwise_div_vectors(bis_ctx *ctx, double *r,
                                            const double *a, const double *b,
                                            int64_t n, double scale);
BIS_API bis_status bis_compute_residual(bis_ctx *ctx, const bis_mat *A,
                                        const double *x, const double *b,
                                        double *res, double *tmp);
BIS_API bis_status bis_euclidean_vec_norm(bis_ctx *ctx, const double *v,
                                          int64_t n, double *result_host);
BIS_API bis_status bis_dot(bis_ctx *ctx, const double *a, const double *b,
                           int64_t n, double *result_host);
BIS_API bis_status bis_dot_dev(bis_ctx *ctx, const double *a, const double *b,
                               int64_t n, double *result_dev);
BIS_API bis_status bis_sumsq_dev(bis_ctx *ctx, const double *v, int64_t n,
                                 double *result_dev);
BIS_API bis_status bis_axpy_dot_dev(bis_ctx *ctx, double *w, const double *u,
                                    const double *scale_dev, const double *v,
                                    int64_t n, double *result_dev);
BIS_API bis_status bis_subtract_vectors_dev(bis_ctx *ctx, double *r, const double *a,
                                            const double *b, int64_t n,
                                            const double *scale_dev);
BIS_API bis_status bis_sum_vectors_dev(bis_ctx *ctx, double *r, const double *a,
                                       const double *b, int64_t n,
                                       const double *scale_dev);
BIS_API bis_status bis_scale_dev(bis_ctx *ctx, double *r, const double *v,
                                 const double *scalar_dev, int64_t n);
BIS_API bis_status bis_scalar_div(bis_ctx *ctx, double *out_dev, const double *a_dev,
                                  const double *b_dev);
BIS_API bis_status bis_scalar_ratio_product(bis_ctx *ctx, double *out_dev,
                                            const double *a_dev, const double *b_dev,
                                            const double *c_dev, const double *d_dev);
BIS_API bis_status bis_scalar_sqrt_inv(bis_ctx *ctx, double *norm_dev, double *inv_dev,
                                       const double *sumsq_dev);
BIS_API bis_status bis_scale(bis_ctx *ctx, double *r, const double *v,
                             double scalar, int64_t n);
BIS_API bis_status bis_init_vector(bis_ctx *ctx, double *v, double val,
                                   int64_t n);
BIS_API bis_status bis_copy_vector(bis_ctx *ctx, double *out, const double *in,
                                   int64_t n);
BIS_API bis_status bis_normalize_x(bis_ctx *ctx, double *x_new,
                                   const double *x_old, const double *D,
                                   const double *b, int64_t n);
BIS_API bis_status bis_multi_axpy(bis_ctx *ctx, const double *V, int64_t ldv,
                                  const double *y_host, int n_vec, double *out,
                                  int64_t n);
BIS_API bis_status bis_two_stage_gauss_seidel(bis_ctx *ctx,
                                              const bis_mat *strict,
                                              double *tmp, double *work,
                                              const double *D_inv,
                                              const double *input,
                                              double *output, int64_t n,
                                              int inner_iters);
BIS_API bis_status bis_itrsv(bis_ctx *ctx, const bis_mat *T_strict, const double *D_inv,
                             const double *b, double *x, double *work, int n_sweeps);
BIS_API const char *bis_itrsv_kernel(const bis_mat *T_strict);
BIS_API bis_status bis_apply_preconditioner(
    bis_ctx *ctx, int precond_type, int64_t n, const bis_mat *L_strict,
    const bis_mat *U_strict, const double *A_D, const double *A_D_inv,
    const double *L_D, const double *U_D, double *output, double *input,
    double *tmp, double *work, int outer_iters, int inner_iters);

BIS_API bis_status bis_sptrsm(bis_ctx *ctx, const bis_mat *L_strict, double *X, const double *D, const double *B, int n_rhs);
BIS_API bis_status bis_bsptrsm(bis_ctx *ctx, const bis_mat *U_strict, double *X, const double *D, const double *B, int n_rhs);
BIS_API const char *bis_mat_sweepm_kernel(const bis_mat *T, int backward);
BIS_API bis_status bis_mvec_div_diag(bis_ctx *ctx, double *R, const double *A, const double *D, int64_t n, int n_rhs);
BIS_API bis_status bis_mvec_mul_diag(bis_ctx *ctx, double *R, const double *A, const double *D, int64_t n, int n_rhs);
BIS_API bis_status bis_mitrsv(bis_ctx *ctx, const bis_mat *T_strict, const double *D_inv, const double *B, double *X,
                              double *WORK, int n_sweeps, int n_rhs);
BIS_API bis_status bis_mapply_preconditioner(
    bis_ctx *ctx, int precond_type, int64_t n, int n_rhs, const bis_mat *L_strict,
    const bis_mat *U_strict, const double *A_D, const double *A_D_inv,
    const double *L_D, const double *U_D, double *OUT, double *IN,
    double *TMP, double *WORK, int outer_iters, int inner_iters);

enum { BIS_KERNEL_SPMV = 0, BIS_KERNEL_SPTRSV = 1 };
BIS_API bis_status bis_register_kernel(bis_ctx *ctx, const char *name, int type);
BIS_API bis_status bis_kernel_register_A(bis_ctx *ctx, const char *name,
                                         const bis_mat *A);
BIS_API bis_status bis_kernel_register_B(bis_ctx *ctx, const char *name,
                                         int64_t size, double *vec);
BIS_API bis_status bis_kernel_register_C(bis_ctx *ctx, const char *name,
                                         int64_t size, double *vec);
BIS_API bis_status bis_kernel_register_D(bis_ctx *ctx, const char *name,
                                         const double *diag);
BIS_API bis_status bis_kernel_set_mat_upper_triang(bis_ctx *ctx,
                                                   const char *name, int flag);
BIS_API bis_status bis_kernel_run(bis_ctx *ctx, const char *name,
                                  int64_t A_offset, int64_t B_offset,
                                  int64_t C_offset);
BIS_API bis_status bis_kernel_swap_operands(bis_ctx *ctx, const char *name);

enum { BIS_STAT_JACOBI = 0, BIS_STAT_GS = 1, BIS_STAT_SGS = 2 };
typedef struct bis_stat bis_stat;
BIS_API bis_status bis_stat_create(bis_ctx *ctx, int kind, const bis_mat *A,
                                   const bis_mat *L_strict, const bis_mat *U_strict,
                                   const double *D, const double *b, double *x,
                                   bis_stat **out);
BIS_API bis_status bis_stat_init(bis_ctx *ctx, bis_stat *s, double tol,
                                 double *r0_norm_host);
BIS_API bis_status bis_stat_iterate(bis_ctx *ctx, bis_stat *s, int n_iters);
BIS_API bis_status bis_stat_status(bis_ctx *ctx, bis_stat *s, int *iters,
                                   int *converged, double *hist_host, int hist_cap);
BIS_API bis_status bis_stat_solution(bis_ctx *ctx, bis_stat *s, double *x_out);
BIS_API bis_status bis_stat_destroy(bis_ctx *ctx, bis_stat *s);

typedef struct bis_cg bis_cg;
BIS_API bis_status bis_cg_create(bis_ctx *ctx, const bis_mat *A,
                                 const double *A_D, const double *b, double *x,
                                 bis_cg **out);
BIS_API bis_status bis_cg_destroy(bis_ctx *ctx, bis_cg *cg);
BIS_API bis_status bis_cg_set_preconditioner(bis_ctx *ctx, bis_cg *cg, int precond_type,
                                             const bis_mat *L_strict, const bis_mat *U_strict,
                                             const double *A_D, const double *A_D_inv,
                                             const double *L_D, const double *U_D,
                                             int outer_iters, int inner_iters);
BIS_API bis_status bis_cg_init(bis_ctx *ctx, bis_cg *cg, double tol,
                               double *r0_norm_host);
BIS_API bis_status bis_cg_iterate(bis_ctx *ctx, bis_cg *cg, int n_iters);
BIS_API bis_status bis_cg_status(bis_ctx *ctx, bis_cg *cg, int *iters,
                                 int *converged, double *hist_host,
                                 int hist_cap);

typedef struct bis_mcg bis_mcg;
BIS_API bis_status bis_mcg_create(bis_ctx *ctx, const bis_mat *A, const double *A_D, const double *B, double *X,
                                  int n_rhs, bis_mcg **out);
BIS_API bis_status bis_mcg_set_preconditioner(bis_ctx *ctx, bis_mcg *m, int precond_type,
                                              const bis_mat *L_strict, const bis_mat *U_strict,
                                              const double *A_D, const double *A_D_inv,
                                              const double *L_D, const double *U_D,
                                              int outer_iters, int inner_iters);
BIS_API bis_status bis_mcg_init(bis_ctx *ctx, bis_mcg *m, double tol, double *r0_norms_host);
BIS_API bis_status bis_mcg_iterate(bis_ctx *ctx, bis_mcg *m, int n_iters);
BIS_API bis_status bis_mcg_status(bis_ctx *ctx, bis_mcg *m, int j, int *iters, int *converged, double *hist_host,
                                  int hist_cap);
BIS_API bis_status bis_mcg_destroy(bis_ctx *ctx, bis_mcg *m);

typedef struct bis_mbicgstab bis_mbicgstab;
BIS_API bis_status bis_mbicgstab_create(bis_ctx *ctx, const bis_mat *A, const double *B, double *X, int n_rhs,
                                        bis_mbicgstab **out);
BIS_API bis_status bis_mbicgstab_set_preconditioner(bis_ctx *ctx, bis_mbicgstab *m, int precond_type,
                                                    const bis_mat *L_strict, const bis_mat *U_strict,
                                                    const double *A_D, const double *A_D_inv,
                                                    const double *L_D, const double *U_D,
                                                    int outer_iters, int inner_iters);
BIS_API bis_status bis_mbicgstab_init(bis_ctx *ctx, bis_mbicgstab *m, double tol, double *r0_norms_host);
BIS_API bis_status bis_mbicgstab_iterate(bis_ctx *ctx, bis_mbicgstab *m, int n_iters);
BIS_API bis_status bis_mbicgstab_status(bis_ctx *ctx, bis_mbicgstab *m, int j, int *iters, int *converged,
                                        double *hist_host, int hist_cap);
BIS_API bis_status bis_mbicgstab_destroy(bis_ctx *ctx, bis_mbicgstab *m);

typedef struct bis_mgmres bis_mgmres;
BIS_API bis_status bis_mgmres_create(bis_ctx *ctx, const bis_mat *A, const double *B, double *X, int n_rhs,
                                     int restart_len, bis_mgmres **out);
BIS_API bis_status bis_mgmres_set_preconditioner(bis_ctx *ctx, bis_mgmres *m, int precond_type,
                                                 const bis_mat *L_strict, const bis_mat *U_strict,
                                                 const double *A_D, const double *A_D_inv,
                                                 const double *L_D, const double *U_D,
                                                 int outer_iters, int inner_iters);
BIS_API bis_status bis_mgmres_init(bis_ctx *ctx, bis_mgmres *m, double tol, double *r0_norms_host);
BIS_API bis_status bis_mgmres_iterate(bis_ctx *ctx, bis_mgmres *m, int n_iters);
BIS_API bis_status bis_mgmres_solution(bis_ctx *ctx, bis_mgmres *m, double *X_out);
BIS_API bis_status bis_mgmres_status(bis_ctx *ctx, bis_mgmres *m, int j, int *iters, int *converged, int *n_hist,
                                     double *hist_host, int hist_cap);
BIS_API bis_status bis_mgmres_destroy(bis_ctx *ctx, bis_mgmres *m);

// ... 114 lines not shown
```

Baseline: 1171.

## Drop padded tail value planes from win8 f64 SpMV stream

Per slice, the last chunk's unused 512-byte value planes (up to two) are left out of the f64 win8 stream. An exclusive scan of the per-slice drop counts gives a skew that shifts later chunk addresses. The kernel gets a TAIL template variant that loads the shortened tail with 8-byte alignment and pads the missing values in registers. This cuts the HBM bytes streamed per SpMV in exchange for extra address arithmetic and per-chunk branching. It is enabled by default when the value stream exceeds 256 MB, or when the option is set.

```diff
diff --git a/basic_iterative_solvers_amd/__init__.py b/basic_iterative_solvers_amd/__init__.py
--- a/basic_iterative_solvers_amd/__init__.py
+++ b/basic_iterative_solvers_amd/__init__.py
@@ -491,6 +491,11 @@
         self.ctx.lib.bis_mat_win8_layout(self.h, C.byref(ch), C.byref(ex), C.byref(sl), C.byref(bl), C.byref(im))
         return ch.value, ex.value, sl.value, bl.value, bool(im.value)
 
+    def win8_tail(self):
+        d, on = C.c_int64(), C.c_int()
+        self.ctx.lib.bis_mat_win8_tail(self.h, C.byref(d), C.byref(on))
+        return d.value, bool(on.value)
+
     def colslab_info(self):
         k, a, b = C.c_int(), C.c_double(), C.c_double()
         self.ctx.lib.bis_mat_colslab_info(self.h, C.byref(k), C.byref(a), C.byref(b))
diff --git a/basic_iterative_solvers_amd/csrc/bis_blas1.hip b/basic_iterative_solvers_amd/csrc/bis_blas1.hip
--- a/basic_iterative_solvers_amd/csrc/bis_blas1.hip
+++ b/basic_iterative_solvers_amd/csrc/bis_blas1.hip
@@ -236,7 +236,7 @@
     return BIS_ERR_SYNC;
 }
 
-#define BIS_OPTIONS_ENV(X) X(spmv_variant) X(spmv_window) X(spmv_chunk) X(spmv_chunk_fused) X(spmv_xcd_remap) X(trsv_grid) X(ilu0_wgs) X(trsv_wave_wgs) X(trsv_trial) X(trsv_one_xcd) X(trsv_host_analysis) X(ilu0_wave) X(spmv_packed) X(spmv_packed32) X(spmv_valdict) X(spmv_sellwin) X(device_share) X(spmv_sellwin_rows) X(spmv_sellwin_joint) X(spmv_sellwin_pairs) X(spmv_sellwin_masks) X(spmv_colslab) X(spmv_win8) X(spmv_win8_rows) X(spmv_win8_depth) X(spmv_win8_sets) X(spmv_win8_implicit) X(spmv_win8_tune) X(spmv_win4) X(grid_autodetect) X(tune_placement) X(force_rp64) X(trsv_tiled) X(trsv_chain) X(trsv_tile_rows) X(trsv_tile_wgs) X(trsv_tile_edge) X(trsv_tile_backoff)
+#define BIS_OPTIONS_ENV(X) X(spmv_variant) X(spmv_window) X(spmv_chunk) X(spmv_chunk_fused) X(spmv_xcd_remap) X(trsv_grid) X(ilu0_wgs) X(trsv_wave_wgs) X(trsv_trial) X(trsv_one_xcd) X(trsv_host_analysis) X(ilu0_wave) X(spmv_packed) X(spmv_packed32) X(spmv_valdict) X(spmv_sellwin) X(device_share) X(spmv_sellwin_rows) X(spmv_sellwin_joint) X(spmv_sellwin_pairs) X(spmv_sellwin_masks) X(spmv_colslab) X(spmv_win8) X(spmv_win8_rows) X(spmv_win8_depth) X(spmv_win8_sets) X(spmv_win8_implicit) X(spmv_win8_tail) X(spmv_win8_tune) X(spmv_win4) X(grid_autodetect) X(tune_placement) X(force_rp64) X(trsv_tiled) X(trsv_chain) X(trsv_tile_rows) X(trsv_tile_wgs) X(trsv_tile_edge) X(trsv_tile_backoff)
 #define BIS_OPTIONS_API(Y) Y(trsv_batch) Y(trsv_wave) Y(ilu0_persistent) Y(trsv_by_pos) Y(spmv_lds_pad) Y(trsv_chain_idle) Y(trsv_chain_pause) Y(trsv_chain_pairs) Y(trsv_chain_prefix) Y(trsv_tile_exp) Y(cg_nt_x) Y(spmv_sellwin_nt) Y(dist_host_plan) Y(trsv_inject_loss) Y(trsv_inject_oom) Y(trsm_form) Y(spgemm_row_cap) Y(spgemm_batch)
 
 namespace {
diff --git a/basic_iterative_solvers_amd/csrc/bis_internal.hpp b/basic_iterative_solvers_amd/csrc/bis_internal.hpp
--- a/basic_iterative_solvers_amd/csrc/bis_internal.hpp
+++ b/basic_iterative_solvers_amd/csrc/bis_internal.hpp
@@ -111,6 +111,7 @@
     int spmv_win8_depth = -1;
     int spmv_win8_sets = -1;
     int spmv_win8_implicit = -1;
+    int spmv_win8_tail = -1;
     int spmv_win8_tune = -1;
     int spmv_win4 = -1;
     int spmv_sellwin_masks = -1;
diff --git a/basic_iterative_solvers_amd/csrc/bis_spmv_sell.hip b/basic_iterative_solvers_amd/csrc/bis_spmv_sell.hip
--- a/basic_iterative_solvers_amd/csrc/bis_spmv_sell.hip
+++ b/basic_iterative_solvers_amd/csrc/bis_spmv_sell.hip
@@ -26,6 +26,8 @@
     void *own_codes = nullptr;
     size_t w8_desc = 0, w8_side = 0, w8_end = 0;
     int64_t *slice_rec = nullptr;
+    int64_t *slice_skew = nullptr;
+    int64_t dropped_planes = 0;
     int64_t expl_chunks = 0;
     int64_t win_gran_sum = 0;
     int tune_trials = 0;
@@ -1130,7 +1132,8 @@
 template <typename RP>
 __global__ __launch_bounds__(256) void w8_plan_kernel(const RP *__restrict__ row_ptr, const int32_t *__restrict__ col, int64_t n_rows, int R,
                                                       int max_gran, int64_t row0, int32_t *__restrict__ hdr, int32_t *__restrict__ slice_chunks,
-                                                      int32_t *__restrict__ own_rank, uint16_t *__restrict__ row_of, int *status) {
+                                                      int32_t *__restrict__ own_rank, uint16_t *__restrict__ row_of, int *status,
+                                                      int32_t *__restrict__ slice_drop) {
     __shared__ int table[kSwHash];
     __shared__ int list[1024];
     __shared__ int keys[1024];
@@ -1168,6 +1171,7 @@
             const int len = (keys[i] >> 10) - 1;
             const int ch = len > 0 ? (len + 3) >> 2 : 0;
             slice_chunks[(size_t)b * 4 * R + (i >> 6)] = ch;
+            if (slice_drop) slice_drop[(size_t)b * 4 * R + (i >> 6)] = len > 0 ? min(3 - ((len - 1) & 3), 2) : 0;
             atomicMax(&status[5], ch);
         }
     }
@@ -1270,7 +1274,8 @@
                                                       int64_t n_rows, int R, const int32_t *__restrict__ hdr,
                                                       const int64_t *__restrict__ slice_chunk0, const uint16_t *__restrict__ row_of,
                                                       unsigned char *__restrict__ stream, int64_t *__restrict__ slice_rec,
-                                                      uint2 *__restrict__ desc, unsigned char *__restrict__ side) {
+                                                      uint2 *__restrict__ desc, unsigned char *__restrict__ side,
+                                                      const int64_t *__restrict__ slice_skew) {
     __shared__ int g0s[kW8Runs], rk[kW8Runs];
     __shared__ int nr_s;
     const int b = blockIdx.x, tid = threadIdx.x, lane = tid & 63, wv = tid >> 6;
@@ -1299,7 +1304,10 @@
         bool implicit = false;
         if (PHASE == 1) implicit = __ballot(r < n_rows && len == __builtin_amdgcn_readfirstlane(len)) == ~0ull;
         if (PHASE == 2) implicit = slice_rec[slice + 1] == slice_rec[slice];
+        const int64_t skew = (PHASE != 1 && sizeof(VT) == 8 && slice_skew) ? slice_skew[slice] : 0;
+        const int tail_drop = (PHASE != 1 && sizeof(VT) == 8 && slice_skew) ? (int)(slice_skew[slice + 1] - skew) : 0;
         for (int c = 0; c < nch && (PHASE != 1 || implicit); ++c) {
+            const int drop = c == nch - 1 ? tail_drop : 0;
             unsigned cc[4];
             double vv[4];
 #pragma unroll
@@ -1327,21 +1335,23 @@
                 for (int q = 0; q < 4; ++q)
                     if (__ballot(base[q] != (unsigned)__builtin_amdgcn_readfirstlane((int)base[q])) != 0ull) implicit = false;
             } else if (PHASE == 0) {
-                unsigned char *p = stream + (size_t)(c0 + c) * w8_chunk_bytes<VT>();
+                unsigned char *p = stream + (size_t)(c0 + c) * w8_chunk_bytes<VT>() - 512 * (size_t)skew;
                 *reinterpret_cast<uint2 *>(p + lane * 8) = make_uint2(cc[0] | cc[1] << 16, cc[2] | cc[3] << 16);
                 if constexpr (sizeof(VT) == 4) {
                     *reinterpret_cast<float4 *>(p + 512 + lane * 16) = make_float4((float)vv[0], (float)vv[1], (float)vv[2], (float)vv[3]);
                 } else {
                     *reinterpret_cast<double2 *>(p + 512 + lane * 16) = make_double2(vv[0], vv[1]);
-                    *reinterpret_cast<double2 *>(p + 1536 + lane * 16) = make_double2(vv[2], vv[3]);
+                    if (drop == 0) *reinterpret_cast<double2 *>(p + 1536 + lane * 16) = make_double2(vv[2], vv[3]);
+                    else if (drop == 1) *reinterpret_cast<double *>(p + 1536 + lane * 8) = vv[2];
                 }
             } else {
-                unsigned char *p = stream + (size_t)(c0 + c) * w8_val_bytes<VT>();
+                unsigned char *p = stream + (size_t)(c0 + c) * w8_val_bytes<VT>() - 512 * (size_t)skew;
                 if constexpr (sizeof(VT) == 4) {
                     *reinterpret_cast<float4 *>(p + lane * 16) = make_float4((float)vv[0], (float)vv[1], (float)vv[2], (float)vv[3]);
                 } else {
                     *reinterpret_cast<double2 *>(p + lane * 16) = make_double2(vv[0], vv[1]);
-                    *reinterpret_cast<double2 *>(p + 1024 + lane * 16) = make_double2(vv[2], vv[3]);
+                    if (drop == 0) *reinterpret_cast<double2 *>(p + 1024 + lane * 16) = make_double2(vv[2], vv[3]);
+                    else if (drop == 1) *reinterpret_cast<double *>(p + 1024 + lane * 8) = vv[2];
                 }
                 if (!implicit) *reinterpret_cast<uint2 *>(side + (size_t)(slice_rec[slice] + c) * 512 + lane * 8) = make_uint2(cc[0] | cc[1] << 16, cc[2] | cc[3] << 16);
                 else if (lane == 0) desc[c0 + c] = make_uint2(base[0] | base[1] << 16, base[2] | base[3] << 16);
@@ -1352,6 +1362,7 @@
 }
 
 typedef double w8_v2d __attribute__((ext_vector_type(2)));
+typedef w8_v2d w8_v2d_al8 __attribute__((aligned(8)));
 typedef unsigned w8_v2u __attribute__((ext_vector_type(2)));
 typedef float w8_v4f __attribute__((ext_vector_type(4)));
 template <typename VT> struct W8Chunk { w8_v2u code; w8_v2d v0, v1; };
@@ -1387,6 +1398,12 @@
     const unsigned pad = (code & 0x10001u) * 0xffffu;
     return __builtin_bit_cast(unsigned, __builtin_bit_cast(w8_v2h, code) + __builtin_bit_cast(w8_v2h, off2)) & ~pad;
 }
+
+__device__ __forceinline__ void w8_pad_tail(W8Chunk<double> &ch, int drop) {
+    if (drop >= 1) ch.v1.y = 1.0;
+    if (drop == 2) ch.v1.x = 1.0;
+}
+__device__ __forceinline__ void w8_pad_tail(W8Chunk<float> &, int) {}
 
 __device__ __forceinline__ void w8_consume(const unsigned char *win, const W8Chunk<double> &ch, double &acc) {
 #pragma clang fp contract(off)
@@ -1413,12 +1430,14 @@
     acc = acc + p3;
 }
 
-template <int MODE, int R, int D, bool IMPL, typename VT = double, bool TWO = false>
+template <int MODE, int R, int D, bool IMPL, typename VT = double, bool TWO = false, bool TAIL = false>
 __global__ __launch_bounds__(256) void spmv_win8_kernel(
     const double *x, double *__restrict__ y, int64_t n_rows, int64_t n_cols, int n_blocks, int remap_arg, const double *w,
     double *__restrict__ partials, const int *stop, const int32_t *__restrict__ hdr, const int64_t *__restrict__ slice_chunk0,
     const unsigned char *__restrict__ stream, int x_al16, const int32_t *__restrict__ own_rank, const uint16_t *__restrict__ row_of,
-    const w8_v2u *__restrict__ desc, const unsigned char *__restrict__ side, const int64_t *__restrict__ slice_rec) {
+    const w8_v2u *__restrict__ desc, const unsigned char *__restrict__ side, const int64_t *__restrict__ slice_rec,
+    const int64_t *__restrict__ slice_skew) {
+    static_assert(!TAIL || sizeof(VT) == 8, "short tails: the 8-byte stream only");
     if (stop && stop[1]) return;
     extern __shared__ __attribute__((aligned(16))) unsigned char lds[];
     const int b = remap_arg > 0 ? xcd_remap(blockIdx.x, remap_arg)
@@ -1456,14 +1475,43 @@
 #pragma unroll
         for (int r = 0; r < R; ++r) off2[r] = rec[r + 1] == rec[r] ? (unsigned)(rows_of[r] - block_row0) * 0x80008u : 0u;
     }
+    int64_t skw[R + 1];
+    int drp[R];
+    if constexpr (TAIL) {
+        const int64_t my_skw = slice_skew[slice0 + min(lane, R)];
+#pragma unroll
+        for (int r = 0; r <= R; ++r) {
+            const unsigned lo = (unsigned)__builtin_amdgcn_readlane((int)(unsigned)(unsigned long long)my_skw, r);
+            const unsigned hi = (unsigned)__builtin_amdgcn_readlane((int)(unsigned)((unsigned long long)my_skw >> 32), r);
+            skw[r] = (int64_t)(((unsigned long long)hi << 32) | lo);
+        }
+#pragma unroll
+        for (int r = 0; r < R; ++r) drp[r] = (int)(skw[r + 1] - skw[r]);
+    }
     auto load = [&](int64_t cc) {
-        if (!IMPL) return w8_load<VT>(stream, cc, lane);
+        if constexpr (!IMPL && !TAIL) return w8_load<VT>(stream, cc, lane);
         W8Chunk<VT> ch;
-        w8_load_values<VT>(stream, cc, lane, ch);
+        if constexpr (!TAIL) w8_load_values<VT>(stream, cc, lane, ch);
         int64_t rs = 0, re = 0, cs = 0;
+        int64_t sk = TAIL ? skw[0] : 0;
+        int drop = 0;
 #pragma unroll
         for (int rr = 0; rr < R; ++rr)
-            if (cc >= (rr ? e[rr - 1] : C0) && cc < e[rr]) { rs = rec[rr]; re = rec[rr + 1]; cs = rr ? e[rr - 1] : C0; }
+            if (cc >= (rr ? e[rr - 1] : C0) && cc < e[rr]) {
+                if (IMPL) { rs = rec[rr]; re = rec[rr + 1]; cs = rr ? e[rr - 1] : C0; }
+                if (TAIL) { sk = skw[rr]; drop = cc == e[rr] - 1 ? drp[rr] : 0; }
+            }
+        if constexpr (TAIL) {
+            const unsigned char *p = stream + (size_t)cc * (IMPL ? kW8ValBytes : kW8ChunkBytes) - 512 * (size_t)sk;
+            if (!IMPL) {
+                ch.code = __builtin_nontemporal_load(reinterpret_cast<const w8_v2u *>(p + lane * 8));
+                p += 512;
+            }
+            ch.v0 = __builtin_nontemporal_load(reinterpret_cast<const w8_v2d *>(p + lane * 16));
+            const unsigned char *q = p + (drop == 2 ? 0 : 1024) + (size_t)((unsigned)lane << (drop == 1 ? 3 : 4));
+            ch.v1 = __builtin_nontemporal_load(reinterpret_cast<const w8_v2d_al8 *>(q));
+            if (!IMPL) return ch;
+        }
         if (re > rs) ch.code = __builtin_nontemporal_load(reinterpret_cast<const w8_v2u *>(side + (size_t)(rs + cc - cs) * 512 + lane * 8));
         else ch.code = desc[cc];
         return ch;
@@ -1514,6 +1562,9 @@
     int next = 0;
     double acc = 0.0;
     unsigned cur_off = IMPL ? off2[0] : 0u;
+    [[maybe_unused]] int64_t cur_end = e[0];
+    [[maybe_unused]] int cur_drop = 0;
+    if constexpr (TAIL) cur_drop = drp[0];
 #define W8_END_SLICES()                                                                    \
     _Pragma("unroll") for (int rr = 0; rr < R; ++rr)                                       \
         if (rr == next && c == e[rr]) {                                                    \
@@ -1523,12 +1574,17 @@
             acc = 0.0;                                                                     \
             ++next;                                                                        \
             if (IMPL) cur_off = off2[rr + 1 < R ? rr + 1 : R - 1];                         \
+            if constexpr (TAIL) {                                                          \
+                cur_end = e[rr + 1 < R ? rr + 1 : R - 1];                                  \
+                cur_drop = drp[rr + 1 < R ? rr + 1 : R - 1];                               \
+            }                                                                              \
         }
     W8_END_SLICES()
 #define W8_STEP(FROM, INTO)                                                                \
     {                                                                                      \
         W8Chunk<VT> cur = FROM;                                                            \
         INTO = load(min(c + D, c_last));                                                   \
+        if constexpr (TAIL) w8_pad_tail(cur, c + 1 == cur_end ? cur_drop : 0);             \
         if (IMPL) {                                                                        \
             cur.code.x = w8_imply(cur.code.x, cur_off);                                    \
             cur.code.y = w8_imply(cur.code.y, cur_off);                                    \
@@ -1541,6 +1597,7 @@
     _Pragma("unroll") for (int d = 0; d < D - 1; ++d)                                      \
         if (c < C1) {                                                                      \
             W8Chunk<VT> cur = FROM[d];                                                     \
+            if constexpr (TAIL) w8_pad_tail(cur, c + 1 == cur_end ? cur_drop : 0);         \
             if (IMPL) {                                                                    \
                 cur.code.x = w8_imply(cur.code.x, cur_off);                                \
                 cur.code.y = w8_imply(cur.code.y, cur_off);                                \
@@ -1593,7 +1650,7 @@
     if (bis_sellwin *&sw = w8_ptr(A, vb)) {
         if (sw->own_codes) sw->codes = reinterpret_cast<uint32_t *>(sw->own_codes);
         hipFree(sw->hdr); hipFree(sw->slice_chunk0); hipFree(sw->own_rank); hipFree(sw->codes); hipFree(sw->row_of);
-        hipFree(sw->slice_rec);
+        hipFree(sw->slice_rec); hipFree(sw->slice_skew);
         delete sw;
         sw = nullptr;
     }
@@ -1615,7 +1672,8 @@
 int64_t bis_spmv_win8_bytes(const bis_mat *A, int vb) {
     const bis_sellwin *sw = w8_get(A, vb);
     if (!sw) return 0;
-    const int64_t meta = (int64_t)sw->n_blocks * (8 * kW8Runs + 2 * kSwRows * sw->R) + 8 * (sw->n_slices + 1);
+    int64_t meta = (int64_t)sw->n_blocks * (8 * kW8Runs + 2 * kSwRows * sw->R) + 8 * (sw->n_slices + 1);
+    if (sw->slice_skew) meta -= 512 * sw->dropped_planes;
     if (!sw->slice_rec) return sw->total_chunks * (int64_t)w8_chunk_bytes(vb) + meta;
     return sw->total_chunks * (int64_t)w8_val_bytes(vb) + 8 * (sw->total_chunks - sw->expl_chunks) + 512 * sw->expl_chunks + meta + 8 * (sw->n_slices + 1);
 }
@@ -1623,7 +1681,7 @@
 size_t bis_spmv_win8_stream_bytes(const bis_mat *A, int vb) {
     const bis_sellwin *sw = w8_get(A, vb);
     if (!sw) return 0;
-    return sw->slice_rec ? sw->w8_end : w8_chunk_bytes(vb) * (size_t)(sw->total_chunks + 1);
+    return sw->slice_rec ? sw->w8_end : w8_chunk_bytes(vb) * (size_t)(sw->total_chunks + 1) - 512 * (size_t)sw->dropped_planes;
 }
 
 double bis_spmv_win8_moved_bytes(const bis_mat *A, int vb) {
@@ -1646,7 +1704,7 @@
         hipError_t e_ = (call);                                                \
         if (e_ != hipSuccess) {                                                \
             (void)hipGetLastError();                                           \
-            hipFree(slice_chunks); hipFree(tmp);                               \
+            hipFree(slice_chunks); hipFree(slice_drop); hipFree(tmp);          \
             w8_drop_one(A, vb);                                                \
             w8_state(A, vb) = -1;                                              \
             if (e_ == hipErrorOutOfMemory) return BIS_OK;  \
@@ -1738,6 +1796,12 @@
     if (implied) *implied = sw && sw->slice_rec != nullptr;
 }
 
+extern "C" BIS_API void bis_mat_win8_tail(const bis_mat *A, int64_t *dropped_planes, int *on) {
+    const bis_sellwin *sw = A ? w8_get(A, bis_spmv_win8_active(A)) : nullptr;
+    if (dropped_planes) *dropped_planes = sw ? sw->dropped_planes : 0;
+    if (on) *on = sw && sw->slice_skew != nullptr;
+}
+
 extern "C" BIS_API void bis_mat_win8_tuning(const bis_mat *A, int *trials, double *first_ms, double *kept_ms) {
     const bis_sellwin *sw = A ? w8_get(A, bis_spmv_win8_active(A)) : nullptr;
     if (trials) *trials = sw ? sw->tune_trials : 0;
@@ -1774,9 +1838,14 @@
     sw->vb = vb;
     sw->n_slices = (int64_t)nb * 4 * R;
     sw->fmt = 5;
-    int32_t *slice_chunks = nullptr;
+    int32_t *slice_chunks = nullptr, *slice_drop = nullptr;
     void *tmp = nullptr;
     int *status = (int *)ctx->counters + 52;
+    const int tail_opt = vb == 8 ? bis_opts().spmv_win8_tail : 0;
+    if (tail_opt != 0) {
+        W8_CHECK(hipMalloc(&slice_drop, sizeof(int32_t) * (size_t)(sw->n_slices + 1)));
+        W8_CHECK(hipMemsetAsync(slice_drop, 0, sizeof(int32_t) * (size_t)(sw->n_slices + 1), ctx->stream));
+    }
     W8_CHECK(hipMalloc(&sw->hdr, sizeof(int32_t) * 2 * kW8Runs * (size_t)nb));
     W8_CHECK(hipMalloc(&sw->own_rank, sizeof(int32_t) * (size_t)nb));
     W8_CHECK(hipMemsetAsync(sw->own_rank, 0xFF, sizeof(int32_t) * (size_t)nb, ctx->stream));
@@ -1787,8 +1856,8 @@
     W8_CHECK(hipMemsetAsync(status + 5, 0, sizeof(int), ctx->stream));
     W8_CHECK(hipMemsetAsync(slice_chunks, 0, sizeof(int32_t) * (size_t)(sw->n_slices + 1), ctx->stream));
     W8_CHECK(hipMemsetAsync(sw->hdr, 0, sizeof(int32_t) * 2 * kW8Runs * (size_t)nb, ctx->stream));
-    if (A->rp64) hipLaunchKernelGGL(w8_plan_kernel<int64_t>, dim3(nb), dim3(256), 0, ctx->stream, (const int64_t *)A->row_ptr, A->col, A->n_rows, R, kSwMaxGran, A->view_row0, sw->hdr, slice_chunks, sw->own_rank, sw->row_of, status);
-    else hipLaunchKernelGGL(w8_plan_kernel<int32_t>, dim3(nb), dim3(256), 0, ctx->stream, (const int32_t *)A->row_ptr, A->col, A->n_rows, R, kSwMaxGran, A->view_row0, sw->hdr, slice_chunks, sw->own_rank, sw->row_of, status);
+    if (A->rp64) hipLaunchKernelGGL(w8_plan_kernel<int64_t>, dim3(nb), dim3(256), 0, ctx->stream, (const int64_t *)A->row_ptr, A->col, A->n_rows, R, kSwMaxGran, A->view_row0, sw->hdr, slice_chunks, sw->own_rank, sw->row_of, status, slice_drop);
+    else hipLaunchKernelGGL(w8_plan_kernel<int32_t>, dim3(nb), dim3(256), 0, ctx->stream, (const int32_t *)A->row_ptr, A->col, A->n_rows, R, kSwMaxGran, A->view_row0, sw->hdr, slice_chunks, sw->own_rank, sw->row_of, status, slice_drop);
     W8_CHECK(hipGetLastError());
     int h[3] = {0, 0, 0};
     W8_CHECK(hipMemcpyAsync(h, status, sizeof h, hipMemcpyDeviceToHost, ctx->stream));
@@ -1810,16 +1879,30 @@
     if (h[0] || (double)total * 256.0 > 1.12 * (double)A->nnz + 256.0 * 4 * 64) {
         if (getenv("BIS_WIN8_STATS")) fprintf(stderr, "win8 plan (R = %d): %s, %.1f %% padding: not used\n", R, h[0] ? "window not representable" : "representable", 100.0 * ((double)total * 256.0 / (double)A->nnz - 1.0));
         *window_too_large = h[0] != 0;
+        hipFree(slice_drop);
         w8_drop_one(A, vb);
         w8_state(A, vb) = -1;
         return BIS_OK;
     }
+    if (slice_drop && (tail_opt > 0 || (size_t)total * kW8ValBytes > ((size_t)256 << 20))) {
+        W8_CHECK(hipMalloc(&sw->slice_skew, sizeof(int64_t) * (size_t)ns1));
+        hipLaunchKernelGGL(sw_widen_kernel, dim3((unsigned)((ns1 + 255) / 256)), dim3(256), 0, ctx->stream, slice_drop, sw->slice_skew, ns1);
+        W8_CHECK(hipGetLastError());
+        tmp_bytes = 0;
+        W8_CHECK(rocprim::exclusive_scan(nullptr, tmp_bytes, sw->slice_skew, sw->slice_skew, (int64_t)0, (size_t)ns1, rocprim::plus<int64_t>(), ctx->stream));
+        W8_CHECK(hipMalloc(&tmp, tmp_bytes));
+        W8_CHECK(rocprim::exclusive_scan(tmp, tmp_bytes, sw->slice_skew, sw->slice_skew, (int64_t)0, (size_t)ns1, rocprim::plus<int64_t>(), ctx->stream));
+        W8_CHECK(hipMemcpyAsync(&sw->dropped_planes, sw->slice_skew + sw->n_slices, sizeof(int64_t), hipMemcpyDeviceToHost, ctx->stream));
+        W8_CHECK(hipStreamSynchronize(ctx->stream));
+        hipFree(tmp); tmp = nullptr;
+    }
+    hipFree(slice_drop); slice_drop = nullptr;
 #define W8_FILL(PHASE, VT, STREAM, DESC, SIDE)                                                                                                    \
     do {                                                                                                                                          \
         if (A->rp64) hipLaunchKernelGGL((w8_fill_kernel<int64_t, PHASE, VT>), dim3(nb), dim3(256), 0, ctx->stream, (const int64_t *)A->row_ptr, A->col, \
-                                        A->val, A->n_rows, R, sw->hdr, sw->slice_chunk0, sw->row_of, STREAM, sw->slice_rec, DESC, SIDE);           \
+                                        A->val, A->n_rows, R, sw->hdr, sw->slice_chunk0, sw->row_of, STREAM, sw->slice_rec, DESC, SIDE, sw->slice_skew);           \
         else hipLaunchKernelGGL((w8_fill_kernel<int32_t, PHASE, VT>), dim3(nb), dim3(256), 0, ctx->stream, (const int32_t *)A->row_ptr, A->col, \
-                                A->val, A->n_rows, R, sw->hdr, sw->slice_chunk0, sw->row_of, STREAM, sw->slice_rec, DESC, SIDE);                   \
+                                A->val, A->n_rows, R, sw->hdr, sw->slice_chunk0, sw->row_of, STREAM, sw->slice_rec, DESC, SIDE, sw->slice_skew);                   \
         W8_CHECK(hipGetLastError());                                                                                                              \
     } while (0)
     sw->expl_chunks = total;
@@ -1840,7 +1923,8 @@
     }
     unsigned char *stream = nullptr;
     const size_t chunk_bytes = sw->slice_rec ? w8_val_bytes(vb) : w8_chunk_bytes(vb);
-    size_t stream_bytes = chunk_bytes * (size_t)(total + 1);
+    const size_t dropped_bytes = 512 * (size_t)sw->dropped_planes;
+    size_t stream_bytes = chunk_bytes * (size_t)(total + 1) - dropped_bytes;
     if (sw->slice_rec) {
         sw->w8_desc = stream_bytes;
         sw->w8_side = sw->w8_desc + ((8 * (size_t)(total + 1) + 255) & ~(size_t)255);
@@ -1848,7 +1932,7 @@
     }
     W8_CHECK(hipMalloc(&stream, stream_bytes));
     sw->codes = reinterpret_cast<uint32_t *>(stream);
-    W8_CHECK(hipMemsetAsync(stream + (size_t)total * chunk_bytes, 0, chunk_bytes, ctx->stream));
+    W8_CHECK(hipMemsetAsync(stream + (size_t)total * chunk_bytes - dropped_bytes, 0, chunk_bytes, ctx->stream));
     if (sw->slice_rec) {
         W8_CHECK(hipMemsetAsync(stream + sw->w8_desc, 0, sw->w8_side - sw->w8_desc, ctx->stream));
         if (vb == 4) W8_FILL(2, float, stream, reinterpret_cast<uint2 *>(stream + sw->w8_desc), stream + sw->w8_side);
@@ -1860,7 +1944,7 @@
 #undef W8_FILL
     w8_state(A, vb) = 1;
     if (bis_status tst = w8_tune_placement(ctx, A, vb)) return tst;
-    if (getenv("BIS_WIN8_STATS")) fprintf(stderr, "win%d plan (R = %d): %d blocks, window <= %d granules (%zu bytes), %.1f %% padding: used; implied slots: %s, %.1f %% of %lld chunks implicit; stream at %p (%zu bytes), hdr %p\n", vb, R, nb, sw->max_gran, (size_t)(2 + 8 * sw->max_gran) * 8, 100.0 * ((double)total * 256.0 / (double)A->nnz - 1.0), sw->slice_rec ? "built" : "not built", 100.0 * (double)(total - sw->expl_chunks) / (double)std::max<int64_t>(total, 1), (long long)total, (void *)sw->codes, bis_spmv_win8_stream_bytes(A, vb), (void *)sw->hdr);
+    if (getenv("BIS_WIN8_STATS")) fprintf(stderr, "win%d plan (R = %d): %d blocks, window <= %d granules (%zu bytes), %.1f %% padding: used; implied slots: %s, %.1f %% of %lld chunks implicit; short tails: %s, %lld planes of 512 bytes dropped; stream at %p (%zu bytes), hdr %p\n", vb, R, nb, sw->max_gran, (size_t)(2 + 8 * sw->max_gran) * 8, 100.0 * ((double)total * 256.0 / (double)A->nnz - 1.0), sw->slice_rec ? "built" : "not built", 100.0 * (double)(total - sw->expl_chunks) / (double)std::max<int64_t>(total, 1), (long long)total, sw->slice_skew ? "on" : "off", (long long)sw->dropped_planes, (void *)sw->codes, bis_spmv_win8_stream_bytes(A, vb), (void *)sw->hdr);
     return BIS_OK;
 }
 #undef W8_CHECK
@@ -1878,10 +1962,11 @@
                       : two ? (sw->R == 1 ? 2 : 3) : (sw->R == 4 ? (ragged ? 2 : 1) : 3);
 #define W8_L3(MODE, RR, DD) do { if (sw->slice_rec) W8_L5(MODE, RR, DD, true); else W8_L5(MODE, RR, DD, false); } while (0)
 #define W8_L5(MODE, RR, DD, IMPL) do { if (vb == 4) W8_L6(MODE, RR, DD, IMPL, float); else W8_L6(MODE, RR, DD, IMPL, double); } while (0)
-#define W8_L6(MODE, RR, DD, IMPL, VT) do { if (two && DD <= 4) W8_L4(MODE, RR, DD, IMPL, VT, (DD <= 4)); else W8_L4(MODE, RR, DD, IMPL, VT, false); } while (0)
-#define W8_L4(MODE, RR, DD, IMPL, VT, TWO) hipLaunchKernelGGL((spmv_win8_kernel<MODE, RR, DD, IMPL, VT, TWO>), dim3(grid), dim3(256), lds, ctx->stream, x, y, A->n_rows, A->n_cols, \
+#define W8_L6(MODE, RR, DD, IMPL, VT) do { if (two && DD <= 4) W8_L7(MODE, RR, DD, IMPL, VT, (DD <= 4)); else W8_L7(MODE, RR, DD, IMPL, VT, false); } while (0)
+#define W8_L7(MODE, RR, DD, IMPL, VT, TWO) do { if (sizeof(VT) == 8 && sw->slice_skew) W8_L4(MODE, RR, DD, IMPL, VT, TWO, (sizeof(VT) == 8)); else W8_L4(MODE, RR, DD, IMPL, VT, TWO, false); } while (0)
+#define W8_L4(MODE, RR, DD, IMPL, VT, TWO, TAIL) hipLaunchKernelGGL((spmv_win8_kernel<MODE, RR, DD, IMPL, VT, TWO, TAIL>), dim3(grid), dim3(256), lds, ctx->stream, x, y, A->n_rows, A->n_cols, \
                                                sw->n_blocks, remap_arg, w, partials, stop, sw->hdr, sw->slice_chunk0, stream, x_al16, own, sw->row_of, \
-                                               reinterpret_cast<const w8_v2u *>(stream + sw->w8_desc), stream + sw->w8_side, sw->slice_rec)
+                                               reinterpret_cast<const w8_v2u *>(stream + sw->w8_desc), stream + sw->w8_side, sw->slice_rec, sw->slice_skew)
 #define W8_L2(MODE, RR) do { if (depth <= 1) W8_L3(MODE, RR, 1); else if (depth == 2) W8_L3(MODE, RR, 2); else if (depth == 3) W8_L3(MODE, RR, 3); else if (depth <= 5) W8_L3(MODE, RR, 4); else W8_L3(MODE, RR, 6); } while (0)
 #define W8_L1(MODE) do { if (sw->R == 4) W8_L2(MODE, 4); else if (sw->R == 2) W8_L2(MODE, 2); else W8_L2(MODE, 1); } while (0)
     if (mode == 1) W8_L1(1); else W8_L1(0);
@@ -1891,6 +1976,7 @@
 #undef W8_L4
 #undef W8_L5
 #undef W8_L6
+#undef W8_L7
     BIS_HIP_CHECK(ctx, hipGetLastError());
     return BIS_OK;
 }
diff --git a/include/bis_hip.h b/include/bis_hip.h
--- a/include/bis_hip.h
+++ b/include/bis_hip.h
@@ -82,6 +82,7 @@
 BIS_API bis_status bis_mat_retune(bis_ctx *ctx, bis_mat *A);
 BIS_API void bis_mat_win8_tuning(const bis_mat *A, int *trials, double *first_ms, double *kept_ms);
 BIS_API void bis_mat_win8_layout(const bis_mat *A, int64_t *chunks, int64_t *explicit_chunks, int64_t *slices, int *blocks, int *implied);
+BIS_API void bis_mat_win8_tail(const bis_mat *A, int64_t *dropped_planes, int *on);
 BIS_API void bis_mat_colslab_info(const bis_mat *A, int *slabs, double *one_pass_ms, double *slab_passes_ms);
 BIS_API bis_status bis_mat_win8_debug_stream(bis_mat *A, void **ptr, size_t *bytes, void *set);
 BIS_API bis_status bis_mat_tune_placement(bis_ctx *ctx, bis_mat *A, int max_trials,
```

New measurement: 1145. 2.3% lower.
